# menmitsu/opticalFlowClustering

Measured on AMD Instinct MI355X. Metric: Mpixels/s dense flow+kmeans @1080p, higher is better.
Workload: dtype f32 storage, f64 accumulation; 1 GPU; BASELINE.json configs[2]: 300-frame 1080p synthetic clip, Farneback flow (0.5,3,15,3,5,1.2,0) + Lloyd k=5 over (u,v), frames sharded over 1 GPU(s); width=1920, height=1080, frames=300, pairs=299, k=5, lloyd_iters=11, flow_batch_pairs=64

## Files before the change

include/ofc.h:

```cpp
#ifndef OFC_H
#define OFC_H
#include <stddef.h>
#include <stdint.h>

#ifdef __cplusplus
extern "C" {
#endif

#define OFC_VERSION 100

enum {
    OFC_OK = 0,
    OFC_EINVAL = -1,
    OFC_ENODEV = -2,
    OFC_EHIP = -3,
    OFC_ENOMEM = -4,
    OFC_ENOTREADY = -5,
    OFC_EUNSUPPORTED = -6,
    OFC_ECOMM = -7
};

enum { OFC_U8 = 0, OFC_F32 = 1, OFC_F64 = 2 };

int ofc_version(void);
const char *ofc_last_error(void);
int ofc_device_count(int *n);

int ofc_malloc(int device, size_t bytes, void **dptr);
int ofc_free(int device, void *dptr);
int ofc_memcpy_h2d(int device, void *dst_dev, const void *src_host, size_t bytes);
int ofc_memcpy_d2h(int device, void *dst_host, const void *src_dev, size_t bytes);
int ofc_memset(int device, void *dst_dev, int value, size_t bytes);
int ofc_device_sync(int device);

typedef struct ofc_fb_params {
    double pyr_scale;
    int levels;
    int winsize;
    int iterations;
    int poly_n;
    double poly_sigma;
    int flags;
} ofc_fb_params;
#define OFC_WINSIZE_MAX 255

void ofc_fb_default_params(ofc_fb_params *p);

typedef struct ofc_flow ofc_flow_t;

int ofc_flow_create(int device, int W, int H, const ofc_fb_params *p, int max_batch,
                    ofc_flow_t **out);
void ofc_flow_destroy(ofc_flow_t *f);

int ofc_flow_calc(ofc_flow_t *f, const uint8_t *prev_gray, const uint8_t *next_gray,
                  float *flow_out);

int ofc_flow_calc_frames_dev(ofc_flow_t *f, const uint8_t *frames_dev, int n_frames,
                             float *flow_dev);
int ofc_flow_calc_frames_dev_stats(ofc_flow_t *f, const uint8_t *frames_dev, int n_frames,
                                   float *flow_dev, double *uv_sum_dev);
int ofc_flow_sync(ofc_flow_t *f);

int ofc_flow_push_gray(ofc_flow_t *f, const uint8_t *gray, float *flow_out);

int ofc_flow_push_bgr(ofc_flow_t *f, const uint8_t *bgr, uint8_t *vis_out, float *mean_mag,
                      float *flow_out);
int ofc_flow_last_vis_dev(ofc_flow_t *f, const uint8_t **vis_dev);

int ofc_level_image(int device, const uint8_t *gray, int W, int H, const ofc_fb_params *p, int k,
                    float *out, int *w_out, int *h_out);
int ofc_polyexp(int device, const float *img, int W, int H, int n, double sigma, float *R5);
int ofc_polyexp_u8(int device, const uint8_t *gray, int W, int H, int n, double sigma, float *R5);
int ofc_update_matrices(int device, const float *R0, const float *R1, const float *flow, int W,
                        int H, float *M);
int ofc_box_solve(int device, const float *M, int W, int H, int winsize, float *flow);
int ofc_flow_resize(int device, const float *flow, int sw, int sh, int dw, int dh, float mul,
                    float *out);

int ofc_flow_iterate(int device, const float *R0, const float *R1, const float *flow_in, int W, int H,
                     int winsize, int iters, int mode, int rows_per_block, float *flow_out);
int ofc_bench_flow_iters(int device, int W, int H, int n_pairs, int reps, int mode, float *ms);

int ofc_bench_polyexp(int device, int W, int H, int n_images, int iters, int rows_per_block,
                      float *ms_per_launch);

int ofc_bgr2gray(int device, const uint8_t *bgr, int W, int H, uint8_t *gray);
int ofc_flow_to_bgr(int device, const float *flow, int W, int H, uint8_t *bgr, float *mean_mag);
int ofc_flow_to_bgr_dev(int device, const float *flow_dev, int W, int H, int n_frames,
                        uint8_t *bgr_dev, float *mean_mag_dev);
int ofc_bgr2hsv(int device, const uint8_t *bgr, int64_t npix, uint8_t *hsv);
int ofc_preprocess_rgba(int device, const uint8_t *img3, int64_t npix, int thresh, uint8_t *rgba);
int ofc_grid_cell_means(int device, const uint8_t *bgr, int W, int H, int rows, int cols,
                        uint8_t *mean_bgr, uint8_t *hsv);

int ofc_kmeans_fit(int device, const void *X, int dtype, int64_t N, int d, int k,
                   const double *init, int max_iter, double tol_rel, double *centers,
                   int32_t *labels, double *inertia, int *n_iter);
int ofc_kmeans_predict(int device, const void *X, int dtype, int64_t N, int d, int k,
                       const double *centers, int32_t *labels);
int ofc_kmeans_fit_dev(int device, const void *X_dev, int dtype, int64_t N, int d, int k,
                       const double *init, int max_iter, double tol_rel, double *centers,
                       uint8_t *labels_dev, double *inertia, int *n_iter);
int ofc_kmeans_fit_dev_stats(int device, const void *X_dev, int dtype, int64_t N, int d, int k,
                             const double *init, int max_iter, double tol_rel, const double *colsum,
                             double *centers, uint8_t *labels_dev, double *inertia, int *n_iter);
int ofc_lloyd_prune_stats(int device, double *out6);
int ofc_bench_lloyd_sweep(int device, const float *X_dev, int64_t N, int k, const double *centers, const double *mean,
                          int what, int iters, float *ms_per_launch);
int ofc_lloyd_colstats_dev(int device, const void *X_dev, int dtype, int64_t N, int d, const double *mean,
                           int pass, double *out);
int ofc_lloyd_step_dev(int device, const void *X_dev, int dtype, int64_t N, int d, int k, const double *mean,
                       const double *centers_c, uint8_t *labels_dev, int accumulate, double *record);
int ofc_lloyd_inertia_dev(int device, const void *X_dev, int dtype, int64_t N, int d, int k, const double *mean,
                          const double *centers_c, const uint8_t *labels_dev, double *inertia);
int ofc_lloyd_farthest_dev(int device, const void *X_dev, int dtype, int64_t N, int d, int k, const double *mean,
                           const double *centers_c, const uint8_t *labels_dev, const int64_t *excl, int n_excl,
                           double *dist2, int64_t *index, double *x_c, int *label);

int ofc_kpp_candidates(int device, const void *X, int dtype, int64_t N, int d, const double *mean,
                       const int64_t *cand, int n_cand, const double *closest, double *out_min, double *pots);
int ofc_kpp_seed_dev(int device, const void *X_dev, int dtype, int64_t N, int d, int k, const double *colsum,
                     int64_t first, const double *u, int n_trials, double *centers, int64_t *indices);
int ofc_kpp_sample_dev(int device, const double *w_dev, int64_t N, const double *r, int n, int64_t *idx);
#define OFC_KPP_CHUNK 1024
int ofc_kmeans_fit_batched(int device, const uint8_t *X, const int64_t *offsets, int n_problems,
                           int d, int k, const double *init, int max_iter, double tol_rel,
                           double *centers, int32_t *counts, int32_t *labels, int *n_iter);
int ofc_grid_kmeans(int device, const uint8_t *bgr, int W, int H, int rows, int cols, int k,
                    const double *init, int max_iter, double tol_rel, int channel_order,
                    double *centers, uint8_t *hsv);

int ofc_grid_kmeans_dev(int device, const uint8_t *bgr_dev, int W, int H, int n_frames, int rows,
                        int cols, int k, const double *init, int max_iter, double tol_rel,
                        int channel_order, double *centers, uint8_t *hsv);

#define OFC_UNIQUE_ID_BYTES 128
int ofc_dist_unique_id(uint8_t id[OFC_UNIQUE_ID_BYTES]);
int ofc_dist_init(int device, int rank, int world, const uint8_t id[OFC_UNIQUE_ID_BYTES]);
int ofc_dist_allreduce_f64(int device, double *buf_dev, int count);
typedef int (*ofc_host_allreduce_fn)(double *buf, int count, int op, void *user);
int ofc_dist_init_host(int device, int rank, int world, ofc_host_allreduce_fn fn, void *user);
int ofc_dist_loopback(int world);
int ofc_dist_finalize(void);

typedef struct ofc_stream ofc_stream_t;
int ofc_stream_create(int device, int W, int H, const ofc_fb_params *p, int batch_pairs, int rows, int cols,
                      ofc_stream_t **out);
int ofc_stream_push_gray(ofc_stream_t *s, const uint8_t *gray, int *pairs_done);
int ofc_stream_finish(ofc_stream_t *s, float *cell_uv, int max_pairs, int *n_pairs);
void ofc_stream_destroy(ofc_stream_t *s);
int ofc_grid_cell_mean_flow(int device, const float *flow, int W, int H, int rows, int cols, float *cell_uv);

int ofc_sliding_cosine(int device, const double *small_v, int n_small, const double *large_v, int n_large,
                       double *sims);

int ofc_synth_frames_dev(int device, uint8_t *frames_dev, int W, int H, int n_frames,
                         int t0, int seed);

#ifdef __cplusplus
}
#endif
#endif
```

opticalflowclustering_amd/_lib.py:

```python
import ctypes as C
import os

import numpy as np

_HERE = os.path.dirname(os.path.abspath(__file__))
LIB_PATH = os.path.join(_HERE, "libofc.so")

OFC_OK, OFC_EINVAL, OFC_ENODEV, OFC_EHIP, OFC_ENOMEM, OFC_ENOTREADY, OFC_EUNSUPPORTED, OFC_ECOMM = \
    0, -1, -2, -3, -4, -5, -6, -7
U8, F32, F64 = 0, 1, 2
UNIQUE_ID_BYTES = 128
KPP_CHUNK = 1024


class OfcError(RuntimeError):
    def __init__(self, code, msg):
        super().__init__(f"libofc error {code}: {msg}")
        self.code = code


class FbParams(C.Structure):
    _fields_ = [("pyr_scale", C.c_double), ("levels", C.c_int), ("winsize", C.c_int),
                ("iterations", C.c_int), ("poly_n", C.c_int), ("poly_sigma", C.c_double),
                ("flags", C.c_int)]

    def __init__(self, pyr_scale=0.5, levels=3, winsize=15, iterations=3, poly_n=5, poly_sigma=1.2,
                 flags=0):
        super().__init__(pyr_scale, levels, winsize, iterations, poly_n, poly_sigma, flags)


_lib = None

_vp, _i, _i64, _f, _d, _sz = C.c_void_p, C.c_int, C.c_int64, C.c_float, C.c_double, C.c_size_t
_ip = C.POINTER(C.c_int)
_PROTOS = {
    "ofc_version": ([], _i),
    "ofc_last_error": ([], C.c_char_p),
    "ofc_device_count": ([_ip], _i),
    "ofc_malloc": ([_i, _sz, C.POINTER(_vp)], _i),
    "ofc_free": ([_i, _vp], _i),
    "ofc_memcpy_h2d": ([_i, _vp, _vp, _sz], _i),
    "ofc_memcpy_d2h": ([_i, _vp, _vp, _sz], _i),
    "ofc_memset": ([_i, _vp, _i, _sz], _i),
    "ofc_device_sync": ([_i], _i),
    "ofc_fb_default_params": ([C.POINTER(FbParams)], None),
    "ofc_flow_create": ([_i, _i, _i, C.POINTER(FbParams), _i, C.POINTER(_vp)], _i),
    "ofc_flow_destroy": ([_vp], None),
    "ofc_flow_calc": ([_vp, _vp, _vp, _vp], _i),
    "ofc_flow_calc_frames_dev": ([_vp, _vp, _i, _vp], _i),
    "ofc_flow_calc_frames_dev_stats": ([_vp, _vp, _i, _vp, _vp], _i),
    "ofc_flow_sync": ([_vp], _i),
    "ofc_flow_push_gray": ([_vp, _vp, _vp], _i),
    "ofc_flow_push_bgr": ([_vp, _vp, _vp, C.POINTER(_f), _vp], _i),
    "ofc_flow_last_vis_dev": ([_vp, C.POINTER(_vp)], _i),
    "ofc_level_image": ([_i, _vp, _i, _i, C.POINTER(FbParams), _i, _vp, _ip, _ip], _i),
    "ofc_polyexp": ([_i, _vp, _i, _i, _i, _d, _vp], _i),
    "ofc_polyexp_u8": ([_i, _vp, _i, _i, _i, _d, _vp], _i),
    "ofc_update_matrices": ([_i, _vp, _vp, _vp, _i, _i, _vp], _i),
    "ofc_box_solve": ([_i, _vp, _i, _i, _i, _vp], _i),
    "ofc_flow_resize": ([_i, _vp, _i, _i, _i, _i, _f, _vp], _i),
    "ofc_flow_iterate": ([_i, _vp, _vp, _vp, _i, _i, _i, _i, _i, _i, _vp], _i),
    "ofc_bench_flow_iters": ([_i, _i, _i, _i, _i, _i, C.POINTER(_f)], _i),
    "ofc_bench_polyexp": ([_i, _i, _i, _i, _i, _i, C.POINTER(_f)], _i),
    "ofc_bgr2gray": ([_i, _vp, _i, _i, _vp], _i),
    "ofc_flow_to_bgr": ([_i, _vp, _i, _i, _vp, C.POINTER(_f)], _i),
    "ofc_flow_to_bgr_dev": ([_i, _vp, _i, _i, _i, _vp, _vp], _i),
    "ofc_bgr2hsv": ([_i, _vp, _i64, _vp], _i),
    "ofc_preprocess_rgba": ([_i, _vp, _i64, _i, _vp], _i),
    "ofc_grid_cell_means": ([_i, _vp, _i, _i, _i, _i, _vp, _vp], _i),
    "ofc_kmeans_fit": ([_i, _vp, _i, _i64, _i, _i, _vp, _i, _d, _vp, _vp, C.POINTER(_d), _ip], _i),
    "ofc_kmeans_predict": ([_i, _vp, _i, _i64, _i, _i, _vp, _vp], _i),
    "ofc_kmeans_fit_dev": ([_i, _vp, _i, _i64, _i, _i, _vp, _i, _d, _vp, _vp, C.POINTER(_d), _ip], _i),
    "ofc_kmeans_fit_dev_stats": ([_i, _vp, _i, _i64, _i, _i, _vp, _i, _d, _vp, _vp, _vp, C.POINTER(_d), _ip], _i),
    "ofc_lloyd_prune_stats": ([_i, _vp], _i),
    "ofc_bench_lloyd_sweep": ([_i, _vp, _i64, _i, _vp, _vp, _i, _i, C.POINTER(_f)], _i),
    "ofc_lloyd_colstats_dev": ([_i, _vp, _i, _i64, _i, _vp, _i, _vp], _i),
    "ofc_lloyd_step_dev": ([_i, _vp, _i, _i64, _i, _i, _vp, _vp, _vp, _i, _vp], _i),
    "ofc_lloyd_inertia_dev": ([_i, _vp, _i, _i64, _i, _i, _vp, _vp, _vp, C.POINTER(_d)], _i),
    "ofc_lloyd_farthest_dev": ([_i, _vp, _i, _i64, _i, _i, _vp, _vp, _vp, _vp, _i, C.POINTER(_d), C.POINTER(_i64), _vp, _ip], _i),
    "ofc_kpp_candidates": ([_i, _vp, _i, _i64, _i, _vp, _vp, _i, _vp, _vp, _vp], _i),
    "ofc_kpp_seed_dev": ([_i, _vp, _i, _i64, _i, _i, _vp, _i64, _vp, _i, _vp, _vp], _i),
    "ofc_kpp_sample_dev": ([_i, _vp, _i64, _vp, _i, _vp], _i),
    "ofc_kmeans_fit_batched": ([_i, _vp, _vp, _i, _i, _i, _vp, _i, _d, _vp, _vp, _vp, _vp], _i),
    "ofc_grid_kmeans": ([_i, _vp, _i, _i, _i, _i, _i, _vp, _i, _d, _i, _vp, _vp], _i),
    "ofc_grid_kmeans_dev": ([_i, _vp, _i, _i, _i, _i, _i, _i, _vp, _i, _d, _i, _vp, _vp], _i),
    "ofc_dist_unique_id": ([_vp], _i),
    "ofc_dist_init": ([_i, _i, _i, _vp], _i),
    "ofc_dist_allreduce_f64": ([_i, _vp, _i], _i),
    "ofc_dist_init_host": ([_i, _i, _i, _vp, _vp], _i),
    "ofc_dist_loopback": ([_i], _i),
    "ofc_dist_finalize": ([], _i),
    "ofc_stream_create": ([_i, _i, _i, C.POINTER(FbParams), _i, _i, _i, C.POINTER(_vp)], _i),
    "ofc_stream_push_gray": ([_vp, _vp, _ip], _i),
    "ofc_stream_finish": ([_vp, _vp, _i, _ip], _i),
    "ofc_stream_destroy": ([_vp], None),
    "ofc_grid_cell_mean_flow": ([_i, _vp, _i, _i, _i, _i, _vp], _i),
    "ofc_sliding_cosine": ([_i, _vp, _i, _vp, _i, _vp], _i),
    "ofc_synth_frames_dev": ([_i, _vp, _i, _i, _i, _i, _i], _i),
}
EXPORTS = tuple(_PROTOS)


def load():
    global _lib
    if _lib is None:
        if not os.path.exists(LIB_PATH):
            raise OfcError(OFC_ENODEV, f"{LIB_PATH} not built: run `make -C {_HERE}/csrc` "
                                       "(python -c 'import __graft_entry__ as g; g.build()')")
        lib = C.CDLL(LIB_PATH)
        for name, (args, res) in _PROTOS.items():
            fn = getattr(lib, name)
            fn.argtypes = args
            fn.restype = res
        _lib = lib
    return _lib


def check(rc):
    if rc != OFC_OK:
        msg = load().ofc_last_error().decode("utf-8", "replace")
        if rc == OFC_EINVAL:
            raise ValueError(msg)
        raise OfcError(rc, msg)


def ptr(a):
    return a.ctypes.data_as(C.c_void_p) if a is not None else None


def device_count():
    n = C.c_int()
    check(load().ofc_device_count(C.byref(n)))
    return n.value


class DeviceBuffer:

    def __init__(self, nbytes, device=0):
        self.device, self.nbytes = device, int(nbytes)
        p = C.c_void_p()
        check(load().ofc_malloc(device, self.nbytes, C.byref(p)))
        self.ptr = p.value

    def upload(self, arr, offset=0):
        arr = np.ascontiguousarray(arr)
        assert offset + arr.nbytes <= self.nbytes
        check(load().ofc_memcpy_h2d(self.device, self.ptr + offset, ptr(arr), arr.nbytes))
        return self

    def download(self, shape, dtype, offset=0):
        out = np.empty(shape, dtype)
        assert offset + out.nbytes <= self.nbytes
        check(load().ofc_memcpy_d2h(self.device, ptr(out), self.ptr + offset, out.nbytes))
        return out

    def zero(self):
        check(load().ofc_memset(self.device, self.ptr, 0, self.nbytes))

    def free(self):
        if self.ptr:
            load().ofc_free(self.device, self.ptr)
            self.ptr = None

    def __del__(self):
        try:
            self.free()
        except Exception:
            pass
```

opticalflowclustering_amd/cluster.py:

```python
import ctypes as C

import numpy as np

from . import _lib
from ._lib import check, load, ptr

_DT = {np.dtype(np.uint8): _lib.U8, np.dtype(np.float32): _lib.F32, np.dtype(np.float64): _lib.F64}


def _as_supported(X):
    X = np.asarray(X)
    if X.ndim != 2:
        raise ValueError(f"Expected 2D array, got {X.ndim}D array instead")
    if X.dtype not in _DT:
        X = X.astype(np.float64)
    return np.ascontiguousarray(X)


def seeded_rows_init(X, k, random_state=0):
    rng = np.random.default_rng(random_state)
    X = np.asarray(X)
    uniq = np.unique(X, axis=0)
    if len(uniq) >= k:
        return uniq[rng.choice(len(uniq), k, replace=False)].astype(np.float64)
    return X[rng.choice(len(X), k, replace=len(X) < k)].astype(np.float64)


def check_random_state(seed):
    if seed is None or seed is np.random:
        return np.random.mtrand._rand
    if isinstance(seed, (int, np.integer)):
        return np.random.RandomState(int(seed))
    if isinstance(seed, np.random.RandomState):
        return seed
    raise ValueError(f"{seed!r} cannot be used to seed a numpy.random.RandomState instance")


def kmeans_plusplus(X, n_clusters, random_state=None, n_local_trials=None, device=0, _step=None):
    X = _as_supported(X)
    N, d = X.shape
    rs = check_random_state(random_state)
    if n_local_trials is None:
        n_local_trials = 2 + int(np.log(n_clusters))
    if n_local_trials > 8:
        raise ValueError("n_local_trials > 8 is not supported")
    mean = X.astype(np.float64).mean(axis=0) if X.dtype != np.float32 else X.mean(axis=0).astype(np.float64)
    weight = np.ones(N, np.float64)
    indices = np.full(n_clusters, -1, dtype=np.int64)
    indices[0] = rs.choice(N, p=weight / weight.sum())

    def step(cand, closest):
        cand = np.ascontiguousarray(cand, np.int64)
        if _step is not None:
            return _step(X, mean, cand, closest)
        out = np.empty((len(cand), N), np.float64)
        pots = np.empty(len(cand), np.float64)
        check(load().ofc_kpp_candidates(device, ptr(X), _DT[X.dtype], N, d, ptr(mean), ptr(cand), len(cand),
                                        ptr(closest) if closest is not None else None, ptr(out), ptr(pots)))
        return out, pots

    out, pots = step(indices[:1], None)
    closest, current_pot = out[0], pots[0]
    for c in range(1, n_clusters):
        rand_vals = rs.uniform(size=n_local_trials) * current_pot
        candidate_ids = np.searchsorted(np.cumsum(closest, dtype=np.float64), rand_vals)
        np.clip(candidate_ids, None, N - 1, out=candidate_ids)
        out, pots = step(candidate_ids, closest)
        best = int(np.argmin(pots))
        current_pot, closest = pots[best], out[best]
        indices[c] = candidate_ids[best]
    return X[indices].astype(np.float64), indices


KPP_CHOICE_MAX = 1 << 24


def kpp_draws(rs, N, n_clusters, n_local_trials=None):
    if n_local_trials is None:
        n_local_trials = 2 + int(np.log(n_clusters))
    if n_local_trials > 8:
        raise ValueError("n_local_trials > 8 is not supported")
    if N <= KPP_CHOICE_MAX:
        weight = np.ones(N, np.float64)
        first = int(rs.choice(N, p=weight / weight.sum()))
    else:
        first = min(int(rs.random_sample() * N), N - 1)
    u = np.empty((n_clusters - 1, n_local_trials), np.float64)
    for c in range(n_clusters - 1):
        u[c] = rs.uniform(size=n_local_trials)
    return first, u, n_local_trials


def kmeans_plusplus_dev(X_ptr, dtype, N, d, n_clusters, random_state=None, n_local_trials=None, device=0,
                        colsum=None, n_global=None):
    n_global = int(N if n_global is None else n_global)
    if n_global < 1:
        raise ValueError(f"n_samples={n_global} should be >= n_clusters={n_clusters}.")
    first, u, n_local_trials = kpp_draws(check_random_state(random_state), n_global, int(n_clusters), n_local_trials)
    cs = np.ascontiguousarray(colsum, np.float64) if colsum is not None else None
    if cs is not None and cs.shape != (d,):
        raise ValueError(f"colsum must have shape ({d},)")
    centers = np.empty((n_clusters, d), np.float64)
    indices = np.empty(n_clusters, np.int64)
    check(load().ofc_kpp_seed_dev(device, C.c_void_p(X_ptr), dtype, N, d, n_clusters, ptr(cs), first, ptr(u),
                                  n_local_trials, ptr(centers), ptr(indices)))
    return centers, indices


class KMeans:
    def __init__(self, n_clusters=8, *, init="seeded-rows", n_init=1, max_iter=300, tol=1e-4,
                 random_state=0, device=0, **_ignored):
        self.n_clusters, self.init, self.n_init = int(n_clusters), init, n_init
        self.max_iter, self.tol, self.random_state, self.device = int(max_iter), float(tol), random_state, device

    def _init_centers(self, X):
        if isinstance(self.init, str):
            if self.init == "k-means++":
                return None
            if self.init not in ("seeded-rows", "random"):
                raise ValueError(f"init should be an array, 'k-means++' or 'seeded-rows', got {self.init!r}")
            return seeded_rows_init(X, self.n_clusters, self.random_state if self.random_state is not None else 0)
        C0 = np.ascontiguousarray(self.init, np.float64)
        if C0.shape != (self.n_clusters, X.shape[1]):
            raise ValueError(f"The shape of the initial centers {C0.shape} does not match "
                             f"({self.n_clusters}, {X.shape[1]})")
        return C0

    def fit(self, X, y=None, sample_weight=None):
        if sample_weight is not None:
            raise ValueError("sample_weight is not supported (the reference never passes it)")
        X = _as_supported(X)
        N, d = X.shape
        k = self.n_clusters
        if N < k:
            raise ValueError(f"n_samples={N} should be >= n_clusters={k}.")
        C0 = self._init_centers(X)
        centers = np.empty((k, d), np.float64)
        labels = np.empty(N, np.int32)
        inertia, n_iter = C.c_double(), C.c_int()
        if C0 is None:
            Xd = _lib.DeviceBuffer(X.nbytes, self.device)
            Ld = _lib.DeviceBuffer(N, self.device)
            try:
                Xd.upload(X)
                C0, _ = kmeans_plusplus_dev(Xd.ptr, _DT[X.dtype], N, d, k, self.random_state, device=self.device)
                check(load().ofc_kmeans_fit_dev(self.device, C.c_void_p(Xd.ptr), _DT[X.dtype], N, d, k, ptr(C0),
                                                self.max_iter, self.tol, ptr(centers), C.c_void_p(Ld.ptr),
                                                C.byref(inertia), C.byref(n_iter)))
                labels[:] = Ld.download((N,), np.uint8)
            finally:
                Xd.free()
                Ld.free()
        else:
            check(load().ofc_kmeans_fit(self.device, ptr(X), _DT[X.dtype], N, d, k, ptr(C0), self.max_iter,
                                        self.tol, ptr(centers), ptr(labels), C.byref(inertia), C.byref(n_iter)))
        self.cluster_centers_, self.labels_ = centers, labels
        self.inertia_, self.n_iter_ = inertia.value, n_iter.value
        self.n_features_in_ = d
        return self

    def predict(self, X):
        X = _as_supported(X)
        N, d = X.shape
        if d != self.cluster_centers_.shape[1]:
            raise ValueError(f"X has {d} features, but KMeans is expecting {self.cluster_centers_.shape[1]}")
        labels = np.empty(N, np.int32)
        cen = np.ascontiguousarray(self.cluster_centers_, np.float64)
        check(load().ofc_kmeans_predict(self.device, ptr(X), _DT[X.dtype], N, d, self.n_clusters, ptr(cen), ptr(labels)))
        return labels

    def fit_predict(self, X, y=None):
        return self.fit(X).labels_


def kmeans_fit_dev(X_ptr, dtype, N, d, init, max_iter=300, tol=1e-4, labels_ptr=None, device=0, colsum=None):
    C0 = np.ascontiguousarray(init, np.float64)
    k = C0.shape[0]
    centers = np.empty((k, d), np.float64)
    inertia, n_iter = C.c_double(), C.c_int()
    cs = np.ascontiguousarray(colsum, np.float64) if colsum is not None else None
    if cs is not None and cs.shape != (d,):
        raise ValueError(f"colsum must have shape ({d},)")
    check(load().ofc_kmeans_fit_dev_stats(device, C.c_void_p(X_ptr), dtype, N, d, k, ptr(C0), max_iter, tol, ptr(cs), ptr(centers),
                                          C.c_void_p(labels_ptr) if labels_ptr else None, C.byref(inertia), C.byref(n_iter)))
    return centers, inertia.value, n_iter.value


def prune_stats(device=0):
    out = np.zeros(6, np.float64)
    check(load().ofc_lloyd_prune_stats(device, ptr(out)))
    return {"tile_sweeps": int(out[0]), "pruned_sweeps": int(out[1]), "probe_sweeps": int(out[4]), "final_pruned": bool(out[5]),
            "skip_fraction": float(out[3] / out[2]) if out[2] > 0 else 0.0}
```

opticalflowclustering_amd/csrc/flow_kernels.hip:

```cpp
#include "flow_device.h"

namespace ofc {

__device__ __forceinline__ void lin_tap_x(int dx, double scale, int sw, int &s0, float &a)
{
#pragma clang fp contract(off)
    float fx = (float)((dx + 0.5) * scale - 0.5);
    int sx = (int)floorf(fx);
    fx -= (float)sx;
    if (sx < 0) { fx = 0.f; sx = 0; }
    if (sx >= sw - 1) { fx = 0.f; sx = sw - 1; }
    s0 = sx;
    a = fx;
}

__device__ __forceinline__ void lin_tap_y(int dy, double scale, int sh, int &s0, int &s1, float &b)
{
#pragma clang fp contract(off)
    float fy = (float)((dy + 0.5) * scale - 0.5);
    int sy = (int)floorf(fy);
    fy -= (float)sy;
    s0 = min(max(sy, 0), sh - 1);
    s1 = min(max(sy + 1, 0), sh - 1);
    b = fy;
}

__device__ __forceinline__ int reflect101(int p, int len)
{
    if (len == 1) return 0;
    while (p < 0 || p >= len) p = p < 0 ? -p : 2 * (len - 1) - p;
    return p;
}

struct LevelArgs {
    int W0, H0, w, h;
    int r;
    int txo, tyo;
    int in_w, in_h;
    int in_pitch;
    double sx, sy;
    float kern[32];
};

__global__ __launch_bounds__(256) void k_level_image(const uint8_t *__restrict__ src,
                                                     float *__restrict__ dst, LevelArgs p)
{
#pragma clang fp contract(off)
    extern __shared__ __align__(16) unsigned char smem[];
    const int tid = threadIdx.x;
    const int ox0 = blockIdx.x * p.txo, oy0 = blockIdx.y * p.tyo;
    const int nox = min(p.txo, p.w - ox0), noy = min(p.tyo, p.h - oy0);
    const uint8_t *img = src + (size_t)blockIdx.z * p.W0 * p.H0;
    float *out = dst + (size_t)blockIdx.z * p.w * p.h;

    int *xs0 = reinterpret_cast<int *>(smem);
    float *xa = reinterpret_cast<float *>(xs0 + p.txo);
    int *ys0 = reinterpret_cast<int *>(xa + p.txo);
    int *ys1 = ys0 + p.tyo;
    float *yb = reinterpret_cast<float *>(ys1 + p.tyo);
    float *h1 = yb + p.tyo;
    unsigned char *tile = reinterpret_cast<unsigned char *>(h1 + (size_t)p.in_h * 2 * p.txo);

    if (tid < nox) {
        int s0; float a;
        lin_tap_x(ox0 + tid, p.sx, p.W0, s0, a);
        xs0[tid] = s0; xa[tid] = a;
    }
    if (tid >= 64 && tid - 64 < noy) {
        int s0, s1; float b;
        lin_tap_y(oy0 + tid - 64, p.sy, p.H0, s0, s1, b);
        ys0[tid - 64] = s0; ys1[tid - 64] = s1; yb[tid - 64] = b;
    }
    __syncthreads();
    const int x_first = xs0[0], x_last = min(xs0[nox - 1] + 1, p.W0 - 1);
    const int y_first = ys0[0], y_last = ys1[noy - 1];
    const int ix0 = x_first - p.r, iy0 = y_first - p.r;
    const int tw = x_last - x_first + 1 + 2 * p.r, th = y_last - y_first + 1 + 2 * p.r;

    for (int i = tid; i < tw * th; i += 256) {
        int ly = i / tw, lx = i - ly * tw;
        int gx = reflect101(ix0 + lx, p.W0), gy = reflect101(iy0 + ly, p.H0);
        tile[ly * p.in_pitch + lx] = img[(size_t)gy * p.W0 + gx];
    }
    __syncthreads();

    const int ks = 2 * p.r + 1;
    for (int i = tid; i < th * nox * 2; i += 256) {
        int ly = i / (nox * 2), rem = i - ly * nox * 2;
        int j = rem >> 1, t = rem & 1;
        int x = min(xs0[j] + t, p.W0 - 1);
        const unsigned char *row = tile + ly * p.in_pitch + (x - x_first);
        float acc = p.kern[0] * (float)row[0];
        for (int q = 1; q < ks; q++) acc += p.kern[q] * (float)row[q];
        h1[(ly * p.txo + j) * 2 + t] = acc;
    }
    __syncthreads();

    for (int i = tid; i < noy * nox; i += 256) {
        int oy = i / nox, ox = i - oy * nox;
        float a1 = xa[ox], a0 = 1.f - a1, b1 = yb[oy], b0 = 1.f - b1;
        float hrow[2];
#pragma unroll
        for (int yt = 0; yt < 2; yt++) {
            int c = (yt ? ys1[oy] : ys0[oy]) - iy0;
            float v[2];
#pragma unroll
            for (int t = 0; t < 2; t++) {
                if (t == 1 && a1 == 0.f) { v[1] = 0.f; continue; }
                const float *col = h1 + (c * p.txo + ox) * 2 + t;
                float acc = p.kern[p.r] * col[0];
                for (int m = 1; m <= p.r; m++)
                    acc += p.kern[p.r + m] * (col[-m * p.txo * 2] + col[m * p.txo * 2]);
                v[t] = acc;
            }
            hrow[yt] = (a1 == 0.f) ? v[0] : v[0] * a0 + v[1] * a1;
        }
        out[(size_t)(oy0 + oy) * p.w + ox0 + ox] = hrow[0] * b0 + hrow[1] * b1;
    }
}

__device__ __forceinline__ float ubyte_of(uint32_t w, int n) { return (float)((w >> (8 * n)) & 255u); }

__global__ __launch_bounds__(256) void k_level0(const uint8_t *__restrict__ src, float *__restrict__ dst,
                                                int W, int H, float k0, float k1, float k2)
{
#pragma clang fp contract(off)
    const int tx = threadIdx.x & 63, ty = threadIdx.x >> 6;
    const int x0 = blockIdx.x * 256 + 4 * tx, y0 = blockIdx.y * 32 + 8 * ty;
    if (x0 >= W || y0 >= H) return;
    const uint8_t *img = src + (size_t)blockIdx.z * W * H;
    float *out = dst + (size_t)blockIdx.z * W * H;
    const bool fast = x0 >= 4 && x0 + 8 <= W;
    float h[10][4];
#pragma unroll
    for (int j = 0; j < 10; j++) {
        const uint8_t *row = img + (size_t)reflect101(y0 - 1 + j, H) * W;
        float b[6];
        if (fast) {
            const uint32_t *rw = reinterpret_cast<const uint32_t *>(row + x0);
            const uint32_t wa = rw[-1], wb = rw[0], wc = rw[1];
            b[0] = ubyte_of(wa, 3);
            b[1] = ubyte_of(wb, 0); b[2] = ubyte_of(wb, 1); b[3] = ubyte_of(wb, 2); b[4] = ubyte_of(wb, 3);
            b[5] = ubyte_of(wc, 0);
        } else {
#pragma unroll
            for (int q = 0; q < 6; q++) b[q] = (float)row[reflect101(x0 - 1 + q, W)];
        }
#pragma unroll
        for (int c = 0; c < 4; c++) {
            float acc = k0 * b[c];
            acc += k1 * b[c + 1];
            acc += k2 * b[c + 2];
            h[j][c] = acc;
// ... 648 lines not shown

        double ex[5];
#pragma unroll
        for (int c = 0; c < 5; c++) {
            double s = 0;
#pragma unroll
            for (int i = 0; i < 4; i++) s += in[i] ? v[c][i] : 0.0;
            double t = s;
#pragma unroll
            for (int d = 1; d < 64; d <<= 1) {
                const double o = __shfl_up(t, d);
                if (lane >= d) t += o;
            }
            ex[c] = __shfl_up(t, 1);
            if (lane == 0) ex[c] = 0;
            if (lane == 63) wtot[c][wave] = t;
        }
        __syncthreads();
#pragma unroll
        for (int c = 0; c < 5; c++) {
            double off = ex[c];
            for (int w = 0; w < wave; w++) off += wtot[c][w];
            double p[4], s = 0;
#pragma unroll
            for (int i = 0; i < 4; i++) {
                s += in[i] ? v[c][i] : 0.0;
                p[i] = s + off;
            }
            *reinterpret_cast<double2 *>(&P[c][4 * tid]) = make_double2(p[0], p[1]);
            *reinterpret_cast<double2 *>(&P[c][4 * tid + 2]) = make_double2(p[2], p[3]);
        }
#pragma unroll
        for (int i = 0; i < 4; i++) {
            if (in[i] && col[i] == 0)
#pragma unroll
                for (int c = 0; c < 5; c++) edge[0][c] = v[c][i];
            if (in[i] && col[i] == W - 1)
#pragma unroll
                for (int c = 0; c < 5; c++) edge[1][c] = v[c][i];
        }
        __syncthreads();
        for (int j = tid; j < TX; j += 256) {
            const int x = x0 + j;
            if (x >= W) break;
            const double nr = (double)max(x + m - (W - 1), 0), nl = (double)max(m - x, 0);
            double S[5];
#pragma unroll
            for (int c = 0; c < 5; c++) {
                S[c] = P[c][j + 2 * m + 1] - P[c][j];
                if (nr > 0) S[c] += nr * edge[1][c];
                if (nl > 0) S[c] += nl * edge[0][c];
            }
            const double g11 = S[0] * scale, g12 = S[1] * scale, g22 = S[2] * scale, h1 = S[3] * scale,
                         h2 = S[4] * scale;
            const double idet = 1. / (g11 * g22 - g12 * g12 + 1e-3);
            flow[(size_t)y * W + x] = make_float2((float)((g11 * h2 - g12 * h1) * idet),
                                                  (float)((g22 * h1 - g12 * h2) * idet));
        }
        __syncthreads();
#pragma unroll
        for (int c = 0; c < 5; c++)
#pragma unroll
            for (int i = 0; i < 4; i++) v[c][i] += (double)fa[c][i] - (double)Mp[c * plane + os + col[i]];
    }
}

int box_wide_rows(int winsize) { return std::max(2 * winsize, 64); }

static int launch_box_solve_wide(const float *M, float *flow, int npair, int W, int H, int winsize,
                                 int rows_per_block, hipStream_t s)
{
    if (!(winsize & 1) || winsize < WINSIZE_WIDE_MIN || winsize > OFC_WINSIZE_MAX) {
        set_error("winsize %d unsupported (odd 5..%d)", winsize, OFC_WINSIZE_MAX);
        return OFC_EUNSUPPORTED;
    }
    if (rows_per_block <= 0) rows_per_block = box_wide_rows(winsize);
    const int m = winsize / 2;
    dim3 grid(cdiv(W, BW_SPAN - 2 * m - 1), cdiv(H, rows_per_block), npair);
    hipLaunchKernelGGL(k_box_solve_wide, grid, dim3(256), 0, s, M, flow, W, H, m, rows_per_block);
    OFC_HIP(hipGetLastError());
    return OFC_OK;
}

int launch_box_solve(const float *M, float *flow, int npair, int W, int H, int winsize,
                     int rows_per_block, hipStream_t s)
{
    if (winsize >= WINSIZE_WIDE_MIN) return launch_box_solve_wide(M, flow, npair, W, H, winsize, rows_per_block, s);
    if (rows_per_block <= 0) rows_per_block = box_default_rows(W, H, npair);
    rows_per_block = cdiv(rows_per_block, BS_ROWS) * BS_ROWS;
    dim3 block(256);
#define OFC_BOX_CASE(MM)                                                                         \
    case 2 * MM + 1: {                                                                           \
        dim3 grid(cdiv(W, 256 - 2 * MM), cdiv(H, rows_per_block), npair);                        \
        hipLaunchKernelGGL(k_box_solve<MM>, grid, block, 0, s, M, flow, W, H, rows_per_block);   \
        break;                                                                                   \
    }
    switch (winsize) {
        OFC_BOX_CASE(2)
        OFC_BOX_CASE(3)
        OFC_BOX_CASE(4)
        OFC_BOX_CASE(5)
        OFC_BOX_CASE(6)
        OFC_BOX_CASE(7)
        OFC_BOX_CASE(8)
    default:
        set_error("winsize %d unsupported (odd 5..%d)", winsize, OFC_WINSIZE_MAX);
        return OFC_EUNSUPPORTED;
    }
#undef OFC_BOX_CASE
    OFC_HIP(hipGetLastError());
    return OFC_OK;
}

struct UpsArgs {
    const float *src;
    int sw, sh;
    double scx, scy;
    float mul;
};

__device__ __forceinline__ float2 upsampled_flow(const float2 *__restrict__ s, int sw, int sh, double scx, double scy,
                                                 float mul, int x, int y)
{
#pragma clang fp contract(off)
    int sx0, sy0, sy1;
    float a1, b1;
    if (scx == 0.5 && scy == 0.5) {
        const int sx = (x + 1) / 2 - 1, sy = (y + 1) / 2 - 1;
        a1 = (x & 1) ? 0.25f : 0.75f;
        b1 = (y & 1) ? 0.25f : 0.75f;
        sx0 = sx;
        if (sx < 0) { a1 = 0.f; sx0 = 0; }
        if (sx >= sw - 1) { a1 = 0.f; sx0 = sw - 1; }
        sy0 = min(max(sy, 0), sh - 1);
        sy1 = min(max(sy + 1, 0), sh - 1);
    } else {
        lin_tap_x(x, scx, sw, sx0, a1);
        lin_tap_y(y, scy, sh, sy0, sy1, b1);
    }
    const float a0 = 1.f - a1, b0 = 1.f - b1;
    const int sx1 = (a1 == 0.f) ? sx0 : sx0 + 1;
    const float2 p00 = s[(size_t)sy0 * sw + sx0], p01 = s[(size_t)sy0 * sw + sx1];
    const float2 p10 = s[(size_t)sy1 * sw + sx0], p11 = s[(size_t)sy1 * sw + sx1];
    float h0x, h0y, h1x, h1y;
    if (a1 == 0.f) {
        h0x = p00.x; h0y = p00.y; h1x = p10.x; h1y = p10.y;
    } else {
        h0x = p00.x * a0 + p01.x * a1; h0y = p00.y * a0 + p01.y * a1;
        h1x = p10.x * a0 + p11.x * a1; h1y = p10.y * a0 + p11.y * a1;
    }
    return make_float2((h0x * b0 + h1x * b1) * mul, (h0y * b0 + h1y * b1) * mul);
}

template <int M, int UPS, bool STAMP = false, bool SUMS = false>
__global__ __launch_bounds__(256, 2) void k_flow_iter(const float *__restrict__ Rb, size_t frame_stride_R,
                                                      const float *__restrict__ flow_inb,
                                                      float *__restrict__ flow_outb, int W, int H,
                                                      int rows_per_block , UpsArgs ups,
                                                      int tiles_x, int n_strips, int npair,
                                                      unsigned long long *__restrict__ dbg = nullptr,
                                                      double *__restrict__ sums = nullptr)
{
    constexpr int TXO = 256 - 2 * M;
    constexpr int NV = 2 * M + 4;
    constexpr int NV2 = (NV + 1) / 2;
    constexpr int PLD = 136, PITCH = 2 * PLD;
    __shared__ __align__(16) double vs[5][BS_ROWS][PITCH];
    const int tid = threadIdx.x, lane = tid & 63, wave = tid >> 6;
    const int tiles = tiles_x * n_strips;
    const int group = blockIdx.x / (8 * npair), rem = blockIdx.x - group * (8 * npair);
    const int pair = rem >> 3, tile = group * 8 + (rem & 7);
    if (tile >= tiles) {
        if (SUMS && threadIdx.x < 2) sums[(size_t)blockIdx.x * 2 + threadIdx.x] = 0.0;
        return;
    }
    double su = 0, sv = 0;
    const int tile_x = tile % tiles_x, tile_y = tile / tiles_x;
    const int x0 = tile_x * TXO;
    const int y_begin = tile_y * rows_per_block;
    const int y_end = min(y_begin + rows_per_block, H);
    const size_t plane = (size_t)W * H;
    const float *R0 = Rb + (size_t)pair * frame_stride_R;
    const float *R1 = R0 + frame_stride_R;
    const float2 *flow_in = UPS ? reinterpret_cast<const float2 *>(ups.src) + (size_t)pair * ups.sw * ups.sh
                                : reinterpret_cast<const float2 *>(flow_inb) + (size_t)pair * plane;
    float2 *flow_out = reinterpret_cast<float2 *>(flow_outb) + (size_t)pair * plane;
    const int xc = min(max(x0 - M + tid, 0), W - 1);
    const int vs_w = ((tid >> 1) & 1) * PLD + 2 * (tid >> 2) + (tid & 1);
    const double scale = 1.0 / ((2 * M + 1) * (2 * M + 1));
    auto flow_at = [&](int row) -> float2 {
        if (UPS) return upsampled_flow(flow_in, ups.sw, ups.sh, ups.scx, ups.scy, ups.mul, xc, row);
        return flow_in[(size_t)row * W + xc];
    };
    constexpr bool ups2 = UPS == 2;
    int usx0 = 0, usx1 = 0;
    float ua1 = 0.f;
    if (ups2) {
        const int sx = (xc + 1) / 2 - 1;
        ua1 = (xc & 1) ? 0.25f : 0.75f;
        usx0 = sx;
        if (sx < 0) { ua1 = 0.f; usx0 = 0; }
        if (sx >= ups.sw - 1) { ua1 = 0.f; usx0 = ups.sw - 1; }
        usx1 = (ua1 == 0.f) ? usx0 : usx0 + 1;
    }
    auto coarse_taps = [&](int sy, float2 &p0, float2 &p1) {
        const float2 *rowp = flow_in + (size_t)min(max(sy, 0), ups.sh - 1) * ups.sw;
        p0 = rowp[usx0];
        p1 = rowp[usx1];
    };
    auto coarse_lerp = [&](float2 p0, float2 p1) -> float2 {
#pragma clang fp contract(off)
        if (ua1 == 0.f) return p0;
        const float a0 = 1.f - ua1;
        return make_float2(p0.x * a0 + p1.x * ua1, p0.y * a0 + p1.y * ua1);
    };
    float2 hcar[2], pn[2][2];
    bool have_next = false;
    float2 fl_last = ups2 ? flow_at(H - 1) : make_float2(0.f, 0.f);

    float ring[16][5];
    double v[5] = {0, 0, 0, 0, 0};

#pragma unroll
    for (int j4 = -M; j4 <= M; j4 += BS_ROWS) {
        float2 fl[BS_ROWS];
        UmIn u[BS_ROWS];
        __builtin_amdgcn_s_setprio(3);
#pragma unroll
        for (int q = 0; q < BS_ROWS; q++) fl[q] = flow_at(min(max(y_begin + j4 + q, 0), H - 1));
#pragma unroll
        for (int q = 0; q < BS_ROWS; q++)
            um_load(R0, R1, plane, W, H, xc, min(max(y_begin + j4 + q, 0), H - 1), fl[q], u[q]);
        __builtin_amdgcn_s_setprio(0);
#pragma unroll
        for (int q = 0; q < BS_ROWS; q++) {
            if (j4 + q <= M) {
                const int row = min(max(y_begin + j4 + q, 0), H - 1);
                float m[5];
                um_math(u[q], W, H, xc, row, fl[q], m);
#pragma unroll
                for (int c = 0; c < 5; c++) {
                    ring[(j4 + q + 16) & 15][c] = m[c];
                    v[c] += (double)m[c];
                }
            }
        }
    }

    float2 fln[BS_ROWS];
    if (!UPS) {
#pragma unroll
        for (int r = 0; r < BS_ROWS; r++) fln[r] = flow_in[(size_t)min(y_begin + r + 1 + M, H - 1) * W + xc];
    }
    unsigned long long acc_t[8] = {0, 0, 0, 0, 0, 0, 0, 0}, tprev = 0;
    auto stamp = [&](int slot) {
        if (STAMP) {
            __builtin_amdgcn_sched_barrier(0);
            const unsigned long long t = __builtin_amdgcn_s_memtime();
            __builtin_amdgcn_sched_barrier(0);
            if (slot >= 0) acc_t[slot] += t - tprev;
            tprev = t;
        }
    };
    stamp(-1);
    for (int y16 = y_begin; y16 < y_end; y16 += 16) {
#pragma unroll
        for (int q4 = 0; q4 < 4; q4++) {
            const int yc = y16 + 4 * q4;
            if (yc < y_end) {
                float2 fl[BS_ROWS];
                float mi[BS_ROWS][5];
                if (ups2) {
#pragma clang fp contract(off)
                    const int e0 = yc + 1 + M, s0 = (e0 + 1) / 2 - 1;
                    float2 hc[BS_ROWS];
                    if (have_next) {
                        hc[0] = hcar[0];
                        hc[1] = hcar[1];
                        hc[2] = coarse_lerp(pn[0][0], pn[0][1]);
                        hc[3] = coarse_lerp(pn[1][0], pn[1][1]);
                    } else {
#pragma unroll
                        for (int j = 0; j < BS_ROWS; j++) {
                            float2 p0, p1;
                            coarse_taps(s0 + j, p0, p1);
                            hc[j] = coarse_lerp(p0, p1);
                        }
                    }
                    hcar[0] = hc[2];
                    hcar[1] = hc[3];
                    have_next = true;
#pragma unroll
                    for (int r = 0; r < BS_ROWS; r++) {
                        constexpr bool E0_EVEN = ((1 + M) & 1) == 0;
                        const int off = E0_EVEN ? (r + 1) / 2 : r / 2;
                        const float b1 = (E0_EVEN == ((r & 1) == 0)) ? 0.75f : 0.25f, b0 = 1.f - b1;
                        const float2 h0 = hc[off], h1 = hc[off + 1];
                        fl[r] = make_float2((h0.x * b0 + h1.x * b1) * ups.mul, (h0.y * b0 + h1.y * b1) * ups.mul);
                        if (e0 + r > H - 1) fl[r] = fl_last; else fl_last = fl[r];
                    }
                } else {
#pragma unroll
                    for (int r = 0; r < BS_ROWS; r++)
                        fl[r] = UPS ? flow_at(min(yc + r + 1 + M, H - 1)) : fln[r];
                }
                {
                    UmIn u[BS_ROWS];
                    stamp(0);
                    __builtin_amdgcn_s_setprio(3);
#pragma unroll
                    for (int q = 0; q < BS_ROWS; q++)
                        um_load(R0, R1, plane, W, H, xc, min(yc + q + 1 + M, H - 1), fl[q], u[q]);
                    if (!UPS) {
#pragma unroll
                        for (int r = 0; r < BS_ROWS; r++)
                            fln[r] = flow_in[(size_t)min(yc + BS_ROWS + r + 1 + M, H - 1) * W + xc];
                    }
                    stamp(1);
                    if (STAMP) {
                        asm volatile("s_waitcnt vmcnt(0)" ::: "memory");
                        stamp(2);
                    }
                    __builtin_amdgcn_s_setprio(2);
#pragma unroll
                    for (int r = 0; r < BS_ROWS; r++)
                        um_math(u[r], W, H, xc, min(yc + r + 1 + M, H - 1), fl[r], mi[r]);
                }
                if (ups2) {
                    const int s0n = (yc + BS_ROWS + 1 + M + 1) / 2 - 1;
                    coarse_taps(s0n + 2, pn[0][0], pn[0][1]);
                    coarse_taps(s0n + 3, pn[1][0], pn[1][1]);
                }
                stamp(7);
                __syncthreads();
                stamp(3);
#pragma unroll
                for (int r = 0; r < BS_ROWS; r++) {
                    const int s_in = (4 * q4 + r + 1 + M) & 15, s_out = (4 * q4 + r + 16 - M) & 15;
#pragma unroll
                    for (int c = 0; c < 5; c++) {
                        vs[c][r][vs_w] = v[c];
                        v[c] += (double)mi[r][c] - (double)ring[s_out][c];
                    }
#pragma unroll
                    for (int c = 0; c < 5; c++) ring[s_in][c] = mi[r][c];
                }
                stamp(4);
                __syncthreads();
                stamp(5);
                __builtin_amdgcn_s_setprio(0);
                const int y = yc + wave;
                const int xo = x0 + 4 * lane;
                if (y < y_end && 4 * lane < TXO && xo < W) {
                    double S[5][4];
#pragma unroll
                    for (int c = 0; c < 5; c++) {
                        double a[2 * NV2];
#pragma unroll
                        for (int q = 0; q < NV2; q++) {
                            double2 d = *reinterpret_cast<const double2 *>(&vs[c][wave][(q & 1) * PLD + 2 * (lane + (q >> 1))]);
                            a[2 * q] = d.x; a[2 * q + 1] = d.y;
                        }
                        double s = a[0];
#pragma unroll
                        for (int q = 1; q <= 2 * M; q++) s += a[q];
                        S[c][0] = s;
#pragma unroll
                        for (int o = 1; o < 4; o++) {
                            s += a[2 * M + o] - a[o - 1];
                            S[c][o] = s;
                        }
                    }
                    float2 fo[4];
#pragma unroll
                    for (int o = 0; o < 4; o++) {
                        const double g11 = S[0][o] * scale, g12 = S[1][o] * scale, g22 = S[2][o] * scale,
                                     h1 = S[3][o] * scale, h2 = S[4][o] * scale;
                        const double idet = 1. / (g11 * g22 - g12 * g12 + 1e-3);
                        fo[o] = make_float2((float)((g11 * h2 - g12 * h1) * idet), (float)((g22 * h1 - g12 * h2) * idet));
                    }
                    if (SUMS) {
#pragma unroll
                        for (int o = 0; o < 4; o++)
                            if (4 * lane + o < TXO && xo + o < W) { su += (double)fo[o].x; sv += (double)fo[o].y; }
                    }
                    float2 *dst = flow_out + (size_t)y * W + xo;
                    if (4 * lane + 3 < TXO && xo + 3 < W && (W & 1) == 0) {
                        reinterpret_cast<float4 *>(dst)[0] = make_float4(fo[0].x, fo[0].y, fo[1].x, fo[1].y);
                        reinterpret_cast<float4 *>(dst)[1] = make_float4(fo[2].x, fo[2].y, fo[3].x, fo[3].y);
                    } else {
#pragma unroll
                        for (int o = 0; o < 4; o++)
                            if (4 * lane + o < TXO && xo + o < W) dst[o] = fo[o];
                    }
                }
                stamp(6);
            }
        }
    }
    if (STAMP && dbg && lane == 0) {
#pragma unroll
        for (int i = 0; i < 8; i++) dbg[((size_t)blockIdx.x * 4 + wave) * 8 + i] = acc_t[i];
    }
    if (SUMS) {
        for (int off = 32; off >= 1; off >>= 1) {
            su += __shfl_down(su, off, 64);
            sv += __shfl_down(sv, off, 64);
        }
        __syncthreads();
        if (lane == 0) { vs[0][0][2 * wave] = su; vs[0][0][2 * wave + 1] = sv; }
        __syncthreads();
        if (tid < 2) sums[(size_t)blockIdx.x * 2 + tid] = ((vs[0][0][tid] + vs[0][0][2 + tid]) + vs[0][0][4 + tid]) + vs[0][0][6 + tid];
    }
}

int flow_iter_rows(int W, int H, int npair, int winsize)
{
    const int tiles_x = cdiv(W, 256 - (winsize - 1));
    const int resident = 2 * 256;
    int best_rows = cdiv(H, 16) * 16;
    int64_t best_cost = LLONG_MAX;
    for (int n = 1; n <= 32; n++) {
        const int rows = cdiv(cdiv(H, n), 16) * 16;
        if (rows < 16 && n > 1) break;
        const int64_t blocks = (int64_t)tiles_x * cdiv(H, rows) * npair;
        const int64_t cost = cdiv64(blocks, resident) * (rows + winsize - 1);
        if (cost < best_cost) { best_cost = cost; best_rows = rows; }
    }
    return best_rows;
}

int flow_iter_max_grid(int W, int H, int npair, int winsize)
{
    const int rows = flow_iter_rows(W, H, npair, winsize);
    return cdiv(cdiv(W, 256 - (winsize - 1)) * cdiv(H, rows), 8) * 8 * npair;
}

static int flow_iter_check(int W, int H, int winsize)
{
    if (winsize > 15) { set_error("fused iteration supports winsize <= 15 (ring of 16 rows)"); return OFC_EUNSUPPORTED; }
    if ((int64_t)W * H * 5 >= (1ll << 30)) { set_error("frame too large for 32-bit R offsets (%dx%d)", W, H); return OFC_EUNSUPPORTED; }
    return OFC_OK;
}

int launch_flow_iter(const float *R, size_t frame_stride_R, const float *flow_in, float *flow_out,
                     int npair, int W, int H, int winsize, hipStream_t s, const float *coarse, int sw, int sh,
                     float mul, double *uv_sum, double *uv_scratch, size_t uv_scratch_doubles)
{
    OFC_TRY(flow_iter_check(W, H, winsize));
    const int rows_per_block = flow_iter_rows(W, H, npair, winsize);
    UpsArgs u;
    u.src = coarse; u.sw = sw; u.sh = sh; u.mul = mul;
    u.scx = coarse ? (double)sw / W : 1.0; u.scy = coarse ? (double)sh / H : 1.0;
    {
        const char *e = getenv("OFC_FLOW_PIPE");
        if (e && e[0] == '1' && winsize == 15 && !coarse)
            return launch_flow_iter_pipe(R, frame_stride_R, flow_in, flow_out, npair, W, H, rows_per_block, s, uv_sum, uv_scratch,
                                         uv_scratch_doubles);
    }
    if (uv_sum) {
        if (coarse || winsize != 15) { set_error("flow sums are emitted by the plain winsize-15 iteration only"); return OFC_EUNSUPPORTED; }
        const int tx = cdiv(W, 256 - 14), ns = cdiv(H, rows_per_block);
        const int grid = cdiv(tx * ns, 8) * 8 * npair;
        if ((size_t)grid * 2 > uv_scratch_doubles) { set_error("flow sums: scratch too small (%d work-groups)", grid); return OFC_EINVAL; }
        hipLaunchKernelGGL((k_flow_iter<7, 0, false, true>), dim3(grid), dim3(256), 0, s, R, frame_stride_R, flow_in, flow_out, W, H,
                           rows_per_block, u, tx, ns, npair, nullptr, uv_scratch);
        OFC_HIP(hipGetLastError());
        return launch_reduce_records(uv_scratch, grid, 2, uv_sum, s, nullptr);
    }
    dim3 block(256);
#define OFC_FI_CASE(MM)                                                                                  \
    case 2 * MM + 1: {                                                                                   \
        const int tx = cdiv(W, 256 - 2 * MM), ns = cdiv(H, rows_per_block);                              \
        dim3 grid(cdiv(tx * ns, 8) * 8 * npair);                                                         \
        if (coarse && u.scx == 0.5 && u.scy == 0.5)                                                      \
            hipLaunchKernelGGL((k_flow_iter<MM, 2>), grid, block, 0, s, R, frame_stride_R, flow_in,      \
                               flow_out, W, H, rows_per_block, u, tx, ns, npair);                        \
        else if (coarse)                                                                                 \
            hipLaunchKernelGGL((k_flow_iter<MM, 1>), grid, block, 0, s, R, frame_stride_R, flow_in,      \
                               flow_out, W, H, rows_per_block, u, tx, ns, npair);                        \
        else                                                                                             \
            hipLaunchKernelGGL((k_flow_iter<MM, 0>), grid, block, 0, s, R, frame_stride_R, flow_in,      \
                               flow_out, W, H, rows_per_block, u, tx, ns, npair);                        \
        break;                                                                                           \
    }
    switch (winsize) {
        OFC_FI_CASE(2)
        OFC_FI_CASE(3)
        OFC_FI_CASE(4)
        OFC_FI_CASE(5)
        OFC_FI_CASE(6)
        OFC_FI_CASE(7)
    default:
        set_error("winsize %d unsupported by the fused iteration (odd 5..15)", winsize);
        return OFC_EUNSUPPORTED;
    }
#undef OFC_FI_CASE
    OFC_HIP(hipGetLastError());
    return OFC_OK;
}

int launch_flow_iter_stamped(const float *R, size_t frame_stride_R, const float *flow_in, float *flow_out, int npair, int W,
                             int H, hipStream_t s, unsigned long long *dbg, int *grid_out)
{
    const int rows_per_block = flow_iter_rows(W, H, npair, 15);
    UpsArgs u;
    u.src = nullptr; u.sw = 0; u.sh = 0; u.mul = 1.f; u.scx = 1.0; u.scy = 1.0;
    const int tx = cdiv(W, 256 - 14), ns = cdiv(H, rows_per_block);
    dim3 grid(cdiv(tx * ns, 8) * 8 * npair);
    if (grid_out) *grid_out = (int)grid.x;
    if (dbg)
        hipLaunchKernelGGL((k_flow_iter<7, 0, true>), grid, dim3(256), 0, s, R, frame_stride_R, flow_in, flow_out, W, H,
                           rows_per_block, u, tx, ns, npair, dbg);
    OFC_HIP(hipGetLastError());
    return OFC_OK;
}

int flow_levels_check(int W, int H, const ofc_fb_params &p, const LevelGeom *geom, int levels, bool fused, bool fuse_level0)
{
    for (int k = levels; k >= 0; k--) {
        const LevelGeom &g = geom[k];
        int rc = OFC_OK;
        if (!(k == 0 && fuse_level0 && polyexp_u8_ok(W, H, g))) {
            LevelArgs a;
            int path;
            size_t lds;
            rc = level_image_plan(W, H, g, true, a, path, lds);
        }
        if (rc == OFC_OK && fused) rc = flow_iter_check(g.w, g.h, p.winsize);
        if (rc == OFC_OK) continue;
        const std::string why = ofc_last_error();
        if (g.ksize > 31) {
            int ok = k;
            while (ok > 0 && geom[ok].ksize > 31) ok--;
            set_error("pyramid level %d (%dx%d, sigma %.3g) of %dx%d at pyr_scale %g: %s; levels <= %d is supported with this "
                      "pyr_scale (a level may shrink the frame by less than 13.6x)", k, g.w, g.h, g.sigma, W, H, p.pyr_scale,
                      why.c_str(), ok);
        } else {
            set_error("pyramid level %d (%dx%d) of %dx%d at pyr_scale %g: %s", k, g.w, g.h, W, H, p.pyr_scale, why.c_str());
        }
        return rc;
    }
    return OFC_OK;
}

__global__ __launch_bounds__(256) void k_flow_resize(const float2 *__restrict__ src,
                                                     float2 *__restrict__ dst, int sw, int sh, int dw,
                                                     int dh, double scx, double scy, float mul)
{
#pragma clang fp contract(off)
    const int x = blockIdx.x * 256 + threadIdx.x, y = blockIdx.y;
    if (x >= dw) return;
    const float2 *s = src + (size_t)blockIdx.z * sw * sh;
    float2 *d = dst + (size_t)blockIdx.z * dw * dh;
    if (sw == dw && sh == dh) {
        float2 v = s[(size_t)y * sw + x];
        d[(size_t)y * dw + x] = make_float2(v.x * mul, v.y * mul);
        return;
    }
    int sx0, sy0, sy1;
    float a1, b1;
    lin_tap_x(x, scx, sw, sx0, a1);
    lin_tap_y(y, scy, sh, sy0, sy1, b1);
    const float a0 = 1.f - a1, b0 = 1.f - b1;
    const int sx1 = (a1 == 0.f) ? sx0 : sx0 + 1;
    const float2 p00 = s[(size_t)sy0 * sw + sx0], p01 = s[(size_t)sy0 * sw + sx1];
    const float2 p10 = s[(size_t)sy1 * sw + sx0], p11 = s[(size_t)sy1 * sw + sx1];
    float h0x, h0y, h1x, h1y;
    if (a1 == 0.f) {
        h0x = p00.x; h0y = p00.y; h1x = p10.x; h1y = p10.y;
    } else {
        h0x = p00.x * a0 + p01.x * a1; h0y = p00.y * a0 + p01.y * a1;
        h1x = p10.x * a0 + p11.x * a1; h1y = p10.y * a0 + p11.y * a1;
    }
    d[(size_t)y * dw + x] = make_float2((h0x * b0 + h1x * b1) * mul, (h0y * b0 + h1y * b1) * mul);
}

int launch_flow_resize(const float *src, float *dst, int npair, int sw, int sh, int dw, int dh,
                       float mul, hipStream_t s)
{
    dim3 grid(cdiv(dw, 256), dh, npair);
    hipLaunchKernelGGL(k_flow_resize, grid, dim3(256), 0, s, reinterpret_cast<const float2 *>(src),
                       reinterpret_cast<float2 *>(dst), sw, sh, dw, dh, (double)sw / dw,
                       (double)sh / dh, mul);
    OFC_HIP(hipGetLastError());
    return OFC_OK;
}

}
```

opticalflowclustering_amd/csrc/lloyd_api.cpp:

```cpp
#include "lloyd_common.h"

#include <algorithm>
#include <cmath>
#include <cstdlib>
#include <mutex>

namespace ofc {

static int lloyd_grid(int64_t N)
{
    return (int)std::max<int64_t>(1, std::min<int64_t>(cdiv64(N / 4, 256), N >= (200ll << 20) ? 2048 : 1024));
}

static size_t dtype_size(int dtype) { return dtype == OFC_U8 ? 1 : (dtype == OFC_F32 ? 4 : 8); }

struct LloydScratch {
    DevBuf state, partial, tot, tot_local, excl, far, labels;
    DevBuf tile_box, tile_sum, tile_sq;
    DevBuf tile_meta;
    DevBuf kpp_closest, kpp_cs, kpp_ss;
    DevBuf kpp_io;
    double prune_stats[6] = {0, 0, 0, 0, 0, 0};
    LloydStatus *status = nullptr;
    LloydStatus *status_dev = nullptr;
    hipStream_t stream = nullptr;
    bool ready = false;
    std::mutex mu;
    int init()
    {
        if (ready) return OFC_OK;
        constexpr int NVMAX = LLOYD_NVMAX;
        OFC_HIP(hipStreamCreateWithFlags(&stream, hipStreamNonBlocking));
        OFC_TRY(state.alloc(sizeof(LloydState)));
        OFC_TRY(partial.alloc(sizeof(double) * 2048 * NVMAX));
        OFC_TRY(tot.alloc(sizeof(double) * (NVMAX + 8)));
        OFC_TRY(tot_local.alloc(sizeof(double) * (NVMAX + 8)));
        OFC_TRY(excl.alloc(sizeof(int64_t) * LLOYD_KMAX));
        OFC_TRY(far.alloc(sizeof(double) * 2 * 2048));
        OFC_TRY(tile_meta.alloc(sizeof(double) * 8));
        OFC_HIP(hipHostMalloc((void **)&status, sizeof(LloydStatus) * LLOYD_WINDOW, hipHostMallocMapped));
        OFC_HIP(hipHostGetDevicePointer((void **)&status_dev, status, 0));
        ready = true;
        return OFC_OK;
    }
};

static int prune_policy_for(int dtype, int64_t N, int d, int k)
{
    if (!lloyd_tiles_supported(dtype, d, k) || N < 64) return LLOYD_PRUNE_OFF;
    const char *e = getenv("OFC_LLOYD_PRUNE");
    const int v = (e && e[0] >= '0' && e[0] <= '3' && !e[1]) ? e[0] - '0' : LLOYD_PRUNE_AUTO;
    if (v == LLOYD_PRUNE_AUTO && N < (1ll << 20)) return LLOYD_PRUNE_OFF;
    return v;
}

static LloydScratch &scratch_for(int device)
{
    static LloydScratch *pool = new LloydScratch[16];
    return pool[device & 15];
}

static int relocate_empty(LloydScratch &sc, const void *X, int dtype, int64_t N, int d, int k, int kmax,
                          int nblocks, const uint8_t *labels, const double *mean_h)
{
    hipStream_t s = sc.stream;
    const int NV = lloyd_record_len(kmax, d);
    std::vector<double> tot(NV);
    OFC_HIP(hipMemcpyAsync(tot.data(), sc.tot.p, sizeof(double) * NV, hipMemcpyDeviceToHost, s));
    OFC_HIP(hipStreamSynchronize(s));
    double *w = tot.data() + kmax * d;
    LloydState *st = sc.state.as<LloydState>();
    const double *c_old = st->centers;
    std::vector<int64_t> excl;
    std::vector<double> blk(2 * nblocks);
    bool first = true;
    for (int j = 0; j < k; j++) {
        if (w[j] != 0.0) continue;
        if (!excl.empty())
            OFC_HIP(hipMemcpyAsync(sc.excl.p, excl.data(), sizeof(int64_t) * excl.size(), hipMemcpyHostToDevice, s));
        OFC_TRY(launch_lloyd_farthest(X, dtype, N, d, st, c_old, labels, sc.excl.as<int64_t>(), (int)excl.size(),
                                      sc.far.as<double>(), nblocks, s));
        OFC_HIP(hipMemcpyAsync(blk.data(), sc.far.p, sizeof(double) * 2 * nblocks, hipMemcpyDeviceToHost, s));
        OFC_HIP(hipStreamSynchronize(s));
        double best = -1;
        int64_t bi = -1;
        for (int b = 0; b < nblocks; b++) {
            const double v = blk[2 * b];
            const int64_t i = (int64_t)blk[2 * b + 1];
            if (i < 0) continue;
            if (v > best || (v == best && i < bi)) { best = v; bi = i; }
        }
        double rec[LLOYD_DMAX + 3];
        int owner = 1;
        if (dist_active()) {
            double *dv = sc.far.as<double>();
            double g = best;
            OFC_HIP(hipMemcpyAsync(dv, &g, sizeof(double), hipMemcpyHostToDevice, s));
            OFC_TRY(dist_allreduce_f64(dv, 1, DIST_MAX, s));
            OFC_HIP(hipMemcpyAsync(&g, dv, sizeof(double), hipMemcpyDeviceToHost, s));
            OFC_HIP(hipStreamSynchronize(s));
            double r = (bi >= 0 && best == g) ? (double)dist_rank() : 1e300;
            OFC_HIP(hipMemcpyAsync(dv, &r, sizeof(double), hipMemcpyHostToDevice, s));
            OFC_TRY(dist_allreduce_f64(dv, 1, DIST_MIN, s));
            OFC_HIP(hipMemcpyAsync(&r, dv, sizeof(double), hipMemcpyDeviceToHost, s));
            OFC_HIP(hipStreamSynchronize(s));
            owner = ((int)r == dist_rank()) && bi >= 0 && best == g;
            best = g;
        }
        if (first && !(best > 0)) return OFC_OK;
        first = false;
        memset(rec, 0, sizeof(rec));
        if (owner) {
            unsigned char raw[LLOYD_DMAX * 8];
            uint8_t lab;
            OFC_HIP(hipMemcpyAsync(raw, (const char *)X + (size_t)bi * d * dtype_size(dtype), d * dtype_size(dtype),
                                   hipMemcpyDeviceToHost, s));
            OFC_HIP(hipMemcpyAsync(&lab, labels + bi, 1, hipMemcpyDeviceToHost, s));
            OFC_HIP(hipStreamSynchronize(s));
            for (int f = 0; f < d; f++) {
                double v = dtype == OFC_U8 ? (double)raw[f]
                         : dtype == OFC_F32 ? (double)((float *)raw)[f] : ((double *)raw)[f];
                rec[f] = v - mean_h[f];
            }
            rec[d] = (double)lab;
            excl.push_back(bi);
        }
        if (dist_active()) {
            double *dv = sc.far.as<double>();
            OFC_HIP(hipMemcpyAsync(dv, rec, sizeof(double) * (d + 1), hipMemcpyHostToDevice, s));
            OFC_TRY(dist_allreduce_f64(dv, d + 1, DIST_BCAST, s));
            OFC_HIP(hipMemcpyAsync(rec, dv, sizeof(double) * (d + 1), hipMemcpyDeviceToHost, s));
            OFC_HIP(hipStreamSynchronize(s));
        }
        const int old = (int)rec[d];
        for (int f = 0; f < d; f++) {
            tot[old * d + f] -= rec[f];
            tot[j * d + f] = rec[f];
        }
        w[j] = 1.0;
        w[old] -= 1.0;
    }
    OFC_HIP(hipMemcpyAsync(sc.tot.p, tot.data(), sizeof(double) * NV, hipMemcpyHostToDevice, s));
    OFC_HIP(hipStreamSynchronize(s));
    return OFC_OK;
}

static int lloyd_fit_dev(int device, const void *X, int dtype, int64_t N, int d, int k, const double *init,
                         int max_iter, double tol_rel, double *centers, uint8_t *labels_dev,
                         double *inertia, int *n_iter, const double *colsum = nullptr)
{
    OFC_REQUIRE(X && init && centers, "null pointer");
    OFC_REQUIRE(dtype >= OFC_U8 && dtype <= OFC_F64, "bad dtype %d", dtype);
    OFC_REQUIRE(d >= 1 && k >= 1 && max_iter >= 1 && N >= 0, "bad shape");
    if (d > LLOYD_DMAX || k > LLOYD_KMAX) {
        set_error("k=%d, d=%d outside the kernels' range (k <= %d, d <= %d)", k, d, LLOYD_KMAX, LLOYD_DMAX);
        return OFC_EUNSUPPORTED;
    }
    OFC_TRY(ensure_device(device));
    const int kmax = lloyd_kmax(k);
    const int NV = lloyd_record_len(kmax, d);
    LloydScratch &sc = scratch_for(device);
    std::lock_guard<std::mutex> lock(sc.mu);
    OFC_TRY(sc.init());
    hipStream_t s = sc.stream;
    const int nblocks = lloyd_grid(N);
    if (!labels_dev) {
        if (sc.labels.bytes < (size_t)std::max<int64_t>(N, 1)) OFC_TRY(sc.labels.alloc((size_t)std::max<int64_t>(N, 1)));
        labels_dev = sc.labels.as<uint8_t>();
    }
    LloydState *st = sc.state.as<LloydState>();
    OFC_HIP(hipMemsetAsync(st, 0, sizeof(LloydState), s));
    double *tot = sc.tot.as<double>();

    double hbuf[LLOYD_DMAX + 1], mean_h[LLOYD_DMAX];
    if (colsum) {
        OFC_HIP(hipMemcpyAsync(tot, colsum, sizeof(double) * d, hipMemcpyHostToDevice, s));
    } else {
        OFC_TRY(launch_lloyd_colstats(X, dtype, N, d, st->mean, 0, sc.partial.as<double>(), nblocks, s));
        OFC_TRY(launch_reduce_records(sc.partial.as<double>(), nblocks, d, tot, s));
    }
    double nloc = (double)N;
    OFC_HIP(hipMemcpyAsync(tot + d, &nloc, sizeof(double), hipMemcpyHostToDevice, s));
    OFC_TRY(dist_allreduce_f64(tot, d + 1, DIST_SUM, s));
    OFC_HIP(hipMemcpyAsync(hbuf, tot, sizeof(double) * (d + 1), hipMemcpyDeviceToHost, s));
    OFC_HIP(hipStreamSynchronize(s));
    const double Ng = hbuf[d];
    if (Ng < (double)k) {
        set_error("n_samples=%.0f should be >= n_clusters=%d.", Ng, k);
        return OFC_EINVAL;
    }
    for (int f = 0; f < d; f++) mean_h[f] = hbuf[f] / Ng;
    OFC_HIP(hipMemcpyAsync(st->mean, mean_h, sizeof(double) * d, hipMemcpyHostToDevice, s));

    double c0[LLOYD_KMAX * LLOYD_DMAX];
    for (int j = 0; j < k * d; j++) c0[j] = init[j] - mean_h[j % d];
    OFC_HIP(hipMemcpyAsync(st->centers, c0, sizeof(double) * k * d, hipMemcpyHostToDevice, s));
    const int prune = prune_policy_for(dtype, N, d, k);
    if (prune) {
        const size_t need = (size_t)(N >> 6) * 16;
        if (sc.tile_box.bytes < need) {
            OFC_TRY(sc.tile_box.alloc(need));
            OFC_TRY(sc.tile_sum.alloc(need));
            OFC_TRY(sc.tile_sq.alloc(need / 2));
        }
    }
    for (double &v : sc.prune_stats) v = 0;
    OFC_TRY(launch_lloyd_set_centers(st, k, d, s, prune));
    bool strict = false, labelled = false, stop = false;
    int tiles_next = LLOYD_TILES_FULL;
    const bool trace = getenv("OFC_LLOYD_TRACE") != nullptr;
    int it = 0;
    const int *halt = &st->halt;
    double *tot_local = dist_has_comm() ? sc.tot_local.as<double>() : tot;
    int window = 4;
    while (it < max_iter && !stop) {
        const int nwin = std::min(window, max_iter - it);
        window = std::min(2 * window, LLOYD_WINDOW);
        for (int w = 0; w < nwin; w++) sc.status[w].valid = 0;
        for (int w = 0; w < nwin; w++) {
            const int tiles = (prune && !labelled) ? (it + w == 0 ? 1 : 2) : 0;
            if (tiles == 1) {
                OFC_TRY(launch_lloyd_tiles((const float *)X, N, k, st, nullptr, nullptr, nullptr, nullptr,
                                           sc.partial.as<double>(), nblocks, LLOYD_WHAT_PROBE, nullptr, s));
                OFC_TRY(launch_lloyd_tiles((const float *)X, N, k, st, sc.tile_box.p, sc.tile_sum.p, sc.tile_sq.p, nullptr,
                                           sc.partial.as<double>(), nblocks, LLOYD_WHAT_META, nullptr, s));
                OFC_TRY(launch_reduce_records(sc.partial.as<double>(), nblocks, 2, sc.tile_meta.as<double>(), s));
            }
            if (tiles)
                OFC_TRY(launch_lloyd_tiles((const float *)X, N, k, st, sc.tile_box.p, sc.tile_sum.p, sc.tile_sq.p, nullptr,
                                           sc.partial.as<double>(), nblocks, LLOYD_WHAT_SWEEP,
                                           tiles == 1 ? sc.tile_meta.as<double>() : nullptr, s));
            else
                OFC_TRY(launch_lloyd_assign(X, dtype, N, d, k, st, labels_dev, sc.partial.as<double>(), nblocks,
                                            labelled ? 1 : 3, it + w == 0, s));
            OFC_TRY(launch_reduce_records(sc.partial.as<double>(), nblocks, NV, tot_local, s, halt));
            OFC_TRY(dist_allreduce_f64(tot_local, tot, NV, DIST_SUM, s));
            OFC_TRY(launch_lloyd_update(st, tot, k, d, 0, labelled, it + w == 0, Ng, tol_rel, sc.status_dev + w, s, tiles));
        }
        OFC_HIP(hipStreamSynchronize(s));
        int done = nwin;
        for (int w = 0; w < nwin; w++) {
            LloydStatus &S = sc.status[w];
            if (!S.valid) { set_error("internal: Lloyd iteration %d did not run", it + w); return OFC_EHIP; }
            if (trace)
                fprintf(stderr, "[ofc lloyd] it %d tiles_mode %d tested %.0f pure %.0f shift %.3e empty %d\n", it + w,
                        S.tiles_mode, S.tiles_tested, S.tiles_pure, S.shift_tot, S.n_empty);
            if (S.tiles_mode != -1) {
                tiles_next = S.tiles_next;
                sc.prune_stats[0] += 1;
                if (S.tiles_mode == LLOYD_TILES_PRUNED) {
                    sc.prune_stats[1] += 1;
                    sc.prune_stats[2] += S.tiles_tested;
                    sc.prune_stats[3] += S.tiles_pure;
                } else if (S.tiles_mode == LLOYD_TILES_PROBE) {
                    sc.prune_stats[4] += 1;
                }
            }
            if (S.n_empty > 0) {
                const bool was_labelled = labelled;
                if (!labelled) {
                    OFC_TRY(launch_lloyd_assign(X, dtype, N, d, k, st, labels_dev, nullptr, nblocks, 0, 0, s));
                    labelled = true;
                }
                OFC_TRY(relocate_empty(sc, X, dtype, N, d, k, kmax, nblocks, labels_dev, mean_h));
                S.valid = 0;
                OFC_TRY(launch_lloyd_update(st, tot, k, d, 1, was_labelled, it + w == 0, Ng, tol_rel, sc.status_dev + w, s));
                OFC_HIP(hipStreamSynchronize(s));
                done = w + 1;
                if (S.converged) { strict = S.strict != 0; it += w; stop = true; }
                break;
            }
            if (S.converged) { strict = S.strict != 0; it += w; stop = true; break; }
        }
        if (!stop) it += done;
    }
    if (!stop) it = max_iter - 1;
    const bool final_tiles = !strict && prune && !labelled && tiles_next == LLOYD_TILES_PRUNED;
    sc.prune_stats[5] = final_tiles ? 1 : 0;
    if (final_tiles)
        OFC_TRY(launch_lloyd_tiles((const float *)X, N, k, st, sc.tile_box.p, sc.tile_sum.p, sc.tile_sq.p, labels_dev,
                                   sc.partial.as<double>(), nblocks, LLOYD_WHAT_FINAL, nullptr, s));
    else if (!strict)
        OFC_TRY(launch_lloyd_assign(X, dtype, N, d, k, st, labels_dev, sc.partial.as<double>(), nblocks, 2, 0, s));
    else
        OFC_TRY(launch_lloyd_inertia(X, dtype, N, d, st, labels_dev, sc.partial.as<double>(), nblocks, s));
    OFC_TRY(launch_reduce_records(sc.partial.as<double>(), nblocks, 1, tot, s));
    OFC_TRY(dist_allreduce_f64(tot, 1, DIST_SUM, s));
    double in = 0, cfin[LLOYD_KMAX * LLOYD_DMAX];
    OFC_HIP(hipMemcpyAsync(&in, tot, sizeof(double), hipMemcpyDeviceToHost, s));
    OFC_HIP(hipMemcpyAsync(cfin, st->centers, sizeof(double) * k * d, hipMemcpyDeviceToHost, s));
    OFC_HIP(hipStreamSynchronize(s));
    for (int j = 0; j < k * d; j++) centers[j] = cfin[j] + mean_h[j % d];
    if (inertia) *inertia = in;
    if (n_iter) *n_iter = it + 1;
    return OFC_OK;
}

static int lloyd_predict_dev(int device, const void *X, int dtype, int64_t N, int d, int k,
                             const double *centers, uint8_t *labels_dev)
{
    OFC_TRY(ensure_device(device));
    if (d > LLOYD_DMAX || k > LLOYD_KMAX || d < 1 || k < 1) {
        set_error("k=%d, d=%d outside the kernels' range (k <= %d, d <= %d)", k, d, LLOYD_KMAX, LLOYD_DMAX);
        return OFC_EUNSUPPORTED;
    }
    DevBuf state;
    OFC_TRY(state.alloc(sizeof(LloydState)));
    LloydState *st = state.as<LloydState>();
    OFC_HIP(hipMemset(st, 0, sizeof(LloydState)));
    OFC_HIP(hipMemcpy(st->centers, centers, sizeof(double) * k * d, hipMemcpyHostToDevice));
    OFC_TRY(launch_lloyd_set_centers(st, k, d, nullptr));
    const int nblocks = lloyd_grid(N);
    OFC_TRY(launch_lloyd_assign(X, dtype, N, d, k, st, labels_dev, nullptr, nblocks, 0, 0, nullptr));
    OFC_HIP(hipStreamSynchronize(nullptr));
    return OFC_OK;
}

static void widen_labels(const uint8_t *src, int64_t N, int32_t *dst)
{
    for (int64_t i = 0; i < N; i++) dst[i] = src[i];
}

}

using namespace ofc;

extern "C" {

int ofc_kmeans_fit_dev(int device, const void *X_dev, int dtype, int64_t N, int d, int k, const double *init,
                       int max_iter, double tol_rel, double *centers, uint8_t *labels_dev, double *inertia,
                       int *n_iter)
{
    return lloyd_fit_dev(device, X_dev, dtype, N, d, k, init, max_iter, tol_rel, centers, labels_dev, inertia, n_iter);
}

int ofc_bench_lloyd_sweep(int device, const float *X_dev, int64_t N, int k, const double *centers, const double *mean,
                          int what, int iters, float *ms_per_launch)
{
    OFC_REQUIRE(X_dev && centers && mean && ms_per_launch && iters >= 1 && N >= 64, "bad arguments");
    OFC_REQUIRE(what >= 0 && what <= 5, "what = %d outside 0..5", what);
    if (!lloyd_tiles_supported(OFC_F32, 2, k)) { set_error("k=%d outside 1..8", k); return OFC_EUNSUPPORTED; }
    OFC_TRY(ensure_device(device));
    LloydScratch &sc = scratch_for(device);
    std::lock_guard<std::mutex> lock(sc.mu);
    OFC_TRY(sc.init());
    hipStream_t s = sc.stream;
    const int nblocks = lloyd_grid(N);
    const size_t need = (size_t)(N >> 6) * 16;
    if (sc.tile_box.bytes < need) {
        OFC_TRY(sc.tile_box.alloc(need));
        OFC_TRY(sc.tile_sum.alloc(need));
        OFC_TRY(sc.tile_sq.alloc(need / 2));
    }
    if (sc.labels.bytes < (size_t)N) OFC_TRY(sc.labels.alloc((size_t)N));
    LloydState *st = sc.state.as<LloydState>();
    OFC_HIP(hipMemsetAsync(st, 0, sizeof(LloydState), s));
    double c0[LLOYD_KMAX * LLOYD_DMAX];
    for (int j = 0; j < k * 2; j++) c0[j] = centers[j] - mean[j % 2];
    OFC_HIP(hipMemcpyAsync(st->mean, mean, sizeof(double) * 2, hipMemcpyHostToDevice, s));
    OFC_HIP(hipMemcpyAsync(st->centers, c0, sizeof(double) * k * 2, hipMemcpyHostToDevice, s));
    OFC_TRY(launch_lloyd_set_centers(st, k, 2, s, LLOYD_PRUNE_ALWAYS));
    double *partial = sc.partial.as<double>();
    const float *X = X_dev;
    auto launch = [&]() -> int {
        switch (what) {
        case 0: return launch_lloyd_assign(X, OFC_F32, N, 2, k, st, sc.labels.as<uint8_t>(), partial, nblocks, 3, 0, s);
        case 1: case 5: return launch_lloyd_tiles(X, N, k, st, sc.tile_box.p, sc.tile_sum.p, sc.tile_sq.p, nullptr, partial, nblocks, LLOYD_WHAT_SWEEP, nullptr, s);
        case 2: return launch_lloyd_tiles(X, N, k, st, sc.tile_box.p, sc.tile_sum.p, sc.tile_sq.p, nullptr, partial, nblocks, LLOYD_WHAT_META, nullptr, s);
        case 3: return launch_lloyd_assign(X, OFC_F32, N, 2, k, st, sc.labels.as<uint8_t>(), partial, nblocks, 2, 0, s);
        default: return launch_lloyd_tiles(X, N, k, st, sc.tile_box.p, sc.tile_sum.p, sc.tile_sq.p, sc.labels.as<uint8_t>(), partial, nblocks, LLOYD_WHAT_FINAL, nullptr, s);
        }
    };
    if (what == 1 || what == 4 || what == 5) {
        OFC_TRY(launch_lloyd_tiles(X, N, k, st, sc.tile_box.p, sc.tile_sum.p, sc.tile_sq.p, nullptr, partial, nblocks, LLOYD_WHAT_META, nullptr, s));
        const int mode = what == 5 ? LLOYD_TILES_FULL : LLOYD_TILES_PRUNED;
        OFC_HIP(hipMemcpyAsync(&st->prune_mode, &mode, sizeof(int), hipMemcpyHostToDevice, s));
    }
    hipEvent_t e0, e1;
    OFC_HIP(hipEventCreate(&e0));
    OFC_HIP(hipEventCreate(&e1));
    for (int w = 0; w < 2; w++) OFC_TRY(launch());
    OFC_HIP(hipEventRecord(e0, s));
    for (int i = 0; i < iters; i++) OFC_TRY(launch());
    OFC_HIP(hipEventRecord(e1, s));
    OFC_HIP(hipEventSynchronize(e1));
    float ms = 0;
    OFC_HIP(hipEventElapsedTime(&ms, e0, e1));
    *ms_per_launch = ms / iters;
    (void)hipEventDestroy(e0);
    (void)hipEventDestroy(e1);
    return OFC_OK;
}

int ofc_lloyd_prune_stats(int device, double *out6)
{
    OFC_REQUIRE(out6, "null pointer");
    OFC_TRY(ensure_device(device));
    LloydScratch &sc = scratch_for(device);
    std::lock_guard<std::mutex> lock(sc.mu);
    for (int i = 0; i < 6; i++) out6[i] = sc.prune_stats[i];
    return OFC_OK;
}

int ofc_kmeans_fit_dev_stats(int device, const void *X_dev, int dtype, int64_t N, int d, int k, const double *init,
                             int max_iter, double tol_rel, const double *colsum, double *centers, uint8_t *labels_dev,
                             double *inertia, int *n_iter)
{
    return lloyd_fit_dev(device, X_dev, dtype, N, d, k, init, max_iter, tol_rel, centers, labels_dev, inertia, n_iter, colsum);
}

namespace {
struct StepCtx {
    DevBuf state, partial, tot, excl, far;
    int nblocks = 1;
    int init(int64_t N, int nv)
    {
        nblocks = lloyd_grid(N);
        OFC_TRY(state.alloc(sizeof(LloydState)));
        OFC_TRY(partial.alloc(sizeof(double) * (size_t)nblocks * std::max(nv, 2)));
        OFC_TRY(tot.alloc(sizeof(double) * (nv + 8)));
        OFC_HIP(hipMemset(state.p, 0, sizeof(LloydState)));
        return OFC_OK;
    }
    int set(const double *mean, const double *centers_c, int k, int d)
    {
        LloydState *st = state.as<LloydState>();
        if (mean) OFC_HIP(hipMemcpy(st->mean, mean, sizeof(double) * d, hipMemcpyHostToDevice));
        if (centers_c) {
            OFC_HIP(hipMemcpy(st->centers, centers_c, sizeof(double) * k * d, hipMemcpyHostToDevice));
            OFC_TRY(launch_lloyd_set_centers(st, k, d, nullptr));
        }
        return OFC_OK;
    }
};
int check_kd(int k, int d)
{
    if (d < 1 || k < 1 || d > LLOYD_DMAX || k > LLOYD_KMAX) {
        set_error("k=%d, d=%d outside the kernels' range (k <= %d, d <= %d)", k, d, LLOYD_KMAX, LLOYD_DMAX);
        return OFC_EUNSUPPORTED;
    }
    return OFC_OK;
}
}

int ofc_lloyd_colstats_dev(int device, const void *X_dev, int dtype, int64_t N, int d, const double *mean, int pass,
                           double *out)
{
    OFC_REQUIRE(X_dev && out && N >= 0 && (pass == 0 || mean), "bad arguments");
    OFC_TRY(check_kd(1, d));
    OFC_TRY(ensure_device(device));
    StepCtx c;
    OFC_TRY(c.init(N, d));
    OFC_TRY(c.set(pass ? mean : nullptr, nullptr, 1, d));
    LloydState *st = c.state.as<LloydState>();
    OFC_TRY(launch_lloyd_colstats(X_dev, dtype, N, d, st->mean, pass, c.partial.as<double>(), c.nblocks, nullptr));
    OFC_TRY(launch_reduce_records(c.partial.as<double>(), c.nblocks, d, c.tot.as<double>(), nullptr));
    OFC_HIP(hipMemcpy(out, c.tot.p, sizeof(double) * d, hipMemcpyDeviceToHost));
    return OFC_OK;
}

int ofc_lloyd_step_dev(int device, const void *X_dev, int dtype, int64_t N, int d, int k, const double *mean,
                       const double *centers_c, uint8_t *labels_dev, int accumulate, double *record)
{
    OFC_REQUIRE(X_dev && mean && centers_c && labels_dev && (record || !accumulate) && N >= 0, "bad arguments");
    OFC_TRY(check_kd(k, d));
    OFC_TRY(ensure_device(device));
    const int kmax = lloyd_kmax(k), NV = lloyd_record_len(kmax, d);
    StepCtx c;
    OFC_TRY(c.init(N, NV));
    OFC_TRY(c.set(mean, centers_c, k, d));
    LloydState *st = c.state.as<LloydState>();
    OFC_TRY(launch_lloyd_assign(X_dev, dtype, N, d, k, st, labels_dev, c.partial.as<double>(), c.nblocks, accumulate ? 1 : 0, 0, nullptr));
    if (accumulate) {
        OFC_TRY(launch_reduce_records(c.partial.as<double>(), c.nblocks, NV, c.tot.as<double>(), nullptr));
        std::vector<double> t(NV);
        OFC_HIP(hipMemcpy(t.data(), c.tot.p, sizeof(double) * NV, hipMemcpyDeviceToHost));
        for (int j = 0; j < k; j++) {
            for (int f = 0; f < d; f++) record[j * d + f] = t[j * d + f];
            record[k * d + j] = t[kmax * d + j];
        }
        record[k * d + k] = t[kmax * d + kmax];
    } else {
        OFC_HIP(hipStreamSynchronize(nullptr));
    }
    return OFC_OK;
}

int ofc_lloyd_inertia_dev(int device, const void *X_dev, int dtype, int64_t N, int d, int k, const double *mean,
                          const double *centers_c, const uint8_t *labels_dev, double *inertia)
{
    OFC_REQUIRE(X_dev && mean && centers_c && labels_dev && inertia && N >= 0, "bad arguments");
    OFC_TRY(check_kd(k, d));
    OFC_TRY(ensure_device(device));
    StepCtx c;
    OFC_TRY(c.init(N, 2));
    OFC_TRY(c.set(mean, centers_c, k, d));
    OFC_TRY(launch_lloyd_inertia(X_dev, dtype, N, d, c.state.as<LloydState>(), labels_dev, c.partial.as<double>(), c.nblocks, nullptr));
    OFC_TRY(launch_reduce_records(c.partial.as<double>(), c.nblocks, 1, c.tot.as<double>(), nullptr));
    OFC_HIP(hipMemcpy(inertia, c.tot.p, sizeof(double), hipMemcpyDeviceToHost));
    return OFC_OK;
}

int ofc_lloyd_farthest_dev(int device, const void *X_dev, int dtype, int64_t N, int d, int k, const double *mean,
                           const double *centers_c, const uint8_t *labels_dev, const int64_t *excl, int n_excl,
                           double *dist2, int64_t *index, double *x_c, int *label)
{
    OFC_REQUIRE(X_dev && mean && centers_c && labels_dev && dist2 && index && x_c && label && N >= 0, "bad arguments");
    OFC_REQUIRE(n_excl >= 0 && n_excl <= LLOYD_KMAX && (n_excl == 0 || excl), "bad exclusion list");
    OFC_TRY(check_kd(k, d));
    OFC_TRY(ensure_device(device));
    StepCtx c;
    OFC_TRY(c.init(N, 2));
    OFC_TRY(c.set(mean, centers_c, k, d));
    OFC_TRY(c.excl.alloc(sizeof(int64_t) * LLOYD_KMAX));
    if (n_excl) OFC_HIP(hipMemcpy(c.excl.p, excl, sizeof(int64_t) * n_excl, hipMemcpyHostToDevice));
    LloydState *st = c.state.as<LloydState>();
    OFC_TRY(launch_lloyd_farthest(X_dev, dtype, N, d, st, st->centers, labels_dev, c.excl.as<int64_t>(), n_excl,
                                  c.partial.as<double>(), c.nblocks, nullptr));
    std::vector<double> blk(2 * c.nblocks);
    OFC_HIP(hipMemcpy(blk.data(), c.partial.p, sizeof(double) * 2 * c.nblocks, hipMemcpyDeviceToHost));
    double best = -1;
    int64_t bi = -1;
    for (int b = 0; b < c.nblocks; b++) {
        const double v = blk[2 * b];
        const int64_t i = (int64_t)blk[2 * b + 1];
        if (i < 0) continue;
        if (v > best || (v == best && i < bi)) { best = v; bi = i; }
    }
    *dist2 = bi >= 0 ? best : -1;
    *index = bi;
    *label = -1;
    if (bi >= 0) {
        unsigned char raw[LLOYD_DMAX * 8];
        uint8_t lab;
        OFC_HIP(hipMemcpy(raw, (const char *)X_dev + (size_t)bi * d * dtype_size(dtype), d * dtype_size(dtype), hipMemcpyDeviceToHost));
        OFC_HIP(hipMemcpy(&lab, labels_dev + bi, 1, hipMemcpyDeviceToHost));
        for (int f = 0; f < d; f++) {
            double v = dtype == OFC_U8 ? (double)raw[f] : dtype == OFC_F32 ? (double)((float *)raw)[f] : ((double *)raw)[f];
            x_c[f] = v - mean[f];
        }
        *label = lab;
    }
    return OFC_OK;
}

int ofc_kmeans_fit(int device, const void *X, int dtype, int64_t N, int d, int k, const double *init,
                   int max_iter, double tol_rel, double *centers, int32_t *labels, double *inertia, int *n_iter)
{
    OFC_REQUIRE(X && init && centers, "null pointer");
    OFC_REQUIRE(dtype >= OFC_U8 && dtype <= OFC_F64 && d >= 1 && N >= 0, "bad arguments");
    OFC_REQUIRE(N >= k, "n_samples=%lld should be >= n_clusters=%d.", (long long)N, k);
    OFC_TRY(ensure_device(device));
    DevBuf dX, dL;
    const size_t bytes = (size_t)N * d * dtype_size(dtype);
    OFC_TRY(dX.alloc(std::max<size_t>(bytes, 16)));
    OFC_TRY(dL.alloc((size_t)std::max<int64_t>(N, 1)));
    OFC_HIP(hipMemcpy(dX.p, X, bytes, hipMemcpyHostToDevice));
    OFC_TRY(lloyd_fit_dev(device, dX.p, dtype, N, d, k, init, max_iter, tol_rel, centers, dL.as<uint8_t>(), inertia, n_iter));
    if (labels) {
        std::vector<uint8_t> l8((size_t)N);
        OFC_HIP(hipMemcpy(l8.data(), dL.p, (size_t)N, hipMemcpyDeviceToHost));
// ... 277 lines not shown
```

opticalflowclustering_amd/csrc/lloyd_common.h:

```cpp
#pragma once
#include "ofc_common.h"

namespace ofc {

constexpr int LLOYD_KMAX = 16;
constexpr int LLOYD_DMAX = 4;

struct LloydState {
    double mean[LLOYD_DMAX];
    double centers[LLOYD_KMAX * LLOYD_DMAX];
    double centers_new[LLOYD_KMAX * LLOYD_DMAX];
    double cn[LLOYD_KMAX];
    double tol;
    int halt;
    int pad;
    int prune_policy;
    int prune_mode;
    int prune_cooldown, prune_backoff;
};

enum { LLOYD_TILES_FULL = 0,
       LLOYD_TILES_PRUNED = 1,
       LLOYD_TILES_PROBE = 2 };
enum { LLOYD_PRUNE_OFF = 0, LLOYD_PRUNE_AUTO = 1, LLOYD_PRUNE_ON = 2, LLOYD_PRUNE_ALWAYS = 3 };

struct LloydStatus {
    double n_changed;
    double shift_tot;
    int n_empty;
    int valid;
    int converged;
    int strict;
    double tol;
    double counts[LLOYD_KMAX];
    double sqsum[LLOYD_DMAX];
    double tiles_tested, tiles_pure;
    int tiles_mode;
    int tiles_next;
};

int lloyd_kmax(int k);
int launch_lloyd_colstats(const void *X, int dtype, int64_t N, int d, const double *mean, int pass,
                          double *partial, int nblocks, hipStream_t s);
int launch_reduce_records(const double *partial, int nblocks, int nv, double *out, hipStream_t s,
                          const int *halt = nullptr);
int launch_lloyd_assign(const void *X, int dtype, int64_t N, int d, int k, const LloydState *st,
                        uint8_t *labels, double *partial, int nblocks, int mode, int first, hipStream_t s);
constexpr int LLOYD_REC_EXTRA = 1 + LLOYD_DMAX + 2;
constexpr int LLOYD_NVMAX = LLOYD_KMAX * LLOYD_DMAX + LLOYD_KMAX + LLOYD_REC_EXTRA;
inline int lloyd_record_len(int kmax, int d) { return kmax * d + kmax + LLOYD_REC_EXTRA; }
enum { LLOYD_WHAT_SWEEP = 0, LLOYD_WHAT_META = 1, LLOYD_WHAT_FINAL = 2, LLOYD_WHAT_PROBE = 3 };
bool lloyd_tiles_supported(int dtype, int d, int k);
int launch_lloyd_tiles(const float *X, int64_t N, int k, const LloydState *st, void *box, void *tsum, void *tsq,
                       uint8_t *labels, double *partial, int nblocks, int what, const double *meta, hipStream_t s);
int launch_lloyd_update(LloydState *st, const double *tot, int k, int d, int after_reloc, int labelled, int first,
                        double n_total, double tol_rel, LloydStatus *status, hipStream_t s, int tiles = 0);
constexpr int LLOYD_WINDOW = 16;
int launch_lloyd_set_centers(LloydState *st, int k, int d, hipStream_t s, int prune_policy = 0);
int launch_lloyd_inertia(const void *X, int dtype, int64_t N, int d, const LloydState *st,
                         const uint8_t *labels, double *partial, int nblocks, hipStream_t s);
int launch_lloyd_farthest(const void *X, int dtype, int64_t N, int d, const LloydState *st,
                          const double *c_old, const uint8_t *labels, const int64_t *excl, int n_excl,
                          double *out, int nblocks, hipStream_t s);

int launch_kpp_candidates(const void *X, int dtype, int64_t N, int d, const double *mean, const double *cand_centred,
                          int n_cand, const double *closest, double *out, double *partial, int nblocks, hipStream_t s);

enum { KPP_PREV_NONE = 0,
       KPP_PREV_APPLY = 1,
       KPP_PREV_FIRST = 2 };
constexpr int64_t KPP_NMAX = 1ll << 30;
inline int64_t kpp_chunks(int64_t N) { return (N + OFC_KPP_CHUNK - 1) / OFC_KPP_CHUNK; }
int launch_kpp_sweep(const void *X, int dtype, int64_t N, int d, const double *mean, const double *prev, int prev_mode,
                     const double *cand_centred, int n_cand, double *closest, double *cs, double *partial, int nblocks,
                     hipStream_t s);
int launch_kpp_sum1024(const double *in, int64_t n, double *out, hipStream_t s);
int launch_kpp_sample(const void *X, int dtype, int64_t N, int d, const double *mean, const double *prev, int prev_mode,
                      const double *closest, const double *cs, const double *ss, const double *r, int n, double base,
                      int64_t *idx, double *rows, hipStream_t s);

bool dist_active();
int dist_rank();
int dist_world();
enum { DIST_SUM = 0, DIST_MAX = 1, DIST_MIN = 2, DIST_BCAST = 3  };
int dist_allreduce_f64(double *buf_dev, int count, int op, hipStream_t s);
int dist_allreduce_f64(const double *send_dev, double *recv_dev, int count, int op, hipStream_t s);
bool dist_has_comm();
int launch_loopback_reduce(const double *send, double *recv, int count, int world, int sum, hipStream_t s);

}
```

opticalflowclustering_amd/csrc/lloyd_device.h:

```cpp
#pragma once
#include "lloyd_common.h"

namespace ofc {

template <int D>
__device__ __forceinline__ void load4(const uint8_t *X, int64_t i, double (&x)[4][D])
{
    if constexpr (D == 4) {
        const uint4 v = *reinterpret_cast<const uint4 *>(X + i * 4);
        const unsigned w[4] = {v.x, v.y, v.z, v.w};
#pragma unroll
        for (int p = 0; p < 4; p++)
#pragma unroll
            for (int f = 0; f < 4; f++) x[p][f] = (double)((w[p] >> (8 * f)) & 0xffu);
    } else {
#pragma unroll
        for (int p = 0; p < 4; p++)
#pragma unroll
            for (int f = 0; f < D; f++) x[p][f] = (double)X[(i + p) * D + f];
    }
}
template <int D>
__device__ __forceinline__ void load4(const float *X, int64_t i, double (&x)[4][D])
{
    if constexpr (D == 2) {
        typedef float v4f __attribute__((ext_vector_type(4)));
        const v4f a = __builtin_nontemporal_load(reinterpret_cast<const v4f *>(X + i * 2));
        const v4f b = __builtin_nontemporal_load(reinterpret_cast<const v4f *>(X + i * 2 + 4));
        x[0][0] = a.x; x[0][1] = a.y; x[1][0] = a.z; x[1][1] = a.w;
        x[2][0] = b.x; x[2][1] = b.y; x[3][0] = b.z; x[3][1] = b.w;
    } else if constexpr (D == 4) {
#pragma unroll
        for (int p = 0; p < 4; p++) {
            const float4 a = *reinterpret_cast<const float4 *>(X + (i + p) * 4);
            x[p][0] = a.x; x[p][1] = a.y; x[p][2] = a.z; x[p][3] = a.w;
        }
    } else {
#pragma unroll
        for (int p = 0; p < 4; p++)
#pragma unroll
            for (int f = 0; f < D; f++) x[p][f] = (double)X[(i + p) * D + f];
    }
}
template <int D>
__device__ __forceinline__ void load4(const double *X, int64_t i, double (&x)[4][D])
{
#pragma unroll
    for (int p = 0; p < 4; p++)
#pragma unroll
        for (int f = 0; f < D; f++) x[p][f] = X[(i + p) * D + f];
}
template <int D, class T>
__device__ __forceinline__ void load1(const T *X, int64_t i, double (&x)[D])
{
#pragma unroll
    for (int f = 0; f < D; f++) x[f] = (double)X[i * D + f];
}

template <int NV>
__device__ __forceinline__ void block_reduce_store(double (&v)[NV], double *lds , double *out)
{
    const int lane = threadIdx.x & 63, wave = threadIdx.x >> 6;
#pragma unroll
    for (int i = 0; i < NV; i++) {
        double a = v[i];
#pragma unroll
        for (int off = 32; off >= 1; off >>= 1) a += __shfl_down(a, off, 64);
        if (lane == 0) lds[wave * NV + i] = a;
    }
    __syncthreads();
    if (threadIdx.x < NV) {
        const int i = threadIdx.x;
        out[i] = ((lds[i] + lds[NV + i]) + lds[2 * NV + i]) + lds[3 * NV + i];
    }
    __syncthreads();
}

}
```

opticalflowclustering_amd/csrc/lloyd_tiles.hip:

```cpp
#include "lloyd_common.h"

#include <algorithm>

namespace ofc {

typedef float v4f __attribute__((ext_vector_type(4)));
typedef double v2d __attribute__((ext_vector_type(2)));

template <int N> __device__ __forceinline__ int row_ror(int v)
{
    return __builtin_amdgcn_update_dpp(0, v, 0x120 + N, 0xf, 0xf, false);
}
template <int N> __device__ __forceinline__ float row_ror(float v) { return __int_as_float(row_ror<N>(__float_as_int(v))); }
template <int N> __device__ __forceinline__ double row_ror(double v)
{
    return __hiloint2double(row_ror<N>(__double2hiint(v)), row_ror<N>(__double2loint(v)));
}
__device__ __forceinline__ float row_min(float v)
{
    v = fminf(v, row_ror<8>(v)); v = fminf(v, row_ror<4>(v)); v = fminf(v, row_ror<2>(v)); return fminf(v, row_ror<1>(v));
}
__device__ __forceinline__ float row_max(float v)
{
    v = fmaxf(v, row_ror<8>(v)); v = fmaxf(v, row_ror<4>(v)); v = fmaxf(v, row_ror<2>(v)); return fmaxf(v, row_ror<1>(v));
}
__device__ __forceinline__ double row_sum(double v)
{
    v += row_ror<8>(v); v += row_ror<4>(v); v += row_ror<2>(v); return v + row_ror<1>(v);
}

template <int KMAX> struct TileCtx {
    double c[KMAX * 2], cn[KMAX], m[2];
    const double (*s_cen)[4];

    __device__ __forceinline__ void load(const LloydState *st, double (*lds)[4])
    {
#pragma unroll
        for (int j = 0; j < KMAX; j++) {
            cn[j] = st->cn[j];
            c[2 * j] = st->centers[2 * j];
            c[2 * j + 1] = st->centers[2 * j + 1];
        }
        m[0] = st->mean[0];
        m[1] = st->mean[1];
        if (threadIdx.x < KMAX) {
            lds[threadIdx.x][0] = st->centers[threadIdx.x * 2];
            lds[threadIdx.x][1] = st->centers[threadIdx.x * 2 + 1];
            lds[threadIdx.x][2] = st->cn[threadIdx.x];
        }
        s_cen = lds;
        __syncthreads();
    }
    __device__ __forceinline__ int label_of(double x0, double x1) const
    {
        double best = 0;
        int label = 0;
#pragma unroll
        for (int j = 0; j < KMAX; j++) {
            const double dj = cn[j] - 2.0 * fma(x1, c[2 * j + 1], x0 * c[2 * j]);
            if (j == 0 || dj < best) { best = dj; label = j; }
        }
        return label;
    }
    __device__ __forceinline__ void centre_of(int j, double &cjx, double &cjy, double &cnj) const
    {
        cjx = s_cen[j][0]; cjy = s_cen[j][1]; cnj = s_cen[j][2];
    }
    __device__ __forceinline__ int box_label(double lox, double loy, double hix, double hiy) const
    {
        const int j = label_of(lox, loy);
        double cjx, cjy, cnj;
        centre_of(j, cjx, cjy, cnj);
        const double ax = fmax(fabs(lox), fabs(hix)), ay = fmax(fabs(loy), fabs(hiy));
        bool pure = true;
#pragma unroll
        for (int q = 0; q < KMAX; q++) {
            const double gx = c[2 * q] - cjx, gy = c[2 * q + 1] - cjy;
            const double wmax = (cnj - cn[q]) + 2.0 * (fmax(lox * gx, hix * gx) + fmax(loy * gy, hiy * gy));
            const double mag = (fabs(cnj) + fabs(cn[q])) +
                               4.0 * (ax * (fabs(c[2 * q]) + fabs(cjx)) + ay * (fabs(c[2 * q + 1]) + fabs(cjy)));
            pure = pure && (q == j || wmax < -1e-12 * mag);
        }
        return pure ? j : -1;
    }
    __device__ __forceinline__ double sq_dist(double x0, double x1, int l) const
    {
#pragma clang fp contract(off)
        double cjx, cjy, cnj;
        centre_of(l, cjx, cjy, cnj);
        double r = 0;
        r += (x0 - cjx) * (x0 - cjx);
        r += (x1 - cjy) * (x1 - cjy);
        return r;
    }
};

template <int KMAX>
__global__ __launch_bounds__(256) void k_tile_probe(const float *__restrict__ X, int64_t N,
                                                    const LloydState *__restrict__ st, double *__restrict__ partial)
{
    __shared__ double s_cen[KMAX][4];
    __shared__ unsigned s_red[4][2];
    TileCtx<KMAX> cx;
    cx.load(st, s_cen);
    const int tid = threadIdx.x, lane = tid & 63, wave = tid >> 6, row = lane >> 4, r16 = lane & 15;
    const int64_t NT = N >> 6, NS = (NT + 3) >> 2;
    const int64_t nw = (int64_t)gridDim.x * 4, w = (int64_t)blockIdx.x * 4 + wave;
    const int64_t stride = NS > 64 * nw ? 64 : (NS > nw ? NS / nw : 1);
    unsigned n_tested = 0, n_pure = 0;
    for (int64_t s = w * stride; s < NS; s += nw * stride) {
        const int64_t t = s * 4 + row;
        if (t < NT) {
            const v4f *p = reinterpret_cast<const v4f *>(X + t * 128 + r16 * 8);
            const v4f a = p[0], b = p[1];
            const float lu = row_min(fminf(fminf(a.x, a.z), fminf(b.x, b.z)));
            const float lv = row_min(fminf(fminf(a.y, a.w), fminf(b.y, b.w)));
            const float hu = row_max(fmaxf(fmaxf(a.x, a.z), fmaxf(b.x, b.z)));
            const float hv = row_max(fmaxf(fmaxf(a.y, a.w), fmaxf(b.y, b.w)));
            const int tl = cx.box_label((double)lu - cx.m[0], (double)lv - cx.m[1], (double)hu - cx.m[0], (double)hv - cx.m[1]);
            if (r16 == 0) {
                n_tested += 1u;
                n_pure += (tl >= 0);
            }
        }
    }
    for (int off = 32; off >= 1; off >>= 1) {
        n_tested += __shfl_down(n_tested, off, 64);
        n_pure += __shfl_down(n_pure, off, 64);
    }
    if (lane == 0) { s_red[wave][0] = n_tested; s_red[wave][1] = n_pure; }
    __syncthreads();
    if (tid < 2) partial[(size_t)blockIdx.x * 2 + tid] = (double)(s_red[0][tid] + s_red[1][tid] + s_red[2][tid] + s_red[3][tid]);
}

__global__ void k_tile_decide(LloydState *st, const double *__restrict__ partial, int nblocks)
{
    __shared__ double s[2][64];
    double a = 0, b = 0;
    for (int i = threadIdx.x; i < nblocks; i += 64) { a += partial[2 * i]; b += partial[2 * i + 1]; }
    s[0][threadIdx.x] = a;
    s[1][threadIdx.x] = b;
    __syncthreads();
    if (threadIdx.x != 0) return;
    double tested = 0, pure = 0;
    for (int i = 0; i < 64; i++) { tested += s[0][i]; pure += s[1][i]; }
    if (st->prune_policy != LLOYD_PRUNE_ALWAYS && !(pure >= 0.45 * tested && tested > 0)) st->prune_policy = LLOYD_PRUNE_OFF;
    st->prune_mode = st->prune_policy == LLOYD_PRUNE_OFF ? LLOYD_TILES_FULL : LLOYD_TILES_PRUNED;
}

__global__ __launch_bounds__(256) void k_tile_meta(const float *__restrict__ X, int64_t N,
                                                   const LloydState *__restrict__ st, v4f *__restrict__ box,
                                                   v2d *__restrict__ tsum, double *__restrict__ tsq,
                                                   double *__restrict__ partial)
{
    __shared__ double s_red[4][2];
    const int tid = threadIdx.x, lane = tid & 63, wave = tid >> 6, row = lane >> 4, r16 = lane & 15;
    if (st->prune_policy == LLOYD_PRUNE_OFF) {
        if (tid < 2) partial[(size_t)blockIdx.x * 2 + tid] = 0.0;
        return;
    }
    const double m0 = st->mean[0], m1 = st->mean[1];
    const int64_t NT = N >> 6;
    const int64_t NS = (NT + 3) >> 2;
    const int64_t s0 = (int64_t)blockIdx.x * 4 + wave, ss = (int64_t)gridDim.x * 4;
    double sq0 = 0, sq1 = 0;
    auto fetch = [&](int64_t s, v4f &a, v4f &b) {
        const int64_t t = s * 4 + row;
        if (s < NS && t < NT) {
            const v4f *p = reinterpret_cast<const v4f *>(X + t * 128 + r16 * 8);
            a = __builtin_nontemporal_load(p);
            b = __builtin_nontemporal_load(p + 1);
        }
    };
    v4f na = {0, 0, 0, 0}, nb = na;
    fetch(s0, na, nb);
    for (int64_t s = s0; s < NS; s += ss) {
        const v4f a = na, b = nb;
        fetch(s + ss, na, nb);
        const int64_t t = s * 4 + row;
        if (t < NT) {
            const double x00 = (double)a.x - m0, x01 = (double)a.y - m1, x10 = (double)a.z - m0, x11 = (double)a.w - m1;
            const double x20 = (double)b.x - m0, x21 = (double)b.y - m1, x30 = (double)b.z - m0, x31 = (double)b.w - m1;
            sq0 += x00 * x00; sq0 += x10 * x10; sq0 += x20 * x20; sq0 += x30 * x30;
            sq1 += x01 * x01; sq1 += x11 * x11; sq1 += x21 * x21; sq1 += x31 * x31;
            const float lu = row_min(fminf(fminf(a.x, a.z), fminf(b.x, b.z)));
            const float lv = row_min(fminf(fminf(a.y, a.w), fminf(b.y, b.w)));
            const float hu = row_max(fmaxf(fmaxf(a.x, a.z), fmaxf(b.x, b.z)));
            const float hv = row_max(fmaxf(fmaxf(a.y, a.w), fmaxf(b.y, b.w)));
            const double su = row_sum((x00 + x10) + (x20 + x30));
            const double sv = row_sum((x01 + x11) + (x21 + x31));
            const double mu = su * 0.015625, mv = sv * 0.015625;
            double sc = (x00 - mu) * (x00 - mu) + (x01 - mv) * (x01 - mv);
            sc += (x10 - mu) * (x10 - mu) + (x11 - mv) * (x11 - mv);
            sc += (x20 - mu) * (x20 - mu) + (x21 - mv) * (x21 - mv);
            sc += (x30 - mu) * (x30 - mu) + (x31 - mv) * (x31 - mv);
            sc = row_sum(sc);
            if (r16 == 0) {
                v4f bx = {lu, lv, hu, hv};
                if (!(su == su && sv == sv)) bx = v4f{__builtin_inff(), __builtin_inff(), -__builtin_inff(), -__builtin_inff()};
                box[t] = bx;
                tsum[t] = v2d{su, sv};
                tsq[t] = sc;
            }
        }
    }
    if (blockIdx.x == 0 && tid < (int)(N - NT * 64)) {
        const int64_t i = NT * 64 + tid;
        const double x0 = (double)X[i * 2] - m0, x1 = (double)X[i * 2 + 1] - m1;
        sq0 += x0 * x0;
        sq1 += x1 * x1;
    }
    for (int off = 32; off >= 1; off >>= 1) {
        sq0 += __shfl_down(sq0, off, 64);
        sq1 += __shfl_down(sq1, off, 64);
    }
    if (lane == 0) { s_red[wave][0] = sq0; s_red[wave][1] = sq1; }
    __syncthreads();
    if (tid < 2) partial[(size_t)blockIdx.x * 2 + tid] = ((s_red[0][tid] + s_red[1][tid]) + s_red[2][tid]) + s_red[3][tid];
}

enum { TILES_SWEEP = 0, TILES_FINAL = 1 };

template <int KMAX, int WHAT>
__global__ __launch_bounds__(256) void k_lloyd_tiles(const float *__restrict__ X, int64_t N,
                                                     const LloydState *__restrict__ st, const v4f *__restrict__ box,
                                                     const v2d *__restrict__ tsum, const double *__restrict__ tsq,
                                                     uint8_t *__restrict__ labels, double *__restrict__ partial,
                                                     const double *__restrict__ meta)
{
    constexpr int D = 2, k = KMAX;
    constexpr int NV = KMAX * D + KMAX + LLOYD_REC_EXTRA;
    constexpr bool FINAL = WHAT == TILES_FINAL, ACCUM = !FINAL;
    if (ACCUM && st->halt) return;
    const int mode = ACCUM ? st->prune_mode : LLOYD_TILES_PRUNED;
    const bool own_sq = ACCUM && meta && st->prune_policy == LLOYD_PRUNE_OFF;
    double sq0 = 0, sq1 = 0;
    extern __shared__ __align__(16) unsigned char smem[];
    double *sacc = reinterpret_cast<double *>(smem);
    unsigned *scnt = reinterpret_cast<unsigned *>(sacc + (size_t)k * D * 256);
    __shared__ unsigned s_tiles[4][2];
    __shared__ double s_cen[KMAX][4];
    const int tid = threadIdx.x, lane = tid & 63, wave = tid >> 6, row = lane >> 4, r16 = lane & 15;
    if (ACCUM) {
        for (int i = 0; i < k * D; i++) sacc[i * 256 + tid] = 0.0;
        for (int j = 0; j < k; j++) scnt[j * 256 + tid] = 0u;
    }
    TileCtx<KMAX> cx;
    cx.load(st, s_cen);
    double inert = 0;
    unsigned n_tested = 0, n_pure = 0;
    auto accumulate = [&](int l, double x0, double x1, unsigned n) {
        sacc[(l * D) * 256 + tid] += x0;
        sacc[(l * D + 1) * 256 + tid] += x1;
        scnt[l * 256 + tid] += n;
    };
    auto walk = [&](int64_t t, const v4f a, const v4f b) {
        double x[4][D];
        x[0][0] = a.x; x[0][1] = a.y; x[1][0] = a.z; x[1][1] = a.w;
        x[2][0] = b.x; x[2][1] = b.y; x[3][0] = b.z; x[3][1] = b.w;
        int nl[4];
#pragma unroll
        for (int p = 0; p < 4; p++) {
            x[p][0] -= cx.m[0];
            x[p][1] -= cx.m[1];
            nl[p] = cx.label_of(x[p][0], x[p][1]);
        }
        if (ACCUM) {
#pragma unroll
            for (int p = 0; p < 4; p++) accumulate(nl[p], x[p][0], x[p][1], 1u);
            if (own_sq) {
#pragma unroll
                for (int p = 0; p < 4; p++) {
                    sq0 += x[p][0] * x[p][0];
                    sq1 += x[p][1] * x[p][1];
                }
            }
        }
        if (FINAL) {
#pragma unroll
            for (int p = 0; p < 4; p++) inert += cx.sq_dist(x[p][0], x[p][1], nl[p]);
            __builtin_nontemporal_store((unsigned)(nl[0] | (nl[1] << 8) | (nl[2] << 16) | (nl[3] << 24)),
                                        reinterpret_cast<unsigned *>(labels) + t * 16 + r16);
        }
    };

    const int64_t NT = N >> 6;
    const int64_t NG = (NT + 63) >> 6;
    const int64_t wg = (int64_t)blockIdx.x * 4 + wave, nw = (int64_t)gridDim.x * 4;
    for (int64_t g = wg; g < NG; g += nw) {
        const int64_t t = g * 64 + lane;
        const bool valid = t < NT;
        unsigned long long todo;
        if (mode == LLOYD_TILES_FULL) {
            todo = __ballot(valid);
        } else {
            int j = -1;
            if (valid) {
                const v4f b = box[t];
                j = cx.box_label((double)b.x - cx.m[0], (double)b.y - cx.m[1], (double)b.z - cx.m[0], (double)b.w - cx.m[1]);
                n_tested += 1u;
                n_pure += (j >= 0);
            }
            const bool skip = j >= 0 && mode == LLOYD_TILES_PRUNED;
            if (skip) {
                const v2d s = tsum[t];
                if (ACCUM) accumulate(j, s.x, s.y, 64u);
                if (FINAL) {
#pragma clang fp contract(off)
                    double cjx, cjy, cnj;
                    cx.centre_of(j, cjx, cjy, cnj);
                    const double du = s.x * 0.015625 - cjx, dv = s.y * 0.015625 - cjy;
                    inert += tsq[t] + 64.0 * (du * du + dv * dv);
                    const unsigned w4 = (unsigned)j * 0x01010101u;
                    typedef unsigned v4u __attribute__((ext_vector_type(4)));
                    v4u *lp = reinterpret_cast<v4u *>(labels + t * 64);
#pragma unroll
                    for (int q = 0; q < 4; q++) __builtin_nontemporal_store((v4u){w4, w4, w4, w4}, lp + q);
                }
            }
            todo = __ballot(valid && !skip);
        }
        while (todo) {
            int ta[8];
#pragma unroll
            for (int i = 0; i < 8; i++) {
                if (todo) {
                    ta[i] = __builtin_ctzll(todo);
                    todo &= todo - 1;
                } else {
                    ta[i] = -1;
                }
            }
            const int tA = row == 0 ? ta[0] : row == 1 ? ta[1] : row == 2 ? ta[2] : ta[3];
            const int tB = row == 0 ? ta[4] : row == 1 ? ta[5] : row == 2 ? ta[6] : ta[7];
            const int64_t tileA = g * 64 + tA, tileB = g * 64 + tB;
            v4f a0 = {0, 0, 0, 0}, a1 = a0, b0 = a0, b1 = a0;
            if (tA >= 0) {
                const v4f *p = reinterpret_cast<const v4f *>(X + tileA * 128 + r16 * 8);
                a0 = __builtin_nontemporal_load(p);
                a1 = __builtin_nontemporal_load(p + 1);
            }
            if (tB >= 0) {
                const v4f *p = reinterpret_cast<const v4f *>(X + tileB * 128 + r16 * 8);
                b0 = __builtin_nontemporal_load(p);
                b1 = __builtin_nontemporal_load(p + 1);
            }
            if (tA >= 0) walk(tileA, a0, a1);
            if (tB >= 0) walk(tileB, b0, b1);
        }
    }
    if (blockIdx.x == 0 && tid < (int)(N - NT * 64)) {
        const int64_t i = NT * 64 + tid;
        const double x0 = (double)X[i * 2] - cx.m[0], x1 = (double)X[i * 2 + 1] - cx.m[1];
        const int l = cx.label_of(x0, x1);
        if (ACCUM) accumulate(l, x0, x1, 1u);
        if (own_sq) {
            sq0 += x0 * x0;
            sq1 += x1 * x1;
        }
        if (FINAL) {
            inert += cx.sq_dist(x0, x1, l);
            labels[i] = (uint8_t)l;
        }
    }
    if (FINAL) {
        __shared__ double lds_in[4];
        for (int off = 32; off >= 1; off >>= 1) inert += __shfl_down(inert, off, 64);
        if (lane == 0) lds_in[wave] = inert;
        __syncthreads();
        if (tid == 0) partial[blockIdx.x] = ((lds_in[0] + lds_in[1]) + lds_in[2]) + lds_in[3];
        return;
    }
    double *rec = partial + (size_t)blockIdx.x * NV;
    if (tid < NV) rec[tid] = 0.0;
    for (int off = 32; off >= 1; off >>= 1) {
        n_tested += __shfl_down(n_tested, off, 64);
        n_pure += __shfl_down(n_pure, off, 64);
    }
    if (lane == 0) { s_tiles[wave][0] = n_tested; s_tiles[wave][1] = n_pure; }
    __syncthreads();
    for (int i = wave; i < k * D + k; i += 4) {
        double a;
        if (i < k * D) {
            const double *col = sacc + (size_t)i * 256;
            a = ((col[lane] + col[lane + 64]) + col[lane + 128]) + col[lane + 192];
        } else {
            const unsigned *col = scnt + (size_t)(i - k * D) * 256;
            a = (double)col[lane] + (double)col[lane + 64] + (double)col[lane + 128] + (double)col[lane + 192];
        }
        for (int off = 32; off >= 1; off >>= 1) a += __shfl_down(a, off, 64);
        if (lane == 0) rec[i < k * D ? i : KMAX * D + (i - k * D)] = a;
    }
    if (tid == 0) {
        rec[KMAX * D + KMAX + 1 + LLOYD_DMAX] = (double)(s_tiles[0][0] + s_tiles[1][0] + s_tiles[2][0] + s_tiles[3][0]);
        rec[KMAX * D + KMAX + 2 + LLOYD_DMAX] = (double)(s_tiles[0][1] + s_tiles[1][1] + s_tiles[2][1] + s_tiles[3][1]);
    }
    if (own_sq) {
        __shared__ double lds_sq[4][2];
        for (int off = 32; off >= 1; off >>= 1) {
            sq0 += __shfl_down(sq0, off, 64);
            sq1 += __shfl_down(sq1, off, 64);
        }
        if (lane == 0) { lds_sq[wave][0] = sq0; lds_sq[wave][1] = sq1; }
        __syncthreads();
        if (tid < D) rec[KMAX * D + KMAX + 1 + tid] = ((lds_sq[0][tid] + lds_sq[1][tid]) + lds_sq[2][tid]) + lds_sq[3][tid];
    } else if (meta && blockIdx.x == 0 && tid >= 64 && tid < 64 + D) {
        rec[KMAX * D + KMAX + 1 + (tid - 64)] = meta[tid - 64];
    }
}

bool lloyd_tiles_supported(int dtype, int d, int k) { return dtype == OFC_F32 && d == 2 && k >= 1 && k <= 8; }

template <int KMAX>
static void launch_tiles_k(const float *X, int64_t N, const LloydState *st, void *box, void *tsum, void *tsq, uint8_t *labels,
                           double *partial, int nblocks, int what, const double *meta, hipStream_t s)
{
    const size_t lds = (size_t)KMAX * (8 * 2 + 4) * 256;
    v4f *b = (v4f *)box;
    v2d *ts = (v2d *)tsum;
    double *tq = (double *)tsq;
    if (what == LLOYD_WHAT_PROBE) {
        const int pb = std::min(nblocks, 256);
        hipLaunchKernelGGL((k_tile_probe<KMAX>), dim3(pb), dim3(256), 0, s, X, N, st, partial);
        hipLaunchKernelGGL(k_tile_decide, dim3(1), dim3(64), 0, s, const_cast<LloydState *>(st), partial, pb);
    } else if (what == LLOYD_WHAT_META)
        hipLaunchKernelGGL(k_tile_meta, dim3(nblocks), dim3(256), 0, s, X, N, st, b, ts, tq, partial);
    else if (what == LLOYD_WHAT_FINAL)
        hipLaunchKernelGGL((k_lloyd_tiles<KMAX, TILES_FINAL>), dim3(nblocks), dim3(256), 0, s, X, N, st, b, ts, tq, labels, partial, nullptr);
    else
        hipLaunchKernelGGL((k_lloyd_tiles<KMAX, TILES_SWEEP>), dim3(nblocks), dim3(256), lds, s, X, N, st, b, ts, tq, labels, partial, meta);
}

int launch_lloyd_tiles(const float *X, int64_t N, int k, const LloydState *st, void *box, void *tsum, void *tsq,
                       uint8_t *labels, double *partial, int nblocks, int what, const double *meta, hipStream_t s)
{
    switch (k) {
    case 1: launch_tiles_k<1>(X, N, st, box, tsum, tsq, labels, partial, nblocks, what, meta, s); break;
    case 2: launch_tiles_k<2>(X, N, st, box, tsum, tsq, labels, partial, nblocks, what, meta, s); break;
    case 3: launch_tiles_k<3>(X, N, st, box, tsum, tsq, labels, partial, nblocks, what, meta, s); break;
    case 4: launch_tiles_k<4>(X, N, st, box, tsum, tsq, labels, partial, nblocks, what, meta, s); break;
    case 5: launch_tiles_k<5>(X, N, st, box, tsum, tsq, labels, partial, nblocks, what, meta, s); break;
    case 6: launch_tiles_k<6>(X, N, st, box, tsum, tsq, labels, partial, nblocks, what, meta, s); break;
    case 7: launch_tiles_k<7>(X, N, st, box, tsum, tsq, labels, partial, nblocks, what, meta, s); break;
    case 8: launch_tiles_k<8>(X, N, st, box, tsum, tsq, labels, partial, nblocks, what, meta, s); break;
    default: set_error("k=%d outside the tile sweep's range (1..8)", k); return OFC_EUNSUPPORTED;
    }
    OFC_HIP(hipGetLastError());
    return OFC_OK;
}

}
```

opticalflowclustering_amd/csrc/ofc_api.cpp:

```cpp
#include "color_common.h"
#include "lloyd_common.h"

#include <cfloat>
#include <algorithm>
#include <cmath>
#include <cstdlib>
#include <memory>

namespace ofc {

static thread_local std::string g_err;

void set_error(const char *fmt, ...)
{
    char buf[1024];
    va_list ap;
    va_start(ap, fmt);
    vsnprintf(buf, sizeof(buf), fmt, ap);
    va_end(ap);
    g_err = buf;
}

int ensure_device(int device)
{
// ... 55 lines not shown
        double t = fixed ? (double)fixed[i] : std::exp(scale2X * x * x);
        k[i] = (float)t;
        sum += k[i];
    }
    sum = 1. / sum;
    for (int i = 0; i < n; i++) k[i] = (float)(k[i] * sum);
}

void polyexp_setup(int n, double sigma, PolyConsts &c)
{
    if (sigma < FLT_EPSILON) sigma = n * 0.3;
    std::vector<float> gf(2 * n + 1);
    double s = 0;
    for (int x = -n; x <= n; x++) {
        gf[x + n] = (float)std::exp(-x * x / (2 * sigma * sigma));
        s += gf[x + n];
    }
    s = 1. / s;
    for (int x = -n; x <= n; x++) gf[x + n] = (float)(gf[x + n] * s);
    memset(&c, 0, sizeof(c));
    c.n = n;
    for (int x = 0; x <= n && x < 8; x++) {
        c.g[x] = gf[x + n];
        c.xg[x] = (float)(x * c.g[x]);
        c.xxg[x] = (float)(x * x * c.g[x]);
    }
    double G00 = 0, G11 = 0, G33 = 0, G55 = 0;
    for (int y = -n; y <= n; y++)
        for (int x = -n; x <= n; x++) {
            float gg = gf[y + n] * gf[x + n];
            G00 += gg;
            G11 += gg * x * x;
            G33 += gg * x * x * x * x;
            G55 += gg * x * x * y * y;
        }
    double a = G00, b = G11, cc = G33, e = G55;
    double det = a * (cc * cc - e * e) - 2 * b * b * (cc - e);
    c.ig11 = 1. / G11;
    c.ig03 = -b * (cc - e) / det;
    c.ig33 = (a * cc - b * b) / det;
    c.ig55 = 1. / G55;
}

static int check_params(const ofc_fb_params &p, int W, int H)
{
    OFC_REQUIRE(W >= 16 && H >= 16 && W <= 16384 && H <= 16384, "frame size %dx%d out of range", W, H);
    OFC_REQUIRE(p.pyr_scale > 0 && p.pyr_scale < 1, "pyr_scale must be in (0,1)");
    OFC_REQUIRE(p.levels >= 0 && p.levels <= 16, "levels out of range");
    OFC_REQUIRE(p.iterations >= 1 && p.iterations <= 64, "iterations out of range");
    if (p.flags != 0) {
        set_error("flags=%d: only the box-filter variant (flags 0) the reference uses is implemented", p.flags);
        return OFC_EUNSUPPORTED;
    }
    if ((p.winsize & 1) && p.winsize > OFC_WINSIZE_MAX) {
        set_error("winsize %d unsupported (odd 5..%d)", p.winsize, OFC_WINSIZE_MAX);
        return OFC_EUNSUPPORTED;
    }
    return polyexp_n_check(p.poly_n);
}

}

using namespace ofc;

extern "C" {

int ofc_version(void) { return OFC_VERSION; }
const char *ofc_last_error(void) { return g_err.c_str(); }

int ofc_device_count(int *n)
{
    OFC_REQUIRE(n, "null pointer");
    int c = 0;
    hipError_t e = hipGetDeviceCount(&c);
    *n = (e == hipSuccess) ? c : 0;
    return OFC_OK;
}

int ofc_malloc(int device, size_t bytes, void **dptr)
{
    OFC_REQUIRE(dptr, "null pointer");
    OFC_TRY(ensure_device(device));
    OFC_HIP(hipMalloc(dptr, bytes));
    return OFC_OK;
}

int ofc_free(int device, void *dptr)
{
    OFC_TRY(ensure_device(device));
    OFC_HIP(hipFree(dptr));
    return OFC_OK;
}

int ofc_memcpy_h2d(int device, void *dst, const void *src, size_t bytes)
{
    OFC_TRY(ensure_device(device));
    OFC_HIP(hipMemcpy(dst, src, bytes, hipMemcpyHostToDevice));
    return OFC_OK;
}

int ofc_memcpy_d2h(int device, void *dst, const void *src, size_t bytes)
{
    OFC_TRY(ensure_device(device));
    OFC_HIP(hipMemcpy(dst, src, bytes, hipMemcpyDeviceToHost));
    return OFC_OK;
}

int ofc_memset(int device, void *dst, int value, size_t bytes)
{
    OFC_TRY(ensure_device(device));
    OFC_HIP(hipMemset(dst, value, bytes));
    return OFC_OK;
}

int ofc_device_sync(int device)
{
    OFC_TRY(ensure_device(device));
    OFC_HIP(hipDeviceSynchronize());
    return OFC_OK;
}

void ofc_fb_default_params(ofc_fb_params *p)
{
    if (!p) return;
    p->pyr_scale = 0.5; p->levels = 3; p->winsize = 15; p->iterations = 3;
    p->poly_n = 5; p->poly_sigma = 1.2; p->flags = 0;
}

}

struct ofc_flow {
    int device = 0, W = 0, H = 0, max_batch = 0, levels = 0;
    ofc_fb_params prm{};
    PolyConsts pc{};
    std::vector<LevelGeom> geom;
    hipStream_t stream = nullptr;
    DevBuf I, R, M, flowA, flowB, flowC;
    bool fused = true;
    bool fuse_level0 = true;
    bool fuse2 = false;
    int fuse2_min_w = 0;
    bool w3 = false;
    int w3_min_w = 0;
    DevBuf frames2, flow1;
    DevBuf prev_gray;
    bool have_prev = false;
    DevBuf bgr_in, vis, vis_partial, vis_stats, mean_mag;
    DevBuf uv_scratch;
    struct Captured {
        const uint8_t *frames = nullptr;
        int n_frames = 0;
        float *flow = nullptr;
        double *uv_sum = nullptr;
        int hits = 0;
        hipGraph_t graph = nullptr;
        hipGraphExec_t exec = nullptr;
    };
    std::vector<Captured> graphs;
    bool use_graph = false;
};

namespace ofc {

static int flow_run(ofc_flow *f, const uint8_t *frames_dev, int n_frames, float *flow_dev, double *uv_sum_dev = nullptr)
{
    const int npair = n_frames - 1;
    const int W = f->W, H = f->H;
    hipStream_t s = f->stream;
    float *I = f->I.as<float>(), *R = f->R.as<float>();
    const int iters = f->prm.iterations;
    float *prevFlow = nullptr;
    int pw = 0, ph = 0;
    for (int k = f->levels; k >= 0; k--) {
        const LevelGeom &g = f->geom[k];
        const size_t P = (size_t)g.w * g.h;
        float *dst = (k == 0) ? flow_dev : (((f->levels - k) & 1) ? f->flowB.as<float>() : f->flowA.as<float>());
        float *tmp = f->flowC.as<float>();
        if (k == 0 && f->fuse_level0 && polyexp_u8_ok(W, H, g)) {
            OFC_TRY(launch_polyexp_u8(frames_dev, R, n_frames, W, H, f->pc, s));
        } else {
            OFC_TRY(launch_level_image(frames_dev, I, n_frames, W, H, g, s));
            OFC_TRY(launch_polyexp(I, R, n_frames, g.w, g.h, f->pc, 0, s));
        }
        const size_t strideR = 5 * P;
        const float mul = (float)(1. / f->prm.pyr_scale);
        if (f->fused) {
            const bool two = f->fuse2 && f->prm.winsize == 15 && g.w >= f->fuse2_min_w;
            int plan[64], L = 0;
            for (int i = 0; i < iters;) {
                const int n = (two && i > 0 && iters - i >= 2) ? 2 : 1;
                plan[L++] = n;
                i += n;
            }
            const float *cur = nullptr;
            for (int l = 0; l < L; l++) {
                float *nxt = ((L - 1 - l) & 1) ? tmp : dst;
                if (l == 0 && prevFlow) {
                    OFC_TRY(launch_flow_iter(R, strideR, nullptr, nxt, npair, g.w, g.h, f->prm.winsize, s, prevFlow, pw, ph, mul));
                } else {
                    if (l == 0) {
                        float *z = (nxt == dst) ? tmp : dst;
                        OFC_HIP(hipMemsetAsync(z, 0, sizeof(float) * 2 * P * npair, s));
                        cur = z;
                    }
                    if (uv_sum_dev && k == 0 && l == L - 1 && plan[l] == 1 && f->prm.winsize == 15 && !(f->w3 && g.w >= f->w3_min_w)) {
                        const size_t need = (size_t)flow_iter_max_grid(g.w, g.h, npair, f->prm.winsize) * 2;
                        if (f->uv_scratch.bytes < need * sizeof(double)) OFC_TRY(f->uv_scratch.alloc(need * sizeof(double)));
                        OFC_TRY(launch_flow_iter(R, strideR, cur, nxt, npair, g.w, g.h, f->prm.winsize, s, nullptr, 0, 0, 1.f,
                                                 uv_sum_dev, f->uv_scratch.as<double>(), need));
                        uv_sum_dev = nullptr;
                    } else
                    if (plan[l] == 2) OFC_TRY(launch_flow_iter2(R, strideR, cur, nxt, npair, g.w, g.h, f->prm.winsize, s));
                    else if (f->w3 && f->prm.winsize == 15 && g.w >= f->w3_min_w)
                        OFC_TRY(launch_flow_iter_w3(R, strideR, cur, nxt, npair, g.w, g.h, f->prm.winsize, s));
                    else OFC_TRY(launch_flow_iter(R, strideR, cur, nxt, npair, g.w, g.h, f->prm.winsize, s));
                }
                cur = nxt;
            }
        } else {
            float *cur = dst;
            if (!prevFlow) {
                OFC_HIP(hipMemsetAsync(cur, 0, sizeof(float) * 2 * P * npair, s));
            } else {
                OFC_TRY(launch_flow_resize(prevFlow, cur, npair, pw, ph, g.w, g.h, mul, s));
            }
            float *M = f->M.as<float>();
            OFC_TRY(launch_update_matrices(R, R + strideR, strideR, cur, M, npair, g.w, g.h, s));
            for (int i = 0; i < iters; i++) {
                OFC_TRY(launch_box_solve(M, cur, npair, g.w, g.h, f->prm.winsize, 0, s));
                if (i < iters - 1)
                    OFC_TRY(launch_update_matrices(R, R + strideR, strideR, cur, M, npair, g.w, g.h, s));
            }
        }
        prevFlow = dst;
        pw = g.w; ph = g.h;
    }
    if (uv_sum_dev) {
        const int64_t N = (int64_t)npair * W * H;
        const int nblocks = (int)std::max<int64_t>(1, std::min<int64_t>(cdiv64(N / 4, 256), 1024));
        if (f->uv_scratch.bytes < sizeof(double) * 2 * nblocks) OFC_TRY(f->uv_scratch.alloc(sizeof(double) * 2 * nblocks));
        OFC_TRY(launch_lloyd_colstats(flow_dev, OFC_F32, N, 2, nullptr, 0, f->uv_scratch.as<double>(), nblocks, s));
        OFC_TRY(launch_reduce_records(f->uv_scratch.as<double>(), nblocks, 2, uv_sum_dev, s));
    }
    return OFC_OK;
}

static int flow_run_cached(ofc_flow *f, const uint8_t *frames_dev, int n_frames, float *flow_dev, double *uv_sum_dev)
{
    if (!f->use_graph) return flow_run(f, frames_dev, n_frames, flow_dev, uv_sum_dev);
    ofc_flow::Captured *c = nullptr;
    for (auto &g : f->graphs)
        if (g.frames == frames_dev && g.n_frames == n_frames && g.flow == flow_dev && g.uv_sum == uv_sum_dev) { c = &g; break; }
    if (!c) {
        if (f->graphs.size() >= 64) {
            for (auto &g : f->graphs) {
                if (g.exec) (void)hipGraphExecDestroy(g.exec);
                if (g.graph) (void)hipGraphDestroy(g.graph);
            }
            f->graphs.clear();
        }
        f->graphs.emplace_back();
        c = &f->graphs.back();
        c->frames = frames_dev; c->n_frames = n_frames; c->flow = flow_dev; c->uv_sum = uv_sum_dev;
    }
    c->hits++;
    if (c->exec) {
        OFC_HIP(hipGraphLaunch(c->exec, f->stream));
        return OFC_OK;
    }
    if (c->hits < 2) return flow_run(f, frames_dev, n_frames, flow_dev, uv_sum_dev);
    OFC_HIP(hipStreamBeginCapture(f->stream, hipStreamCaptureModeThreadLocal));
    const int rc = flow_run(f, frames_dev, n_frames, flow_dev, uv_sum_dev);
    hipGraph_t g = nullptr;
    const hipError_t e = hipStreamEndCapture(f->stream, &g);
    if (rc != OFC_OK || e != hipSuccess || !g) {
        if (g) (void)hipGraphDestroy(g);
        f->use_graph = false;
        (void)hipGetLastError();
        return flow_run(f, frames_dev, n_frames, flow_dev, uv_sum_dev);
    }
    hipGraphExec_t ex = nullptr;
    if (hipGraphInstantiate(&ex, g, nullptr, nullptr, 0) != hipSuccess || !ex) {
        (void)hipGraphDestroy(g);
        f->use_graph = false;
        (void)hipGetLastError();
        return flow_run(f, frames_dev, n_frames, flow_dev, uv_sum_dev);
    }
    c->graph = g;
    c->exec = ex;
    OFC_HIP(hipGraphLaunch(c->exec, f->stream));
    return OFC_OK;
}

}

extern "C" {

int ofc_flow_create(int device, int W, int H, const ofc_fb_params *p, int max_batch, ofc_flow_t **out)
{
    OFC_REQUIRE(out, "null out pointer");
    *out = nullptr;
    ofc_fb_params prm;
    if (p) prm = *p; else ofc_fb_default_params(&prm);
    OFC_TRY(check_params(prm, W, H));
    OFC_REQUIRE(max_batch >= 1 && max_batch <= 4096, "max_batch out of range");
    OFC_REQUIRE((prm.winsize & 1) && prm.winsize >= 5, "winsize must be odd and >= 5");
    std::unique_ptr<ofc_flow> f(new ofc_flow);
    f->device = device; f->W = W; f->H = H; f->max_batch = max_batch; f->prm = prm;
    f->levels = pyramid_levels(W, H, prm);
    for (int k = 0; k <= f->levels; k++) f->geom.push_back(level_geometry(W, H, prm, k));
    {
        const char *e = getenv("OFC_FLOW_STAGED");
        f->fused = prm.winsize <= 15 && !(e && e[0] == '1');
        f->fuse_level0 = !(e && e[0] == '1');
        const char *e3 = getenv("OFC_FLOW_W3");
        if (e3 && e3[0]) {
            const int v = atoi(e3);
            f->w3 = v != 0;
            f->w3_min_w = v > 1 ? v : 0;
        }
        const char *eg = getenv("OFC_FLOW_GRAPH");
        f->use_graph = eg && eg[0] == '1';
        const char *e2 = getenv("OFC_FLOW_FUSE2");
        if (e2 && e2[0]) {
            const int v = atoi(e2);
            f->fuse2 = v != 0;
            if (v > 1) f->fuse2_min_w = v;
        }
    }
    OFC_TRY(flow_levels_check(W, H, prm, f->geom.data(), f->levels, f->fused, f->fuse_level0));
    OFC_TRY(ensure_device(device));
    polyexp_setup(prm.poly_n, prm.poly_sigma, f->pc);
    OFC_HIP(hipStreamCreateWithFlags(&f->stream, hipStreamNonBlocking));
    const size_t P0 = (size_t)W * H, nb = (size_t)max_batch;
    OFC_TRY(f->I.alloc(sizeof(float) * P0 * (nb + 1)));
    OFC_TRY(f->R.alloc(sizeof(float) * 5 * P0 * (nb + 1)));
    if (f->fused) {
        OFC_TRY(f->flowC.alloc(sizeof(float) * 2 * P0 * nb));
    } else {
        OFC_TRY(f->M.alloc(sizeof(float) * 5 * P0 * nb));
    }
    const size_t P1 = f->levels >= 1 ? (size_t)f->geom[1].w * f->geom[1].h : 1;
    OFC_TRY(f->flowA.alloc(sizeof(float) * 2 * P1 * nb));
    OFC_TRY(f->flowB.alloc(sizeof(float) * 2 * P1 * nb));
    OFC_TRY(f->frames2.alloc(2 * P0));
    OFC_TRY(f->flow1.alloc(sizeof(float) * 2 * P0));
    OFC_TRY(f->prev_gray.alloc(P0));
    *out = f.release();
    return OFC_OK;
}

void ofc_flow_destroy(ofc_flow_t *f)
{
    if (!f) return;
    (void)hipSetDevice(f->device);
    if (f->stream) {
        (void)hipStreamSynchronize(f->stream);
        (void)hipStreamDestroy(f->stream);
    }
    for (auto &g : f->graphs) {
        if (g.exec) (void)hipGraphExecDestroy(g.exec);
        if (g.graph) (void)hipGraphDestroy(g.graph);
    }
    delete f;
}

int ofc_flow_calc_frames_dev(ofc_flow_t *f, const uint8_t *frames_dev, int n_frames, float *flow_dev)
{
    OFC_REQUIRE(f && frames_dev && flow_dev, "null pointer");
    OFC_REQUIRE(n_frames >= 2 && n_frames - 1 <= f->max_batch, "n_frames-1 = %d pairs not in [1, max_batch=%d]",
                n_frames - 1, f->max_batch);
    OFC_TRY(ensure_device(f->device));
    return flow_run_cached(f, frames_dev, n_frames, flow_dev, nullptr);
}

int ofc_flow_calc_frames_dev_stats(ofc_flow_t *f, const uint8_t *frames_dev, int n_frames, float *flow_dev, double *uv_sum_dev)
{
    OFC_REQUIRE(f && frames_dev && flow_dev && uv_sum_dev, "null pointer");
    OFC_REQUIRE(n_frames >= 2 && n_frames - 1 <= f->max_batch, "n_frames-1 = %d pairs not in [1, max_batch=%d]",
                n_frames - 1, f->max_batch);
    OFC_TRY(ensure_device(f->device));
    return flow_run_cached(f, frames_dev, n_frames, flow_dev, uv_sum_dev);
}

hipStream_t ofc_flow_stream_internal(ofc_flow_t *f) { return f->stream; }

int ofc_flow_sync(ofc_flow_t *f)
{
    OFC_REQUIRE(f, "null pointer");
    OFC_TRY(ensure_device(f->device));
    OFC_HIP(hipStreamSynchronize(f->stream));
    return OFC_OK;
}

int ofc_flow_calc(ofc_flow_t *f, const uint8_t *prev_gray, const uint8_t *next_gray, float *flow_out)
{
    OFC_REQUIRE(f && prev_gray && next_gray && flow_out, "null pointer");
    OFC_TRY(ensure_device(f->device));
    const size_t P0 = (size_t)f->W * f->H;
    uint8_t *fr = f->frames2.as<uint8_t>();
    OFC_HIP(hipMemcpyAsync(fr, prev_gray, P0, hipMemcpyHostToDevice, f->stream));
    OFC_HIP(hipMemcpyAsync(fr + P0, next_gray, P0, hipMemcpyHostToDevice, f->stream));
    OFC_TRY(flow_run(f, fr, 2, f->flow1.as<float>()));
    OFC_HIP(hipMemcpyAsync(flow_out, f->flow1.p, sizeof(float) * 2 * P0, hipMemcpyDeviceToHost, f->stream));
    OFC_HIP(hipStreamSynchronize(f->stream));
    return OFC_OK;
}

int ofc_flow_push_gray(ofc_flow_t *f, const uint8_t *gray, float *flow_out)
{
    OFC_REQUIRE(f && gray, "null pointer");
    OFC_TRY(ensure_device(f->device));
    const size_t P0 = (size_t)f->W * f->H;
    uint8_t *fr = f->frames2.as<uint8_t>();
    if (!f->have_prev) {
        OFC_HIP(hipMemcpyAsync(f->prev_gray.p, gray, P0, hipMemcpyHostToDevice, f->stream));
        OFC_HIP(hipStreamSynchronize(f->stream));
        f->have_prev = true;
        set_error("first frame pushed: no pair yet");
        return OFC_ENOTREADY;
    }
    OFC_REQUIRE(flow_out, "null flow_out");
    OFC_HIP(hipMemcpyAsync(fr, f->prev_gray.p, P0, hipMemcpyDeviceToDevice, f->stream));
    OFC_HIP(hipMemcpyAsync(fr + P0, gray, P0, hipMemcpyHostToDevice, f->stream));
    OFC_HIP(hipMemcpyAsync(f->prev_gray.p, fr + P0, P0, hipMemcpyDeviceToDevice, f->stream));
    OFC_TRY(flow_run(f, fr, 2, f->flow1.as<float>()));
    OFC_HIP(hipMemcpyAsync(flow_out, f->flow1.p, sizeof(float) * 2 * P0, hipMemcpyDeviceToHost, f->stream));
    OFC_HIP(hipStreamSynchronize(f->stream));
    return OFC_OK;
}

int ofc_flow_push_bgr(ofc_flow_t *f, const uint8_t *bgr, uint8_t *vis_out, float *mean_mag, float *flow_out)
{
    OFC_REQUIRE(f && bgr, "null pointer");
    OFC_TRY(ensure_device(f->device));
    const size_t P0 = (size_t)f->W * f->H;
    hipStream_t s = f->stream;
    if (!f->bgr_in.p) {
        OFC_TRY(f->bgr_in.alloc(P0 * 3 + 16));
        OFC_TRY(f->vis.alloc(P0 * 3 + 16));
        OFC_TRY(f->vis_partial.alloc(sizeof(double) * 3 * VIS_BLOCKS));
        OFC_TRY(f->vis_stats.alloc(sizeof(VisFrameStats)));
        OFC_TRY(f->mean_mag.alloc(sizeof(float)));
    }
    uint8_t *fr = f->frames2.as<uint8_t>();
    OFC_HIP(hipMemcpyAsync(f->bgr_in.p, bgr, P0 * 3, hipMemcpyHostToDevice, s));
    if (!f->have_prev) {
        OFC_TRY(launch_bgr2gray(f->bgr_in.as<uint8_t>(), f->prev_gray.as<uint8_t>(), (int64_t)P0, s));
        OFC_HIP(hipStreamSynchronize(s));
        f->have_prev = true;
        set_error("first frame pushed: no pair yet");
        return OFC_ENOTREADY;
    }
    OFC_HIP(hipMemcpyAsync(fr, f->prev_gray.p, P0, hipMemcpyDeviceToDevice, s));
    OFC_TRY(launch_bgr2gray(f->bgr_in.as<uint8_t>(), fr + P0, (int64_t)P0, s));
    OFC_HIP(hipMemcpyAsync(f->prev_gray.p, fr + P0, P0, hipMemcpyDeviceToDevice, s));
    OFC_TRY(flow_run(f, fr, 2, f->flow1.as<float>()));
    OFC_TRY(launch_flow_to_bgr(f->flow1.as<float>(), f->W, f->H, 1, f->vis.as<uint8_t>(), f->mean_mag.as<float>(),
                               f->vis_partial.as<double>(), f->vis_stats.as<VisFrameStats>(), s));
    if (vis_out) OFC_HIP(hipMemcpyAsync(vis_out, f->vis.p, P0 * 3, hipMemcpyDeviceToHost, s));
    if (mean_mag) OFC_HIP(hipMemcpyAsync(mean_mag, f->mean_mag.p, sizeof(float), hipMemcpyDeviceToHost, s));
    if (flow_out) OFC_HIP(hipMemcpyAsync(flow_out, f->flow1.p, sizeof(float) * 2 * P0, hipMemcpyDeviceToHost, s));
    OFC_HIP(hipStreamSynchronize(s));
    return OFC_OK;
}

int ofc_flow_last_vis_dev(ofc_flow_t *f, const uint8_t **vis_dev)
{
    OFC_REQUIRE(f && vis_dev, "null pointer");
    OFC_REQUIRE(f->vis.p, "no visualisation yet: call ofc_flow_push_bgr twice first");
    *vis_dev = f->vis.as<uint8_t>();
    return OFC_OK;
}

static void interleave5(const float *planar, size_t P, float *inter)
{
    for (int c = 0; c < 5; c++)
        for (size_t i = 0; i < P; i++) inter[i * 5 + c] = planar[c * P + i];
}
static void planarize5(const float *inter, size_t P, float *planar)
{
    for (int c = 0; c < 5; c++)
        for (size_t i = 0; i < P; i++) planar[c * P + i] = inter[i * 5 + c];
}

int ofc_level_image(int device, const uint8_t *gray, int W, int H, const ofc_fb_params *p, int k,
                    float *out, int *w_out, int *h_out)
{
    OFC_REQUIRE(gray && out, "null pointer");
    ofc_fb_params prm;
    if (p) prm = *p; else ofc_fb_default_params(&prm);
    OFC_TRY(check_params(prm, W, H));
    OFC_REQUIRE(k >= 0 && k <= pyramid_levels(W, H, prm), "level %d out of range", k);
    OFC_TRY(ensure_device(device));
    LevelGeom g = level_geometry(W, H, prm, k);
    DevBuf src, dst;
    OFC_TRY(src.alloc((size_t)W * H));
    OFC_TRY(dst.alloc(sizeof(float) * g.w * g.h));
    OFC_HIP(hipMemcpy(src.p, gray, (size_t)W * H, hipMemcpyHostToDevice));
    OFC_TRY(launch_level_image(src.as<uint8_t>(), dst.as<float>(), 1, W, H, g, nullptr));
    OFC_HIP(hipMemcpy(out, dst.p, sizeof(float) * g.w * g.h, hipMemcpyDeviceToHost));
    if (w_out) *w_out = g.w;
    if (h_out) *h_out = g.h;
    return OFC_OK;
}

int ofc_polyexp(int device, const float *img, int W, int H, int n, double sigma, float *R5)
{
    OFC_REQUIRE(img && R5, "null pointer");
    OFC_REQUIRE(W >= 1 && H >= 1, "bad size");
    OFC_TRY(polyexp_n_check(n));
    OFC_TRY(ensure_device(device));
    const size_t P = (size_t)W * H;
    PolyConsts pc;
    polyexp_setup(n, sigma, pc);
    DevBuf I, R;
    OFC_TRY(I.alloc(sizeof(float) * P));
    OFC_TRY(R.alloc(sizeof(float) * 5 * P));
    OFC_HIP(hipMemcpy(I.p, img, sizeof(float) * P, hipMemcpyHostToDevice));
    OFC_TRY(launch_polyexp(I.as<float>(), R.as<float>(), 1, W, H, pc, 0, nullptr));
    OFC_HIP(hipMemcpy(R5, R.p, sizeof(float) * 5 * P, hipMemcpyDeviceToHost));
    return OFC_OK;
}

int ofc_polyexp_u8(int device, const uint8_t *gray, int W, int H, int n, double sigma, float *R5)
{
    OFC_REQUIRE(gray && R5 && W >= 1 && H >= 1, "bad arguments");
    OFC_TRY(polyexp_n_check(n));
    OFC_TRY(ensure_device(device));
    ofc_fb_params prm = {0.5, 0, 15, 3, n, sigma, 0};
    const LevelGeom g = level_geometry(W, H, prm, 0);
    if (!polyexp_u8_ok(W, H, g)) { set_error("fused level-0 expansion needs W >= 4 and H >= 2"); return OFC_EUNSUPPORTED; }
    const size_t P = (size_t)W * H;
    PolyConsts pc;
    polyexp_setup(n, sigma, pc);
// ... 201 lines not shown
```

opticalflowclustering_amd/csrc/ofc_common.h:

```cpp
#pragma once
#include <hip/hip_runtime.h>
#include <cstdarg>
#include <cstdint>
#include <cstdio>
#include <cstring>
#include <string>
#include <vector>

#include "../../include/ofc.h"

namespace ofc {

void set_error(const char *fmt, ...);
int ensure_device(int device);

#define OFC_HIP(expr)                                                                         \
    do {                                                                                      \
        hipError_t _e = (expr);                                                               \
        if (_e != hipSuccess) {                                                               \
            ofc::set_error("%s failed: %s (%s:%d)", #expr, hipGetErrorString(_e), __FILE__,   \
                           __LINE__);                                                         \
            return _e == hipErrorOutOfMemory ? OFC_ENOMEM : OFC_EHIP;                         \
        }                                                                                     \
    } while (0)

#define OFC_TRY(expr)                    \
    do {                                 \
        int _rc = (expr);                \
        if (_rc != OFC_OK) return _rc;   \
    } while (0)

#define OFC_REQUIRE(cond, ...)           \
    do {                                 \
        if (!(cond)) {                   \
            ofc::set_error(__VA_ARGS__); \
            return OFC_EINVAL;           \
        }                                \
    } while (0)

struct DevBuf {
    void *p = nullptr;
    size_t bytes = 0;
    DevBuf() = default;
    DevBuf(const DevBuf &) = delete;
    DevBuf &operator=(const DevBuf &) = delete;
    ~DevBuf() { release(); }
    int alloc(size_t n)
    {
        release();
        if (n == 0) return OFC_OK;
        OFC_HIP(hipMalloc(&p, n));
        bytes = n;
        return OFC_OK;
    }
    void release()
    {
        if (p) (void)hipFree(p);
        p = nullptr;
        bytes = 0;
    }
    template <class T> T *as() const { return reinterpret_cast<T *>(p); }
};

static inline int cdiv(int a, int b) { return (a + b - 1) / b; }
static inline int64_t cdiv64(int64_t a, int64_t b) { return (a + b - 1) / b; }

struct LevelGeom {
    int w, h, ksize;
    double sigma;
};
int pyramid_levels(int W, int H, const ofc_fb_params &p);
LevelGeom level_geometry(int W, int H, const ofc_fb_params &p, int k);
void gaussian_kernel(int n, double sigma, float *k);
struct PolyConsts {
    int n;
    float g[8], xg[8], xxg[8];
    double ig11, ig03, ig33, ig55;
};
void polyexp_setup(int n, double sigma, PolyConsts &c);
int polyexp_n_check(int n);
constexpr int WINSIZE_WIDE_MIN = 19;

int launch_level_image(const uint8_t *src, float *dst, int nimg, int W0, int H0,
                       const LevelGeom &g, hipStream_t s);
bool polyexp_u8_ok(int W, int H, const LevelGeom &g);
int launch_polyexp_u8(const uint8_t *frames, float *R, int nimg, int W, int H, const PolyConsts &c, hipStream_t s);
int launch_polyexp(const float *I, float *R, int nimg, int W, int H, const PolyConsts &c,
                   int rows_per_block, hipStream_t s, bool bench_tag = false);
int launch_update_matrices(const float *R0, const float *R1, size_t pair_stride_R,
                           const float *flow, float *M, int npair, int W, int H, hipStream_t s);
int launch_box_solve(const float *M, float *flow, int npair, int W, int H, int winsize,
                     int rows_per_block, hipStream_t s);
int launch_flow_resize(const float *src, float *dst, int npair, int sw, int sh, int dw, int dh,
                       float mul, hipStream_t s);
int launch_flow_iter(const float *R, size_t frame_stride_R, const float *flow_in, float *flow_out,
                     int npair, int W, int H, int winsize, hipStream_t s, const float *coarse = nullptr,
                     int sw = 0, int sh = 0, float mul = 1.f, double *uv_sum = nullptr, double *uv_scratch = nullptr,
                     size_t uv_scratch_doubles = 0);
int flow_iter_max_grid(int W, int H, int npair, int winsize);
int launch_flow_iter2(const float *R, size_t frame_stride_R, const float *flow_in, float *flow_out, int npair, int W,
                      int H, int winsize, hipStream_t s, int rows_per_block = 0);
int launch_flow_iter_w3(const float *R, size_t frame_stride_R, const float *flow_in, float *flow_out, int npair, int W,
                        int H, int winsize, hipStream_t s, int rows_per_block = 0);
int launch_flow_iter_pipe(const float *R, size_t frame_stride_R, const float *flow_in, float *flow_out, int npair, int W,
                          int H, int rows_per_block, hipStream_t s, double *uv_sum, double *uv_scratch,
                          size_t uv_scratch_doubles);
int launch_flow_iter_stamped(const float *R, size_t frame_stride_R, const float *flow_in, float *flow_out, int npair, int W,
                             int H, hipStream_t s, unsigned long long *dbg, int *grid_out);
int flow_levels_check(int W, int H, const ofc_fb_params &p, const LevelGeom *geom, int levels, bool fused, bool fuse_level0);
int polyexp_default_rows(int W, int H, int nimg);
int box_default_rows(int W, int H, int npair);
int box_wide_rows(int winsize);

}
```

opticalflowclustering_amd/flow.py:

```python
import ctypes as C
import threading
from collections import OrderedDict

import numpy as np

from . import _lib
from ._lib import FbParams, check, load, ptr


class FlowEngine:

    def __init__(self, W, H, params=None, max_batch=1, device=0):
        self.W, self.H, self.device, self.max_batch = int(W), int(H), device, int(max_batch)
        self.params = params or FbParams()
        h = C.c_void_p()
        check(load().ofc_flow_create(device, self.W, self.H, C.byref(self.params), self.max_batch, C.byref(h)))
        self._h = h

    def calc(self, prev_gray, next_gray, out=None):
        prev_gray = np.ascontiguousarray(prev_gray, np.uint8)
        next_gray = np.ascontiguousarray(next_gray, np.uint8)
        if prev_gray.shape != (self.H, self.W) or next_gray.shape != (self.H, self.W):
            raise ValueError(f"expected two {self.H}x{self.W} uint8 images")
        if out is None:
            out = np.empty((self.H, self.W, 2), np.float32)
        elif not _is_flow_buffer(out, self.H, self.W):
            raise ValueError(f"out must be a writeable C-contiguous {self.H}x{self.W}x2 float32 array")
        check(load().ofc_flow_calc(self._h, ptr(prev_gray), ptr(next_gray), ptr(out)))
        return out

    def push(self, gray):
        gray = np.ascontiguousarray(gray, np.uint8)
        if gray.shape != (self.H, self.W):
            raise ValueError(f"expected a {self.H}x{self.W} uint8 image")
        flow = np.empty((self.H, self.W, 2), np.float32)
        rc = load().ofc_flow_push_gray(self._h, ptr(gray), ptr(flow))
        if rc == _lib.OFC_ENOTREADY:
            return None
        check(rc)
        return flow

    def calc_frames_dev(self, frames_ptr, n_frames, flow_ptr, sync=True, uv_sum_ptr=None):
        if uv_sum_ptr:
            check(load().ofc_flow_calc_frames_dev_stats(self._h, C.c_void_p(frames_ptr), n_frames, C.c_void_p(flow_ptr),
                                                        C.c_void_p(uv_sum_ptr)))
        else:
            check(load().ofc_flow_calc_frames_dev(self._h, C.c_void_p(frames_ptr), n_frames, C.c_void_p(flow_ptr)))
        if sync:
            self.sync()

    def sync(self):
        check(load().ofc_flow_sync(self._h))

    def close(self):
        if getattr(self, "_h", None):
            load().ofc_flow_destroy(self._h)
            self._h = None

    def __del__(self):
        try:
            self.close()
        except Exception:
            pass


def _is_flow_buffer(a, H, W):
    return (isinstance(a, np.ndarray) and a.dtype == np.float32 and a.shape == (H, W, 2)
            and a.flags.c_contiguous and a.flags.writeable)


OPTFLOW_USE_INITIAL_FLOW = 4
OPTFLOW_FARNEBACK_GAUSSIAN = 256

_FB_CACHE_MAX = 4
_fb_engines = OrderedDict()
_fb_lock = threading.Lock()


def _gray_arg(a, name):
    if not isinstance(a, np.ndarray) or a.dtype != np.uint8 or a.ndim != 2:
        raise ValueError(f"{name} must be a 2-D uint8 array (one grey frame)")
    return np.ascontiguousarray(a)


def calcOpticalFlowFarneback(prev, next, flow, pyr_scale, levels, winsize, iterations, poly_n, poly_sigma, flags,
                             device=0):
    prev = _gray_arg(prev, "prev")
    next = _gray_arg(next, "next")
    if prev.shape != next.shape:
        raise ValueError(f"prev {prev.shape} and next {next.shape} differ in shape")
    H, W = prev.shape
    out = flow if _is_flow_buffer(flow, H, W) else np.empty((H, W, 2), np.float32)
    key = (int(device), W, H, float(pyr_scale), int(levels), int(winsize), int(iterations), int(poly_n),
           float(poly_sigma), int(flags))
    with _fb_lock:
        eng = _fb_engines.get(key)
        if eng is None:
            eng = FlowEngine(W, H, FbParams(*key[3:]), max_batch=1, device=key[0])
            _fb_engines[key] = eng
            while len(_fb_engines) > _FB_CACHE_MAX:
                _fb_engines.popitem(last=False)[1].close()
        else:
            _fb_engines.move_to_end(key)
        eng.calc(prev, next, out)
    return out


def clear_farneback_cache():
    with _fb_lock:
        while _fb_engines:
            _fb_engines.popitem()[1].close()
```

opticalflowclustering_amd/pipeline.py:

```python
import ctypes as C

import numpy as np

from . import _lib
from ._lib import DeviceBuffer, FbParams, check, load
from .cluster import kmeans_fit_dev, kmeans_plusplus_dev
from .flow import FlowEngine


def shard_pairs(n_pairs, world, rank):
    base, rem = divmod(n_pairs, world)
    start = rank * base + min(rank, rem)
    return start, start + base + (1 if rank < rem else 0)


def batch_schedule(n_pairs, batch_pairs):
    if isinstance(batch_pairs, (list, tuple)):
        schedule = [int(b) for b in batch_pairs]
        if sum(schedule) != n_pairs or min(schedule) < 1:
            raise ValueError(f"batch schedule {schedule} does not cover {n_pairs} pairs")
        return schedule
    b = max(1, min(int(batch_pairs), n_pairs))
    return ([n_pairs % b] if n_pairs % b else []) + [b] * (n_pairs // b)


class ClipPipeline:
    def __init__(self, W, H, n_frames_local, batch_pairs=16, params=None, device=0, n_engines=2):
        self.W, self.H, self.device = W, H, device
        self.n_frames = int(n_frames_local)
        self.n_pairs = self.n_frames - 1
        self.schedule = batch_schedule(self.n_pairs, batch_pairs)
        self.batch = max(self.schedule)
        self.engines = [FlowEngine(W, H, params or FbParams(), max_batch=self.batch, device=device)
                        for _ in range(max(1, min(n_engines, len(self.schedule))))]
        self.engine = self.engines[0]
        P = W * H
        self.frames = DeviceBuffer(self.n_frames * P, device)
        self.flows = DeviceBuffer(self.n_pairs * P * 8, device)
        self.labels = DeviceBuffer(self.n_pairs * P, device)
        self.n_batches = len(self.schedule)
        self.uv_sums = DeviceBuffer(self.n_batches * 16, device)
        self._sums_valid = False

    def synth(self, t0=0, seed=0):
        check(load().ofc_synth_frames_dev(self.device, C.c_void_p(self.frames.ptr), self.W, self.H,
                                          self.n_frames, t0, seed))

    def upload_frames(self, frames):
        frames = np.ascontiguousarray(frames, np.uint8)
        assert frames.shape == (self.n_frames, self.H, self.W)
        self.frames.upload(frames)

    def run_flow(self, sync=True, stats=True):
        P = self.W * self.H
        p0 = 0
        for i, n in enumerate(self.schedule):
            self.engines[i % len(self.engines)].calc_frames_dev(self.frames.ptr + p0 * P, n + 1,
                                                                self.flows.ptr + p0 * P * 8, sync=False,
                                                                uv_sum_ptr=self.uv_sums.ptr + 16 * i if stats else None)
            p0 += n
        self._sums_valid = stats
        if sync:
            self.sync()

    def sync(self):
        for e in self.engines:
            e.sync()

    def run_kmeans(self, init, max_iter=300, tol=1e-4, k=None, random_state=None, n_global=None):
        self.sync()
        N = self.n_pairs * self.W * self.H
        colsum = None
        if self._sums_valid:
            per_batch = self.uv_sums.download((self.n_batches, 2), np.float64)
            colsum = np.zeros(2)
            for b in range(self.n_batches):
                colsum += per_batch[b]
        if isinstance(init, str):
            if init != "k-means++" or k is None:
                raise ValueError(f"init should be a (k,2) array or 'k-means++' together with k=, got {init!r}, k={k!r}")
            init, _ = kmeans_plusplus_dev(self.flows.ptr, _lib.F32, N, 2, int(k), random_state, device=self.device,
                                          colsum=colsum, n_global=n_global)
        return kmeans_fit_dev(self.flows.ptr, _lib.F32, N, 2, init, max_iter, tol, self.labels.ptr, self.device, colsum=colsum)

    def sample_uv(self, idx):
        out = np.empty((len(idx), 2), np.float32)
        for i, j in enumerate(idx):
            out[i] = self.flows.download((2,), np.float32, offset=int(j) * 8)
        return out

    def flows_host(self):
        return self.flows.download((self.n_pairs, self.H, self.W, 2), np.float32)

    def labels_host(self):
        return self.labels.download((self.n_pairs, self.H, self.W), np.uint8)

    def close(self):
        for e in self.engines:
            e.close()
        for b in (self.frames, self.flows, self.labels, self.uv_sums):
            b.free()
```

Baseline: 16710 Mpixels/s.

## Emit k-means tile records from the final flow iteration kernel

The last Farneback iteration kernel now stages each output row in shared memory and computes per-64-sample tile records (bounding box, sum, squared sum) for the pruned Lloyd k-means. The k-means fit then reuses these records instead of running a separate META pass over the whole flow field, and only handles the segments the flow tiles did not cover. This removes one full read of the flow field, at the cost of extra shared memory, compute and register pressure inside the flow kernel and more coupling between the two stages.

```diff
diff --git a/include/ofc.h b/include/ofc.h
--- a/include/ofc.h
+++ b/include/ofc.h
@@ -59,6 +59,9 @@
                              float *flow_dev);
 int ofc_flow_calc_frames_dev_stats(ofc_flow_t *f, const uint8_t *frames_dev, int n_frames,
                                    float *flow_dev, double *uv_sum_dev);
+int ofc_flow_calc_frames_dev_tiles(ofc_flow_t *f, const uint8_t *frames_dev, int n_frames, float *flow_dev,
+                                   double *uv_sum_dev, void *box_dev, void *sum_dev, void *sq_dev, int64_t tile0);
+int ofc_flow_tile_width(const ofc_flow_t *f);
 int ofc_flow_sync(ofc_flow_t *f);
 
 int ofc_flow_push_gray(ofc_flow_t *f, const uint8_t *gray, float *flow_out);
@@ -104,6 +107,11 @@
 int ofc_kmeans_fit_dev_stats(int device, const void *X_dev, int dtype, int64_t N, int d, int k,
                              const double *init, int max_iter, double tol_rel, const double *colsum,
                              double *centers, uint8_t *labels_dev, double *inertia, int *n_iter);
+int ofc_kmeans_fit_dev_tiles(int device, const float *X_dev, int64_t N, int k, const double *init, int max_iter,
+                             double tol_rel, const double *colsum, int W, int tile_w, void *box_dev, void *sum_dev,
+                             void *sq_dev, double *centers, uint8_t *labels_dev, double *inertia, int *n_iter);
+int ofc_lloyd_tile_records_dev(int device, const float *X_dev, int64_t N, const double *mean, int W, int tile_w,
+                               void *box_dev, void *sum_dev, void *sq_dev, double *sqsum);
 int ofc_lloyd_prune_stats(int device, double *out6);
 int ofc_bench_lloyd_sweep(int device, const float *X_dev, int64_t N, int k, const double *centers, const double *mean,
                           int what, int iters, float *ms_per_launch);
diff --git a/opticalflowclustering_amd/_lib.py b/opticalflowclustering_amd/_lib.py
--- a/opticalflowclustering_amd/_lib.py
+++ b/opticalflowclustering_amd/_lib.py
@@ -49,6 +49,8 @@
     "ofc_flow_calc": ([_vp, _vp, _vp, _vp], _i),
     "ofc_flow_calc_frames_dev": ([_vp, _vp, _i, _vp], _i),
     "ofc_flow_calc_frames_dev_stats": ([_vp, _vp, _i, _vp, _vp], _i),
+    "ofc_flow_calc_frames_dev_tiles": ([_vp, _vp, _i, _vp, _vp, _vp, _vp, _vp, _i64], _i),
+    "ofc_flow_tile_width": ([_vp], _i),
     "ofc_flow_sync": ([_vp], _i),
     "ofc_flow_push_gray": ([_vp, _vp, _vp], _i),
     "ofc_flow_push_bgr": ([_vp, _vp, _vp, C.POINTER(_f), _vp], _i),
@@ -72,6 +74,8 @@
     "ofc_kmeans_predict": ([_i, _vp, _i, _i64, _i, _i, _vp, _vp], _i),
     "ofc_kmeans_fit_dev": ([_i, _vp, _i, _i64, _i, _i, _vp, _i, _d, _vp, _vp, C.POINTER(_d), _ip], _i),
     "ofc_kmeans_fit_dev_stats": ([_i, _vp, _i, _i64, _i, _i, _vp, _i, _d, _vp, _vp, _vp, C.POINTER(_d), _ip], _i),
+    "ofc_kmeans_fit_dev_tiles": ([_i, _vp, _i64, _i, _vp, _i, _d, _vp, _i, _i, _vp, _vp, _vp, _vp, _vp, C.POINTER(_d), _ip], _i),
+    "ofc_lloyd_tile_records_dev": ([_i, _vp, _i64, _vp, _i, _i, _vp, _vp, _vp, _vp], _i),
     "ofc_lloyd_prune_stats": ([_i, _vp], _i),
     "ofc_bench_lloyd_sweep": ([_i, _vp, _i64, _i, _vp, _vp, _i, _i, C.POINTER(_f)], _i),
     "ofc_lloyd_colstats_dev": ([_i, _vp, _i, _i64, _i, _vp, _i, _vp], _i),
diff --git a/opticalflowclustering_amd/cluster.py b/opticalflowclustering_amd/cluster.py
--- a/opticalflowclustering_amd/cluster.py
+++ b/opticalflowclustering_amd/cluster.py
@@ -173,7 +173,8 @@
         return self.fit(X).labels_
 
 
-def kmeans_fit_dev(X_ptr, dtype, N, d, init, max_iter=300, tol=1e-4, labels_ptr=None, device=0, colsum=None):
+def kmeans_fit_dev(X_ptr, dtype, N, d, init, max_iter=300, tol=1e-4, labels_ptr=None, device=0, colsum=None,
+                   tile_records=None):
     C0 = np.ascontiguousarray(init, np.float64)
     k = C0.shape[0]
     centers = np.empty((k, d), np.float64)
@@ -181,6 +182,14 @@
     cs = np.ascontiguousarray(colsum, np.float64) if colsum is not None else None
     if cs is not None and cs.shape != (d,):
         raise ValueError(f"colsum must have shape ({d},)")
+    if tile_records is not None:
+        if dtype != _lib.F32 or d != 2:
+            raise ValueError("tile_records come with a float32 (u,v) field only")
+        box, tsum, tsq, W, tile_w = tile_records
+        check(load().ofc_kmeans_fit_dev_tiles(device, C.c_void_p(X_ptr), N, k, ptr(C0), max_iter, tol, ptr(cs), W, tile_w,
+                                              C.c_void_p(box), C.c_void_p(tsum), C.c_void_p(tsq), ptr(centers),
+                                              C.c_void_p(labels_ptr) if labels_ptr else None, C.byref(inertia), C.byref(n_iter)))
+        return centers, inertia.value, n_iter.value
     check(load().ofc_kmeans_fit_dev_stats(device, C.c_void_p(X_ptr), dtype, N, d, k, ptr(C0), max_iter, tol, ptr(cs), ptr(centers),
                                           C.c_void_p(labels_ptr) if labels_ptr else None, C.byref(inertia), C.byref(n_iter)))
     return centers, inertia.value, n_iter.value
diff --git a/opticalflowclustering_amd/csrc/flow_kernels.hip b/opticalflowclustering_amd/csrc/flow_kernels.hip
--- a/opticalflowclustering_amd/csrc/flow_kernels.hip
+++ b/opticalflowclustering_amd/csrc/flow_kernels.hip
@@ -1,4 +1,5 @@
 #include "flow_device.h"
+#include "lloyd_device.h"
 
 namespace ofc {
 
@@ -953,6 +954,12 @@
     return make_float2((h0x * b0 + h1x * b1) * mul, (h0y * b0 + h1y * b1) * mul);
 }
 
+struct FlowTileRecs {
+    v4f *box;
+    v2d *sum;
+    double *sq;
+};
+
 template <int M, int UPS, bool STAMP = false, bool SUMS = false>
 __global__ __launch_bounds__(256, 2) void k_flow_iter(const float *__restrict__ Rb, size_t frame_stride_R,
                                                       const float *__restrict__ flow_inb,
@@ -960,7 +967,8 @@
                                                       int rows_per_block , UpsArgs ups,
                                                       int tiles_x, int n_strips, int npair,
                                                       unsigned long long *__restrict__ dbg = nullptr,
-                                                      double *__restrict__ sums = nullptr)
+                                                      double *__restrict__ sums = nullptr,
+                                                      FlowTileRecs recs = FlowTileRecs{nullptr, nullptr, nullptr})
 {
     constexpr int TXO = 256 - 2 * M;
     constexpr int NV = 2 * M + 4;
@@ -981,6 +989,15 @@
     const int y_begin = tile_y * rows_per_block;
     const int y_end = min(y_begin + rows_per_block, H);
     const size_t plane = (size_t)W * H;
+    const bool with_recs = SUMS && recs.box != nullptr;
+    int rec_off = 0, rec_n = 0;
+    size_t rec_t0 = 0;
+    if (with_recs) {
+        const int seg0 = (x0 + 63) >> 6;
+        rec_off = seg0 * 64 - x0;
+        rec_n = (min(TXO, W - x0) - rec_off) >> 6;
+        rec_t0 = (size_t)pair * H * (W >> 6) + seg0;
+    }
     const float *R0 = Rb + (size_t)pair * frame_stride_R;
     const float *R1 = R0 + frame_stride_R;
     const float2 *flow_in = UPS ? reinterpret_cast<const float2 *>(ups.src) + (size_t)pair * ups.sw * ups.sh
@@ -1019,6 +1036,7 @@
     bool have_next = false;
     float2 fl_last = ups2 ? flow_at(H - 1) : make_float2(0.f, 0.f);
 
+    __shared__ __align__(16) float2 rec_row[SUMS ? BS_ROWS : 1][SUMS ? 256 : 2];
     float ring[16][5];
     double v[5] = {0, 0, 0, 0, 0};
 
@@ -1185,6 +1203,13 @@
                         for (int o = 0; o < 4; o++)
                             if (4 * lane + o < TXO && xo + o < W) { su += (double)fo[o].x; sv += (double)fo[o].y; }
                     }
+                    if constexpr (SUMS) {
+                        if (with_recs) {
+                            float4 *rb = reinterpret_cast<float4 *>(&rec_row[wave][4 * lane]);
+                            rb[0] = make_float4(fo[0].x, fo[0].y, fo[1].x, fo[1].y);
+                            rb[1] = make_float4(fo[2].x, fo[2].y, fo[3].x, fo[3].y);
+                        }
+                    }
                     float2 *dst = flow_out + (size_t)y * W + xo;
                     if (4 * lane + 3 < TXO && xo + 3 < W && (W & 1) == 0) {
                         reinterpret_cast<float4 *>(dst)[0] = make_float4(fo[0].x, fo[0].y, fo[1].x, fo[1].y);
@@ -1193,6 +1218,23 @@
 #pragma unroll
                         for (int o = 0; o < 4; o++)
                             if (4 * lane + o < TXO && xo + o < W) dst[o] = fo[o];
+                    }
+                }
+                if constexpr (SUMS) {
+                    if (with_recs && y < y_end && (lane >> 4) < rec_n) {
+                        const int seg = lane >> 4, r16 = lane & 15;
+                        const float2 *rp = &rec_row[wave][rec_off + 64 * seg + 4 * r16];
+                        const float2 p0 = rp[0], p1 = rp[1], p2 = rp[2], p3 = rp[3];
+                        double x[8], sc;
+                        v4f bx;
+                        v2d sm;
+                        tile_record(v4f{p0.x, p0.y, p1.x, p1.y}, v4f{p2.x, p2.y, p3.x, p3.y}, 0.0, 0.0, x, bx, sm, sc);
+                        if (r16 == 0) {
+                            const size_t t = rec_t0 + (size_t)y * (W >> 6) + seg;
+                            recs.box[t] = bx;
+                            recs.sum[t] = sm;
+                            recs.sq[t] = sc;
+                        }
                     }
                 }
                 stamp(6);
@@ -1246,7 +1288,7 @@
 
 int launch_flow_iter(const float *R, size_t frame_stride_R, const float *flow_in, float *flow_out,
                      int npair, int W, int H, int winsize, hipStream_t s, const float *coarse, int sw, int sh,
-                     float mul, double *uv_sum, double *uv_scratch, size_t uv_scratch_doubles)
+                     float mul, double *uv_sum, double *uv_scratch, size_t uv_scratch_doubles, TileRecs *recs)
 {
     OFC_TRY(flow_iter_check(W, H, winsize));
     const int rows_per_block = flow_iter_rows(W, H, npair, winsize);
@@ -1264,8 +1306,13 @@
         const int tx = cdiv(W, 256 - 14), ns = cdiv(H, rows_per_block);
         const int grid = cdiv(tx * ns, 8) * 8 * npair;
         if ((size_t)grid * 2 > uv_scratch_doubles) { set_error("flow sums: scratch too small (%d work-groups)", grid); return OFC_EINVAL; }
+        FlowTileRecs fr{nullptr, nullptr, nullptr};
+        if (recs && recs->box && (W & 63) == 0) {
+            fr = FlowTileRecs{(v4f *)recs->box, (v2d *)recs->sum, (double *)recs->sq};
+            recs->emitted = true;
+        }
         hipLaunchKernelGGL((k_flow_iter<7, 0, false, true>), dim3(grid), dim3(256), 0, s, R, frame_stride_R, flow_in, flow_out, W, H,
-                           rows_per_block, u, tx, ns, npair, nullptr, uv_scratch);
+                           rows_per_block, u, tx, ns, npair, nullptr, uv_scratch, fr);
         OFC_HIP(hipGetLastError());
         return launch_reduce_records(uv_scratch, grid, 2, uv_sum, s, nullptr);
     }
diff --git a/opticalflowclustering_amd/csrc/lloyd_api.cpp b/opticalflowclustering_amd/csrc/lloyd_api.cpp
--- a/opticalflowclustering_amd/csrc/lloyd_api.cpp
+++ b/opticalflowclustering_amd/csrc/lloyd_api.cpp
@@ -145,9 +145,14 @@
     return OFC_OK;
 }
 
+struct FieldRecs {
+    void *box, *sum, *sq;
+    int W, txo;
+};
+
 static int lloyd_fit_dev(int device, const void *X, int dtype, int64_t N, int d, int k, const double *init,
                          int max_iter, double tol_rel, double *centers, uint8_t *labels_dev,
-                         double *inertia, int *n_iter, const double *colsum = nullptr)
+                         double *inertia, int *n_iter, const double *colsum = nullptr, const FieldRecs *recs = nullptr)
 {
     OFC_REQUIRE(X && init && centers, "null pointer");
     OFC_REQUIRE(dtype >= OFC_U8 && dtype <= OFC_F64, "bad dtype %d", dtype);
@@ -196,13 +201,18 @@
     for (int j = 0; j < k * d; j++) c0[j] = init[j] - mean_h[j % d];
     OFC_HIP(hipMemcpyAsync(st->centers, c0, sizeof(double) * k * d, hipMemcpyHostToDevice, s));
     const int prune = prune_policy_for(dtype, N, d, k);
+    if (!prune) recs = nullptr;
+    void *t_box = nullptr, *t_sum = nullptr, *t_sq = nullptr;
     if (prune) {
         const size_t need = (size_t)(N >> 6) * 16;
-        if (sc.tile_box.bytes < need) {
-            OFC_TRY(sc.tile_box.alloc(need));
-            OFC_TRY(sc.tile_sum.alloc(need));
-            OFC_TRY(sc.tile_sq.alloc(need / 2));
-        }
+        if (sc.tile_sum.bytes < need) OFC_TRY(sc.tile_sum.alloc(need));
+        if (!recs) {
+            if (sc.tile_box.bytes < need) OFC_TRY(sc.tile_box.alloc(need));
+            if (sc.tile_sq.bytes < need / 2) OFC_TRY(sc.tile_sq.alloc(need / 2));
+        }
+        t_box = recs ? recs->box : sc.tile_box.p;
+        t_sq = recs ? recs->sq : sc.tile_sq.p;
+        t_sum = sc.tile_sum.p;
     }
     for (double &v : sc.prune_stats) v = 0;
     OFC_TRY(launch_lloyd_set_centers(st, k, d, s, prune));
@@ -222,12 +232,17 @@
             if (tiles == 1) {
                 OFC_TRY(launch_lloyd_tiles((const float *)X, N, k, st, nullptr, nullptr, nullptr, nullptr,
                                            sc.partial.as<double>(), nblocks, LLOYD_WHAT_PROBE, nullptr, s));
-                OFC_TRY(launch_lloyd_tiles((const float *)X, N, k, st, sc.tile_box.p, sc.tile_sum.p, sc.tile_sq.p, nullptr,
+                if (recs) {
+                    OFC_TRY(launch_tile_records_rest((const float *)X, N / recs->W, recs->W, recs->txo, st, recs->box, recs->sum,
+                                                     recs->sq, nblocks, s));
+                    OFC_TRY(launch_tile_centre(N >> 6, st, recs->sum, recs->sq, t_sum, sc.partial.as<double>(), nblocks, s));
+                } else
+                OFC_TRY(launch_lloyd_tiles((const float *)X, N, k, st, t_box, t_sum, t_sq, nullptr,
                                            sc.partial.as<double>(), nblocks, LLOYD_WHAT_META, nullptr, s));
                 OFC_TRY(launch_reduce_records(sc.partial.as<double>(), nblocks, 2, sc.tile_meta.as<double>(), s));
             }
             if (tiles)
-                OFC_TRY(launch_lloyd_tiles((const float *)X, N, k, st, sc.tile_box.p, sc.tile_sum.p, sc.tile_sq.p, nullptr,
+                OFC_TRY(launch_lloyd_tiles((const float *)X, N, k, st, t_box, t_sum, t_sq, nullptr,
                                            sc.partial.as<double>(), nblocks, LLOYD_WHAT_SWEEP,
                                            tiles == 1 ? sc.tile_meta.as<double>() : nullptr, s));
             else
@@ -278,7 +293,7 @@
     const bool final_tiles = !strict && prune && !labelled && tiles_next == LLOYD_TILES_PRUNED;
     sc.prune_stats[5] = final_tiles ? 1 : 0;
     if (final_tiles)
-        OFC_TRY(launch_lloyd_tiles((const float *)X, N, k, st, sc.tile_box.p, sc.tile_sum.p, sc.tile_sq.p, labels_dev,
+        OFC_TRY(launch_lloyd_tiles((const float *)X, N, k, st, t_box, t_sum, t_sq, labels_dev,
                                    sc.partial.as<double>(), nblocks, LLOYD_WHAT_FINAL, nullptr, s));
     else if (!strict)
         OFC_TRY(launch_lloyd_assign(X, dtype, N, d, k, st, labels_dev, sc.partial.as<double>(), nblocks, 2, 0, s));
@@ -347,11 +362,9 @@
     hipStream_t s = sc.stream;
     const int nblocks = lloyd_grid(N);
     const size_t need = (size_t)(N >> 6) * 16;
-    if (sc.tile_box.bytes < need) {
-        OFC_TRY(sc.tile_box.alloc(need));
-        OFC_TRY(sc.tile_sum.alloc(need));
-        OFC_TRY(sc.tile_sq.alloc(need / 2));
-    }
+    if (sc.tile_box.bytes < need) OFC_TRY(sc.tile_box.alloc(need));
+    if (sc.tile_sum.bytes < need) OFC_TRY(sc.tile_sum.alloc(need));
+    if (sc.tile_sq.bytes < need / 2) OFC_TRY(sc.tile_sq.alloc(need / 2));
     if (sc.labels.bytes < (size_t)N) OFC_TRY(sc.labels.alloc((size_t)N));
     LloydState *st = sc.state.as<LloydState>();
     OFC_HIP(hipMemsetAsync(st, 0, sizeof(LloydState), s));
@@ -407,6 +420,46 @@
                              double *inertia, int *n_iter)
 {
     return lloyd_fit_dev(device, X_dev, dtype, N, d, k, init, max_iter, tol_rel, centers, labels_dev, inertia, n_iter, colsum);
+}
+
+int ofc_kmeans_fit_dev_tiles(int device, const float *X_dev, int64_t N, int k, const double *init, int max_iter,
+                             double tol_rel, const double *colsum, int W, int tile_w, void *box_dev, void *sum_dev,
+                             void *sq_dev, double *centers, uint8_t *labels_dev, double *inertia, int *n_iter)
+{
+    OFC_REQUIRE(box_dev && sum_dev && sq_dev, "null pointer");
+    OFC_REQUIRE(W >= 64 && W % 64 == 0 && N >= 0 && N % W == 0, "tile records need rows of a multiple of 64 samples (W=%d)", W);
+    OFC_REQUIRE(tile_w >= 64, "tile_w=%d: a column tile holds at least one 64-sample segment", tile_w);
+    const FieldRecs r{box_dev, sum_dev, sq_dev, W, tile_w};
+    return lloyd_fit_dev(device, X_dev, OFC_F32, N, 2, k, init, max_iter, tol_rel, centers, labels_dev, inertia, n_iter, colsum, &r);
+}
+
+int ofc_lloyd_tile_records_dev(int device, const float *X_dev, int64_t N, const double *mean, int W, int tile_w,
+                               void *box_dev, void *sum_dev, void *sq_dev, double *sqsum)
+{
+    OFC_REQUIRE(X_dev && mean && box_dev && sum_dev && sq_dev && sqsum && N >= 64, "bad arguments");
+    OFC_REQUIRE(W == 0 || (W >= 64 && W % 64 == 0 && N % W == 0 && tile_w >= 0), "bad geometry");
+    OFC_TRY(ensure_device(device));
+    LloydScratch &sc = scratch_for(device);
+    std::lock_guard<std::mutex> lock(sc.mu);
+    OFC_TRY(sc.init());
+    hipStream_t s = sc.stream;
+    const int nblocks = lloyd_grid(N);
+    LloydState *st = sc.state.as<LloydState>();
+    OFC_HIP(hipMemsetAsync(st, 0, sizeof(LloydState), s));
+    OFC_HIP(hipMemcpyAsync(st->mean, mean, sizeof(double) * 2, hipMemcpyHostToDevice, s));
+    const int policy = LLOYD_PRUNE_ALWAYS;
+    OFC_HIP(hipMemcpyAsync(&st->prune_policy, &policy, sizeof(int), hipMemcpyHostToDevice, s));
+    double *partial = sc.partial.as<double>();
+    if (W == 0) {
+        OFC_TRY(launch_lloyd_tiles(X_dev, N, 1, st, box_dev, sum_dev, sq_dev, nullptr, partial, nblocks, LLOYD_WHAT_META, nullptr, s));
+    } else {
+        OFC_TRY(launch_tile_records_rest(X_dev, N / W, W, tile_w, st, box_dev, sum_dev, sq_dev, nblocks, s));
+        OFC_TRY(launch_tile_centre(N >> 6, st, sum_dev, sq_dev, sum_dev, partial, nblocks, s));
+    }
+    OFC_TRY(launch_reduce_records(partial, nblocks, 2, sc.tile_meta.as<double>(), s));
+    OFC_HIP(hipMemcpyAsync(sqsum, sc.tile_meta.p, sizeof(double) * 2, hipMemcpyDeviceToHost, s));
+    OFC_HIP(hipStreamSynchronize(s));
+    return OFC_OK;
 }
 
 namespace {
diff --git a/opticalflowclustering_amd/csrc/lloyd_common.h b/opticalflowclustering_amd/csrc/lloyd_common.h
--- a/opticalflowclustering_amd/csrc/lloyd_common.h
+++ b/opticalflowclustering_amd/csrc/lloyd_common.h
@@ -53,6 +53,10 @@
 bool lloyd_tiles_supported(int dtype, int d, int k);
 int launch_lloyd_tiles(const float *X, int64_t N, int k, const LloydState *st, void *box, void *tsum, void *tsq,
                        uint8_t *labels, double *partial, int nblocks, int what, const double *meta, hipStream_t s);
+int launch_tile_records_rest(const float *X, int64_t rows, int W, int txo, const LloydState *st, void *box, void *tsum,
+                             void *tsq, int nblocks, hipStream_t s);
+int launch_tile_centre(int64_t NT, const LloydState *st, const void *tsum_in, const void *tsq, void *tsum_out, double *partial,
+                       int nblocks, hipStream_t s);
 int launch_lloyd_update(LloydState *st, const double *tot, int k, int d, int after_reloc, int labelled, int first,
                         double n_total, double tol_rel, LloydStatus *status, hipStream_t s, int tiles = 0);
 constexpr int LLOYD_WINDOW = 16;
diff --git a/opticalflowclustering_amd/csrc/lloyd_device.h b/opticalflowclustering_amd/csrc/lloyd_device.h
--- a/opticalflowclustering_amd/csrc/lloyd_device.h
+++ b/opticalflowclustering_amd/csrc/lloyd_device.h
@@ -2,6 +2,54 @@
 #include "lloyd_common.h"
 
 namespace ofc {
+
+typedef float v4f __attribute__((ext_vector_type(4)));
+typedef double v2d __attribute__((ext_vector_type(2)));
+
+template <int N> __device__ __forceinline__ int row_ror(int v)
+{
+    return __builtin_amdgcn_update_dpp(0, v, 0x120 + N, 0xf, 0xf, false);
+}
+template <int N> __device__ __forceinline__ float row_ror(float v) { return __int_as_float(row_ror<N>(__float_as_int(v))); }
+template <int N> __device__ __forceinline__ double row_ror(double v)
+{
+    return __hiloint2double(row_ror<N>(__double2hiint(v)), row_ror<N>(__double2loint(v)));
+}
+__device__ __forceinline__ float row_min(float v)
+{
+    v = fminf(v, row_ror<8>(v)); v = fminf(v, row_ror<4>(v)); v = fminf(v, row_ror<2>(v)); return fminf(v, row_ror<1>(v));
+}
+__device__ __forceinline__ float row_max(float v)
+{
+    v = fmaxf(v, row_ror<8>(v)); v = fmaxf(v, row_ror<4>(v)); v = fmaxf(v, row_ror<2>(v)); return fmaxf(v, row_ror<1>(v));
+}
+__device__ __forceinline__ double row_sum(double v)
+{
+    v += row_ror<8>(v); v += row_ror<4>(v); v += row_ror<2>(v); return v + row_ror<1>(v);
+}
+
+__device__ __forceinline__ void tile_record(const v4f a, const v4f b, const double m0, const double m1, double (&x)[8],
+                                            v4f &bx, v2d &sm, double &sc)
+{
+    const double x00 = (double)a.x - m0, x01 = (double)a.y - m1, x10 = (double)a.z - m0, x11 = (double)a.w - m1;
+    const double x20 = (double)b.x - m0, x21 = (double)b.y - m1, x30 = (double)b.z - m0, x31 = (double)b.w - m1;
+    const float lu = row_min(fminf(fminf(a.x, a.z), fminf(b.x, b.z)));
+    const float lv = row_min(fminf(fminf(a.y, a.w), fminf(b.y, b.w)));
+    const float hu = row_max(fmaxf(fmaxf(a.x, a.z), fmaxf(b.x, b.z)));
+    const float hv = row_max(fmaxf(fmaxf(a.y, a.w), fmaxf(b.y, b.w)));
+    const double su = row_sum((x00 + x10) + (x20 + x30));
+    const double sv = row_sum((x01 + x11) + (x21 + x31));
+    const double mu = su * 0.015625, mv = sv * 0.015625;
+    double s = (x00 - mu) * (x00 - mu) + (x01 - mv) * (x01 - mv);
+    s += (x10 - mu) * (x10 - mu) + (x11 - mv) * (x11 - mv);
+    s += (x20 - mu) * (x20 - mu) + (x21 - mv) * (x21 - mv);
+    s += (x30 - mu) * (x30 - mu) + (x31 - mv) * (x31 - mv);
+    sc = row_sum(s);
+    bx = v4f{lu, lv, hu, hv};
+    if (!(su == su && sv == sv)) bx = v4f{__builtin_inff(), __builtin_inff(), -__builtin_inff(), -__builtin_inff()};
+    sm = v2d{su, sv};
+    x[0] = x00; x[1] = x01; x[2] = x10; x[3] = x11; x[4] = x20; x[5] = x21; x[6] = x30; x[7] = x31;
+}
 
 template <int D>
 __device__ __forceinline__ void load4(const uint8_t *X, int64_t i, double (&x)[4][D])
diff --git a/opticalflowclustering_amd/csrc/lloyd_tiles.hip b/opticalflowclustering_amd/csrc/lloyd_tiles.hip
--- a/opticalflowclustering_amd/csrc/lloyd_tiles.hip
+++ b/opticalflowclustering_amd/csrc/lloyd_tiles.hip
@@ -1,33 +1,8 @@
-#include "lloyd_common.h"
+#include "lloyd_device.h"
 
 #include <algorithm>
 
 namespace ofc {
-
-typedef float v4f __attribute__((ext_vector_type(4)));
-typedef double v2d __attribute__((ext_vector_type(2)));
-
-template <int N> __device__ __forceinline__ int row_ror(int v)
-{
-    return __builtin_amdgcn_update_dpp(0, v, 0x120 + N, 0xf, 0xf, false);
-}
-template <int N> __device__ __forceinline__ float row_ror(float v) { return __int_as_float(row_ror<N>(__float_as_int(v))); }
-template <int N> __device__ __forceinline__ double row_ror(double v)
-{
-    return __hiloint2double(row_ror<N>(__double2hiint(v)), row_ror<N>(__double2loint(v)));
-}
-__device__ __forceinline__ float row_min(float v)
-{
-    v = fminf(v, row_ror<8>(v)); v = fminf(v, row_ror<4>(v)); v = fminf(v, row_ror<2>(v)); return fminf(v, row_ror<1>(v));
-}
-__device__ __forceinline__ float row_max(float v)
-{
-    v = fmaxf(v, row_ror<8>(v)); v = fmaxf(v, row_ror<4>(v)); v = fmaxf(v, row_ror<2>(v)); return fmaxf(v, row_ror<1>(v));
-}
-__device__ __forceinline__ double row_sum(double v)
-{
-    v += row_ror<8>(v); v += row_ror<4>(v); v += row_ror<2>(v); return v + row_ror<1>(v);
-}
 
 template <int KMAX> struct TileCtx {
     double c[KMAX * 2], cn[KMAX], m[2];
@@ -179,27 +154,15 @@
         fetch(s + ss, na, nb);
         const int64_t t = s * 4 + row;
         if (t < NT) {
-            const double x00 = (double)a.x - m0, x01 = (double)a.y - m1, x10 = (double)a.z - m0, x11 = (double)a.w - m1;
-            const double x20 = (double)b.x - m0, x21 = (double)b.y - m1, x30 = (double)b.z - m0, x31 = (double)b.w - m1;
-            sq0 += x00 * x00; sq0 += x10 * x10; sq0 += x20 * x20; sq0 += x30 * x30;
-            sq1 += x01 * x01; sq1 += x11 * x11; sq1 += x21 * x21; sq1 += x31 * x31;
-            const float lu = row_min(fminf(fminf(a.x, a.z), fminf(b.x, b.z)));
-            const float lv = row_min(fminf(fminf(a.y, a.w), fminf(b.y, b.w)));
-            const float hu = row_max(fmaxf(fmaxf(a.x, a.z), fmaxf(b.x, b.z)));
-            const float hv = row_max(fmaxf(fmaxf(a.y, a.w), fmaxf(b.y, b.w)));
-            const double su = row_sum((x00 + x10) + (x20 + x30));
-            const double sv = row_sum((x01 + x11) + (x21 + x31));
-            const double mu = su * 0.015625, mv = sv * 0.015625;
-            double sc = (x00 - mu) * (x00 - mu) + (x01 - mv) * (x01 - mv);
-            sc += (x10 - mu) * (x10 - mu) + (x11 - mv) * (x11 - mv);
-            sc += (x20 - mu) * (x20 - mu) + (x21 - mv) * (x21 - mv);
-            sc += (x30 - mu) * (x30 - mu) + (x31 - mv) * (x31 - mv);
-            sc = row_sum(sc);
+            double x[8], sc;
+            v4f bx;
+            v2d sm;
+            tile_record(a, b, m0, m1, x, bx, sm, sc);
+            sq0 += x[0] * x[0]; sq0 += x[2] * x[2]; sq0 += x[4] * x[4]; sq0 += x[6] * x[6];
+            sq1 += x[1] * x[1]; sq1 += x[3] * x[3]; sq1 += x[5] * x[5]; sq1 += x[7] * x[7];
             if (r16 == 0) {
-                v4f bx = {lu, lv, hu, hv};
-                if (!(su == su && sv == sv)) bx = v4f{__builtin_inff(), __builtin_inff(), -__builtin_inff(), -__builtin_inff()};
                 box[t] = bx;
-                tsum[t] = v2d{su, sv};
+                tsum[t] = sm;
                 tsq[t] = sc;
             }
         }
@@ -217,6 +180,75 @@
     if (lane == 0) { s_red[wave][0] = sq0; s_red[wave][1] = sq1; }
     __syncthreads();
     if (tid < 2) partial[(size_t)blockIdx.x * 2 + tid] = ((s_red[0][tid] + s_red[1][tid]) + s_red[2][tid]) + s_red[3][tid];
+}
+
+__global__ __launch_bounds__(256) void k_tile_meta_rest(const float *__restrict__ X, int64_t rows, int tpr, int txo, int nb,
+                                                        const LloydState *__restrict__ st, v4f *__restrict__ box,
+                                                        v2d *__restrict__ tsum, double *__restrict__ tsq)
+{
+    if (st && st->prune_policy == LLOYD_PRUNE_OFF) return;
+    const int tid = threadIdx.x, lane = tid & 63, wave = tid >> 6, row = lane >> 4, r16 = lane & 15;
+    const int64_t NI = rows * nb;
+    const int64_t NS = (NI + 3) >> 2;
+    const int64_t s0 = (int64_t)blockIdx.x * 4 + wave, ss = (int64_t)gridDim.x * 4;
+    auto tile_of = [&](int64_t i) -> int64_t {
+        const int64_t r = i / nb;
+        const int q = (int)(i - r * nb);
+        return r * tpr + (txo ? ((q + 1) * txo) >> 6 : q);
+    };
+    auto fetch = [&](int64_t s, v4f &a, v4f &b) {
+        const int64_t i = s * 4 + row;
+        if (s < NS && i < NI) {
+            const v4f *p = reinterpret_cast<const v4f *>(X + tile_of(i) * 128 + r16 * 8);
+            a = __builtin_nontemporal_load(p);
+            b = __builtin_nontemporal_load(p + 1);
+        }
+    };
+    v4f na = {0, 0, 0, 0}, nb4 = na;
+    fetch(s0, na, nb4);
+    for (int64_t s = s0; s < NS; s += ss) {
+        const v4f a = na, b = nb4;
+        fetch(s + ss, na, nb4);
+        const int64_t i = s * 4 + row;
+        if (i < NI) {
+            double x[8], sc;
+            v4f bx;
+            v2d sm;
+            tile_record(a, b, 0.0, 0.0, x, bx, sm, sc);
+            if (r16 == 0) {
+                const int64_t t = tile_of(i);
+                box[t] = bx;
+                tsum[t] = sm;
+                tsq[t] = sc;
+            }
+        }
+    }
+}
+
+__global__ __launch_bounds__(256) void k_tile_centre(int64_t NT, const LloydState *__restrict__ st,
+                                                     const v2d *tsum_in, const double *__restrict__ tsq,
+                                                     v2d *tsum_out , double *__restrict__ partial)
+{
+    __shared__ double s_red[4];
+    const int tid = threadIdx.x, lane = tid & 63, wave = tid >> 6;
+    if (st->prune_policy == LLOYD_PRUNE_OFF) {
+        if (tid < 2) partial[(size_t)blockIdx.x * 2 + tid] = 0.0;
+        return;
+    }
+    const double m0 = st->mean[0], m1 = st->mean[1];
+    double sq = 0;
+    for (int64_t t = (int64_t)blockIdx.x * 256 + tid; t < NT; t += (int64_t)gridDim.x * 256) {
+#pragma clang fp contract(off)
+        const v2d su = __builtin_nontemporal_load(tsum_in + t);
+        const double sc = __builtin_nontemporal_load(tsq + t);
+        const double du = su.x * 0.015625 - m0, dv = su.y * 0.015625 - m1;
+        sq += sc + 64.0 * (du * du + dv * dv);
+        tsum_out[t] = v2d{su.x - 64.0 * m0, su.y - 64.0 * m1};
+    }
+    for (int off = 32; off >= 1; off >>= 1) sq += __shfl_down(sq, off, 64);
+    if (lane == 0) s_red[wave] = sq;
+    __syncthreads();
+    if (tid < 2) partial[(size_t)blockIdx.x * 2 + tid] = tid ? 0.0 : ((s_red[0] + s_red[1]) + s_red[2]) + s_red[3];
 }
 
 enum { TILES_SWEEP = 0, TILES_FINAL = 1 };
@@ -449,4 +481,27 @@
     return OFC_OK;
 }
 
-}
+int launch_tile_records_rest(const float *X, int64_t rows, int W, int txo, const LloydState *st, void *box, void *tsum,
+                             void *tsq, int nblocks, hipStream_t s)
+{
+    if (W < 64 || (W & 63) || txo < 0 || rows < 0) { set_error("tile records: W=%d is no multiple of 64", W); return OFC_EINVAL; }
+    const int tpr = W >> 6, nb = txo ? cdiv(W, txo) - 1 : tpr;
+    if (nb <= 0 || rows == 0) return OFC_OK;
+    const int64_t steps = cdiv64(rows * nb, 4);
+    const int grid = (int)std::max<int64_t>(1, std::min<int64_t>(cdiv64(steps, 4), nblocks));
+    hipLaunchKernelGGL(k_tile_meta_rest, dim3(grid), dim3(256), 0, s, X, rows, tpr, txo, nb, st, (v4f *)box, (v2d *)tsum,
+                       (double *)tsq);
+    OFC_HIP(hipGetLastError());
+    return OFC_OK;
+}
+
+int launch_tile_centre(int64_t NT, const LloydState *st, const void *tsum_in, const void *tsq, void *tsum_out, double *partial,
+                       int nblocks, hipStream_t s)
+{
+    hipLaunchKernelGGL(k_tile_centre, dim3(nblocks), dim3(256), 0, s, NT, st, (const v2d *)tsum_in, (const double *)tsq,
+                       (v2d *)tsum_out, partial);
+    OFC_HIP(hipGetLastError());
+    return OFC_OK;
+}
+
+}
diff --git a/opticalflowclustering_amd/csrc/ofc_api.cpp b/opticalflowclustering_amd/csrc/ofc_api.cpp
--- a/opticalflowclustering_amd/csrc/ofc_api.cpp
+++ b/opticalflowclustering_amd/csrc/ofc_api.cpp
@@ -231,6 +231,7 @@
         int n_frames = 0;
         float *flow = nullptr;
         double *uv_sum = nullptr;
+        void *rec_box = nullptr;
         int hits = 0;
         hipGraph_t graph = nullptr;
         hipGraphExec_t exec = nullptr;
@@ -241,7 +242,8 @@
 
 namespace ofc {
 
-static int flow_run(ofc_flow *f, const uint8_t *frames_dev, int n_frames, float *flow_dev, double *uv_sum_dev = nullptr)
+static int flow_run(ofc_flow *f, const uint8_t *frames_dev, int n_frames, float *flow_dev, double *uv_sum_dev = nullptr,
+                    TileRecs recs = TileRecs())
 {
     const int npair = n_frames - 1;
     const int W = f->W, H = f->H;
@@ -286,7 +288,7 @@
                         const size_t need = (size_t)flow_iter_max_grid(g.w, g.h, npair, f->prm.winsize) * 2;
                         if (f->uv_scratch.bytes < need * sizeof(double)) OFC_TRY(f->uv_scratch.alloc(need * sizeof(double)));
                         OFC_TRY(launch_flow_iter(R, strideR, cur, nxt, npair, g.w, g.h, f->prm.winsize, s, nullptr, 0, 0, 1.f,
-                                                 uv_sum_dev, f->uv_scratch.as<double>(), need));
+                                                 uv_sum_dev, f->uv_scratch.as<double>(), need, &recs));
                         uv_sum_dev = nullptr;
                     } else
                     if (plan[l] == 2) OFC_TRY(launch_flow_iter2(R, strideR, cur, nxt, npair, g.w, g.h, f->prm.winsize, s));
@@ -321,15 +323,18 @@
         OFC_TRY(launch_lloyd_colstats(flow_dev, OFC_F32, N, 2, nullptr, 0, f->uv_scratch.as<double>(), nblocks, s));
         OFC_TRY(launch_reduce_records(f->uv_scratch.as<double>(), nblocks, 2, uv_sum_dev, s));
     }
-    return OFC_OK;
-}
-
-static int flow_run_cached(ofc_flow *f, const uint8_t *frames_dev, int n_frames, float *flow_dev, double *uv_sum_dev)
-{
-    if (!f->use_graph) return flow_run(f, frames_dev, n_frames, flow_dev, uv_sum_dev);
+    if (recs.box && !recs.emitted)
+        OFC_TRY(launch_tile_records_rest(flow_dev, (int64_t)npair * H, W, 0, nullptr, recs.box, recs.sum, recs.sq, 2048, s));
+    return OFC_OK;
+}
+
+static int flow_run_cached(ofc_flow *f, const uint8_t *frames_dev, int n_frames, float *flow_dev, double *uv_sum_dev,
+                           TileRecs recs = TileRecs())
+{
+    if (!f->use_graph) return flow_run(f, frames_dev, n_frames, flow_dev, uv_sum_dev, recs);
     ofc_flow::Captured *c = nullptr;
     for (auto &g : f->graphs)
-        if (g.frames == frames_dev && g.n_frames == n_frames && g.flow == flow_dev && g.uv_sum == uv_sum_dev) { c = &g; break; }
+        if (g.frames == frames_dev && g.n_frames == n_frames && g.flow == flow_dev && g.uv_sum == uv_sum_dev && g.rec_box == recs.box) { c = &g; break; }
     if (!c) {
         if (f->graphs.size() >= 64) {
             for (auto &g : f->graphs) {
@@ -340,30 +345,30 @@
         }
         f->graphs.emplace_back();
         c = &f->graphs.back();
-        c->frames = frames_dev; c->n_frames = n_frames; c->flow = flow_dev; c->uv_sum = uv_sum_dev;
+        c->frames = frames_dev; c->n_frames = n_frames; c->flow = flow_dev; c->uv_sum = uv_sum_dev; c->rec_box = recs.box;
     }
     c->hits++;
     if (c->exec) {
         OFC_HIP(hipGraphLaunch(c->exec, f->stream));
         return OFC_OK;
     }
-    if (c->hits < 2) return flow_run(f, frames_dev, n_frames, flow_dev, uv_sum_dev);
+    if (c->hits < 2) return flow_run(f, frames_dev, n_frames, flow_dev, uv_sum_dev, recs);
     OFC_HIP(hipStreamBeginCapture(f->stream, hipStreamCaptureModeThreadLocal));
-    const int rc = flow_run(f, frames_dev, n_frames, flow_dev, uv_sum_dev);
+    const int rc = flow_run(f, frames_dev, n_frames, flow_dev, uv_sum_dev, recs);
     hipGraph_t g = nullptr;
     const hipError_t e = hipStreamEndCapture(f->stream, &g);
     if (rc != OFC_OK || e != hipSuccess || !g) {
         if (g) (void)hipGraphDestroy(g);
         f->use_graph = false;
         (void)hipGetLastError();
-        return flow_run(f, frames_dev, n_frames, flow_dev, uv_sum_dev);
+        return flow_run(f, frames_dev, n_frames, flow_dev, uv_sum_dev, recs);
     }
     hipGraphExec_t ex = nullptr;
     if (hipGraphInstantiate(&ex, g, nullptr, nullptr, 0) != hipSuccess || !ex) {
         (void)hipGraphDestroy(g);
         f->use_graph = false;
         (void)hipGetLastError();
-        return flow_run(f, frames_dev, n_frames, flow_dev, uv_sum_dev);
+        return flow_run(f, frames_dev, n_frames, flow_dev, uv_sum_dev, recs);
     }
     c->graph = g;
     c->exec = ex;
@@ -460,6 +465,26 @@
                 n_frames - 1, f->max_batch);
     OFC_TRY(ensure_device(f->device));
     return flow_run_cached(f, frames_dev, n_frames, flow_dev, uv_sum_dev);
+}
+
+int ofc_flow_calc_frames_dev_tiles(ofc_flow_t *f, const uint8_t *frames_dev, int n_frames, float *flow_dev, double *uv_sum_dev,
+                                   void *box_dev, void *sum_dev, void *sq_dev, int64_t tile0)
+{
+    OFC_REQUIRE(f && frames_dev && flow_dev && uv_sum_dev && box_dev && sum_dev && sq_dev, "null pointer");
+    OFC_REQUIRE(n_frames >= 2 && n_frames - 1 <= f->max_batch, "n_frames-1 = %d pairs not in [1, max_batch=%d]",
+                n_frames - 1, f->max_batch);
+    OFC_REQUIRE(f->W % 64 == 0 && tile0 >= 0, "tile records need a frame width that is a multiple of 64 (W=%d)", f->W);
+    OFC_TRY(ensure_device(f->device));
+    TileRecs r;
+    r.box = (char *)box_dev + tile0 * 16;
+    r.sum = (char *)sum_dev + tile0 * 16;
+    r.sq = (char *)sq_dev + tile0 * 8;
+    return flow_run_cached(f, frames_dev, n_frames, flow_dev, uv_sum_dev, r);
+}
+
+int ofc_flow_tile_width(const ofc_flow_t *f)
+{
+    return (f && f->fused && f->prm.winsize == 15) ? FLOW_ITER_TXO15 : 0;
 }
 
 hipStream_t ofc_flow_stream_internal(ofc_flow_t *f) { return f->stream; }
diff --git a/opticalflowclustering_amd/csrc/ofc_common.h b/opticalflowclustering_amd/csrc/ofc_common.h
--- a/opticalflowclustering_amd/csrc/ofc_common.h
+++ b/opticalflowclustering_amd/csrc/ofc_common.h
@@ -93,10 +93,15 @@
                      int rows_per_block, hipStream_t s);
 int launch_flow_resize(const float *src, float *dst, int npair, int sw, int sh, int dw, int dh,
                        float mul, hipStream_t s);
+struct TileRecs {
+    void *box = nullptr, *sum = nullptr, *sq = nullptr;
+    bool emitted = false;
+};
+constexpr int FLOW_ITER_TXO15 = 256 - 14;
 int launch_flow_iter(const float *R, size_t frame_stride_R, const float *flow_in, float *flow_out,
                      int npair, int W, int H, int winsize, hipStream_t s, const float *coarse = nullptr,
                      int sw = 0, int sh = 0, float mul = 1.f, double *uv_sum = nullptr, double *uv_scratch = nullptr,
-                     size_t uv_scratch_doubles = 0);
+                     size_t uv_scratch_doubles = 0, TileRecs *recs = nullptr);
 int flow_iter_max_grid(int W, int H, int npair, int winsize);
 int launch_flow_iter2(const float *R, size_t frame_stride_R, const float *flow_in, float *flow_out, int npair, int W,
                       int H, int winsize, hipStream_t s, int rows_per_block = 0);
diff --git a/opticalflowclustering_amd/flow.py b/opticalflowclustering_amd/flow.py
--- a/opticalflowclustering_amd/flow.py
+++ b/opticalflowclustering_amd/flow.py
@@ -40,8 +40,16 @@
         check(rc)
         return flow
 
-    def calc_frames_dev(self, frames_ptr, n_frames, flow_ptr, sync=True, uv_sum_ptr=None):
-        if uv_sum_ptr:
+    def tile_width(self):
+        return load().ofc_flow_tile_width(self._h)
+
+    def calc_frames_dev(self, frames_ptr, n_frames, flow_ptr, sync=True, uv_sum_ptr=None, tile_records=None):
+        if uv_sum_ptr and tile_records:
+            box, tsum, tsq, tile0 = tile_records
+            check(load().ofc_flow_calc_frames_dev_tiles(self._h, C.c_void_p(frames_ptr), n_frames, C.c_void_p(flow_ptr),
+                                                        C.c_void_p(uv_sum_ptr), C.c_void_p(box), C.c_void_p(tsum),
+                                                        C.c_void_p(tsq), tile0))
+        elif uv_sum_ptr:
             check(load().ofc_flow_calc_frames_dev_stats(self._h, C.c_void_p(frames_ptr), n_frames, C.c_void_p(flow_ptr),
                                                         C.c_void_p(uv_sum_ptr)))
         else:
diff --git a/opticalflowclustering_amd/pipeline.py b/opticalflowclustering_amd/pipeline.py
--- a/opticalflowclustering_amd/pipeline.py
+++ b/opticalflowclustering_amd/pipeline.py
@@ -25,7 +25,7 @@
 
 
 class ClipPipeline:
-    def __init__(self, W, H, n_frames_local, batch_pairs=16, params=None, device=0, n_engines=2):
+    def __init__(self, W, H, n_frames_local, batch_pairs=16, params=None, device=0, n_engines=2, tile_records=True):
         self.W, self.H, self.device = W, H, device
         self.n_frames = int(n_frames_local)
         self.n_pairs = self.n_frames - 1
@@ -41,6 +41,12 @@
         self.n_batches = len(self.schedule)
         self.uv_sums = DeviceBuffer(self.n_batches * 16, device)
         self._sums_valid = False
+        self.tile_w = self.engine.tile_width() if (tile_records and W % 64 == 0) else 0
+        self.recs = None
+        if self.tile_w:
+            nt = self.n_pairs * P // 64
+            self.recs = (DeviceBuffer(nt * 16, device), DeviceBuffer(nt * 16, device), DeviceBuffer(nt * 8, device))
+        self._recs_valid = False
 
     def synth(self, t0=0, seed=0):
         check(load().ofc_synth_frames_dev(self.device, C.c_void_p(self.frames.ptr), self.W, self.H,
@@ -54,12 +60,15 @@
     def run_flow(self, sync=True, stats=True):
         P = self.W * self.H
         p0 = 0
+        recs = self.recs if stats else None
         for i, n in enumerate(self.schedule):
-            self.engines[i % len(self.engines)].calc_frames_dev(self.frames.ptr + p0 * P, n + 1,
-                                                                self.flows.ptr + p0 * P * 8, sync=False,
-                                                                uv_sum_ptr=self.uv_sums.ptr + 16 * i if stats else None)
+            self.engines[i % len(self.engines)].calc_frames_dev(
+                self.frames.ptr + p0 * P, n + 1, self.flows.ptr + p0 * P * 8, sync=False,
+                uv_sum_ptr=self.uv_sums.ptr + 16 * i if stats else None,
+                tile_records=(recs[0].ptr, recs[1].ptr, recs[2].ptr, p0 * P // 64) if recs else None)
             p0 += n
         self._sums_valid = stats
+        self._recs_valid = recs is not None
         if sync:
             self.sync()
 
@@ -81,7 +90,9 @@
                 raise ValueError(f"init should be a (k,2) array or 'k-means++' together with k=, got {init!r}, k={k!r}")
             init, _ = kmeans_plusplus_dev(self.flows.ptr, _lib.F32, N, 2, int(k), random_state, device=self.device,
                                           colsum=colsum, n_global=n_global)
-        return kmeans_fit_dev(self.flows.ptr, _lib.F32, N, 2, init, max_iter, tol, self.labels.ptr, self.device, colsum=colsum)
+        recs = (self.recs[0].ptr, self.recs[1].ptr, self.recs[2].ptr, self.W, self.tile_w) if self._recs_valid else None
+        return kmeans_fit_dev(self.flows.ptr, _lib.F32, N, 2, init, max_iter, tol, self.labels.ptr, self.device, colsum=colsum,
+                              tile_records=recs)
 
     def sample_uv(self, idx):
         out = np.empty((len(idx), 2), np.float32)
@@ -98,5 +109,5 @@
     def close(self):
         for e in self.engines:
             e.close()
-        for b in (self.frames, self.flows, self.labels, self.uv_sums):
+        for b in (self.frames, self.flows, self.labels, self.uv_sums) + (self.recs or ()):
             b.free()
```

New measurement: 16800 Mpixels/s, median of 6. No clear change (+0.5%).
